# Andareon/Path-Tracing

Hardware: AMD Instinct MI355X
Metric: Msamples/sec (WxHxspp/wall) on Tor.obj 1080p x 256 spp (higher is better)
Workload: dtype f32

## Files before the change

path-tracing_amd/csrc/pt_capi.cpp:

```cpp
#include "pt_capi_internal.hpp"
#include "pt_bmp.hpp"

#include <algorithm>
#include <chrono>
#include <cmath>
#include <cstdio>
#include <cstdlib>
#include <cstring>
#include <thread>

#include "pt_filters.hpp"

static pt::plan::Overrides g_plan_overrides;

namespace ptc {

thread_local std::string g_error;

int fail(int code, const std::string &msg) {
    g_error = msg;
    return code;
}
int hip_fail(hipError_t e, const char *what) {
    const int code = (e == hipErrorNoDevice || e == hipErrorInvalidDevice || e == hipErrorInsufficientDriver)
                         ? PT_ERR_NO_DEVICE
                         : (e == hipErrorOutOfMemory ? PT_ERR_OUT_OF_MEMORY : PT_ERR_HIP);
    return fail(code, std::string(what) + ": " + hipGetErrorString(e));
}

std::atomic<long> g_live_device_objects{0};

int use_device(int device, const char *stage) {
    int n = 0;
    if (hipGetDeviceCount(&n) != hipSuccess || n <= 0 || device < 0 || device >= n)
        return fail(PT_ERR_NO_DEVICE, std::string(stage) + ": device " + std::to_string(device) + " is not a visible HIP device (there is no CPU fallback)");
    PT_HIP_TRY(hipSetDevice(device));
    return PT_OK;
}

}

using ptc::fail;
using ptc::guarded;
using ptc::hip_fail;

namespace {

int check_table_limits(unsigned long long n_slots, unsigned long long n_bvh_nodes, long long n_levels, long long bvh_depth = 0) {
    if (n_slots >= (1ull << 24))
        return fail(PT_ERR_UNSUPPORTED, "the culling hierarchy has " + std::to_string(n_slots) + " slots; (ray, slot) work items hold 24 bits");
    if (n_bvh_nodes >= (1ull << 20))
        return fail(PT_ERR_UNSUPPORTED, "the box tree has " + std::to_string(n_bvh_nodes) + " nodes; a node's child base holds 20 bits");
    if (n_bvh_nodes > 0 && n_slots >= (1ull << 23))
        return fail(PT_ERR_UNSUPPORTED, "the culling hierarchy has " + std::to_string(n_slots) + " slots under a box tree; a leaf's base (first slot / 8) holds 20 bits");
    if (bvh_depth > pt::kMaxBvhDepth)
        return fail(PT_ERR_UNSUPPORTED, "the box tree has " + std::to_string(bvh_depth) + " levels; the walk's stack slack holds " + std::to_string(pt::kMaxBvhDepth));
    if (n_levels > pt::kMaxLevels)
        return fail(PT_ERR_UNSUPPORTED, "a sphere tree has " + std::to_string(n_levels) + " levels; the walk holds " + std::to_string(pt::kMaxLevels));
    return PT_OK;
}

int get_cull(pt_scene_host &h, float eps, double r_camera, std::shared_ptr<const pt::CullTables> &out) {
    std::lock_guard<std::mutex> lock(h.cull_mutex);
#ifndef PT_TEST_HOOKS
    const double r_max = pt::cull_r_max(h.vertex_extent, r_camera);
    for (const auto &t : h.cull_cache)
        if (std::memcmp(&t->eps, &eps, sizeof eps) == 0 && t->r_max == r_max) {
            out = t;
            return PT_OK;
        }
#endif
    const auto t0 = std::chrono::steady_clock::now();
    auto t = std::make_shared<pt::CullTables>();
    pt::build_cull_tables(h.host, eps, *t, r_camera);
    t->eps = eps;
    h.cull_build_seconds += std::chrono::duration<double>(std::chrono::steady_clock::now() - t0).count();
    long long levels = 0;
    for (const auto &c : t->clusters)
        if (c.kind == 0) levels = std::max<long long>(levels, c.n_levels);
    const int rc = check_table_limits(t->slot_tri.size(), t->bvh.size(), levels, t->bvh_depth);
    if (rc != PT_OK) return rc;
    if (!t->big && (t->slot_tri.size() >= 65536u || h.host.n_tri() >= 65536))
        return fail(PT_ERR_UNSUPPORTED, "a scene on the sphere-tree path has " + std::to_string(t->slot_tri.size()) + " slots; its closest-hit key holds 16 bits");
    if (h.cull_cache.size() >= 4) h.cull_cache.erase(h.cull_cache.begin());
    h.cull_cache.push_back(t);
    out = t;
    return PT_OK;
}

int upload(pt_scene *s, int device) {
    int rc = ptc::use_device(device, "scene");
    if (rc != PT_OK) return rc;
    s->device = device;
    int cus = 0;
    if (hipDeviceGetAttribute(&cus, hipDeviceAttributeMultiprocessorCount, device) == hipSuccess && cus > 0) s->cu_count = cus;
    const auto &t = s->shared->tables;
    if ((rc = s->d_exact.upload(t.exact, "exact records", 64)) != PT_OK || (rc = s->d_mats.upload(t.mats, "materials", 64)) != PT_OK) return rc;
    if (s->sky && !s->sky->texels.empty()) {
        if ((rc = s->d_sky.upload(s->sky->texels, "skybox", 64)) != PT_OK) return rc;
        s->sky_w = s->sky->w;
        s->sky_h = s->sky->h;
    }
    if (s->env && (rc = s->d_env.upload(pt::env_with_apron(s->env->n, s->env->rgb.data()), "environment map", 64)) != PT_OK) return rc;
    if ((rc = ptc::upload_surface(s->surface, t, s->d_surface, s->d_surface)) != PT_OK) return rc;
    return PT_OK;
}

int ctx_stats_ready(LaunchCtx &c) {
    int rc = c.d_stats ? static_cast<int>(PT_OK) : c.d_stats.alloc(24 * sizeof(unsigned long long), "statistics block");
    if (rc == PT_OK && !c.ev0) rc = c.ev0.create("statistics");
    if (rc == PT_OK && !c.ev1) rc = c.ev1.create("statistics");
    return rc;
}

const pt_camera kReferenceCamera = {{0.0f, 0.0f, -20.0f}, {1.0f, 0.0f, 0.0f}, {0.0f, 1.0f, 0.0f}, {0.0f, 0.0f, 1.0f}};

using ptc::view_camera;

void lens_axes(const pt_camera &c, float out[9]) {
    const float *v[3] = {c.right, c.up, c.forward};
    for (int a = 0; a < 3; ++a) {
        const double x = v[a][0], y = v[a][1], z = v[a][2];
        const double n = std::sqrt(x * x + y * y + z * z);
        for (int i = 0; i < 3; ++i) out[3 * a + i] = static_cast<float>(v[a][i] / n);
    }
}

double lens_extent(const pt_camera &c, const pt_lens &l) {
    float ax[9];
    lens_axes(c, ax);
    double e = 0.0;
    for (int i = 0; i < 3; ++i) {
        const double lat = std::sqrt(static_cast<double>(ax[i]) * ax[i] + static_cast<double>(ax[3 + i]) * ax[3 + i]);
        double ei = std::fabs(static_cast<double>(c.origin[i]));
        if (lat > 0.0) ei = (ei + static_cast<double>(l.radius) * lat) * (1.0 + 0x1p-18);
        e = std::max(e, ei);
    }
    return e;
}

bool motion_active(const pt_scene *s) { return s->has_motion && std::memcmp(&view_camera(s), &s->motion_end, sizeof(pt_camera)) != 0; }

double motion_extent(const pt_camera &a, const pt_camera &b, const pt_lens *l) {
    float axa[9] = {0}, axb[9] = {0};
    if (l) {
        lens_axes(a, axa);
        lens_axes(b, axb);
    }
    double e = 0.0;
    for (int i = 0; i < 3; ++i) {
        const double lata = std::sqrt(static_cast<double>(axa[i]) * axa[i] + static_cast<double>(axa[3 + i]) * axa[3 + i]);
        const double latb = std::sqrt(static_cast<double>(axb[i]) * axb[i] + static_cast<double>(axb[3 + i]) * axb[3 + i]);
        const double radius = l ? static_cast<double>(l->radius) : 0.0;
        double ei = std::max(std::fabs(static_cast<double>(a.origin[i])) + radius * lata, std::fabs(static_cast<double>(b.origin[i])) + radius * latb);
        if (lata > 0.0 || latb > 0.0 || std::memcmp(&a.origin[i], &b.origin[i], sizeof(float)) != 0) ei *= 1.0 + 0x1p-18;
        e = std::max(e, ei);
    }
    return e;
}

double ortho_extent(const pt_camera &c) {
    double e = 0.0;
    for (int i = 0; i < 3; ++i)
        e = std::max(e, std::fabs(static_cast<double>(c.origin[i])) + 0.5 * (std::fabs(static_cast<double>(c.right[i])) + std::fabs(static_cast<double>(c.up[i]))));
    return e * (1.0 + 0x1p-18);
}
// ... 48 lines not shown
        const int rc = upload(s.get(), device);
        if (rc != PT_OK) return rc;
    }
    *out = s.release();
    return PT_OK;
}

void bind_surface(const pt_scene &scene, pt::RenderArgs &a) {
    const SurfaceTables &h = scene.surface;
    const DeviceSurface &d = scene.d_surface;
    const bool glass = h.glass && d.glass, tex = h.textures && d.tex_recs, smooth = h.smooth && d.normals, rough = h.rough && d.alpha,
               direct = h.direct && d.lights, envdirect = h.envdirect && d.env_alias && d.env_lights && scene.env && scene.d_env;
    const int unit = envdirect ? pt::kEnvDirectUnit : direct ? pt::kDirectUnit : rough ? pt::kRoughUnit : smooth ? pt::kSmoothUnit : tex ? pt::kTextureUnit : glass ? pt::kGlassUnit : pt::kNoSurfaceUnit;
    if (unit >= pt::kGlassUnit) a.glass = (glass ? d.glass : d.no_glass).get<void>();
    if (unit >= pt::kTextureUnit) {
        a.tex_recs = (tex ? d.tex_recs : d.no_tex).get<void>();
        a.tex_uv = (tex ? d.tex_uv : d.no_tex).get<float>();
        a.tex_texels = (tex ? d.tex_texels : d.no_tex).get<void>();
        a.tex_bary = d.bary.get<void>();
    }
    if (unit >= pt::kSmoothUnit) a.smooth_normals = (smooth ? d.normals : d.no_normals).get<void>();
    if (unit >= pt::kRoughUnit) a.rough_alpha = (rough ? d.alpha : d.no_alpha).get<float>();
    if (unit == pt::kDirectUnit) {
        a.lights = d.lights.get<void>();
        a.n_lights = static_cast<int32_t>(h.direct->lights.size());
        a.light_area = h.direct->area;
    }
    if (unit == pt::kEnvDirectUnit) {
        a.lights = d.env_lights.get<void>();
        a.n_lights = static_cast<int32_t>(h.envdirect->lights->lights.size());
        a.light_area = h.envdirect->lights->area;
        a.env_alias = d.env_alias.get<void>();
        a.env_cells = h.envdirect->cells;
        a.env_share = h.envdirect->share;
    }
}

void fill_scene_args(const pt_scene *scene, float eps, pt::RenderArgs &a) {
    std::memset(&a, 0, sizeof a);
    const pt::CullTables &t = *scene->cull.host;
    const pt::CullConstants &cc = t.cc, &ca = t.cc_all;
    a.clusters = scene->cull.clusters.get<pt::ClusterDesc>();
    a.spheres = scene->cull.spheres.get<pt::SphereRec>();
    a.bary = scene->cull.bary.get<pt::CullRec>();
    a.bary_all = scene->cull.bary_all.get<pt::CullRec>();
    a.a_max_all = ca.a_max; a.m0_all = ca.m0; a.t_guard_all = ca.t_guard;
    a.exact = scene->d_exact.get<pt::ExactRec>();
    a.exact_slot = scene->cull.exact_slot.get<pt::ExactRec>();
    a.bvh = scene->cull.bvh.get<pt::BvhNode>();
    a.n_bvh = static_cast<uint32_t>(t.bvh.size());
    a.bvh_err = t.bvh_err;
    a.mats = scene->d_mats.get<pt::MatRec>();
    a.n_mats = static_cast<int32_t>(scene->shared->tables.mats.size());
    a.sky = scene->d_sky.get<uint8_t>();
    a.sky_w = scene->d_sky ? scene->sky_w : 0;
    a.sky_h = scene->d_sky ? scene->sky_h : 0;
    if (scene->env && scene->d_env) {
        a.env_map = scene->d_env.get<void>();
        a.env_n = scene->env->n;
    }
    bind_surface(*scene, a);
    a.n_clusters = static_cast<int32_t>(t.clusters.size());
    a.n_tri = scene->shared->host.n_tri();
    a.big = t.big ? 1 : 0;
    a.n_slots = static_cast<uint32_t>(t.slot_tri.size());
    a.eps = eps;
    a.k1 = cc.k1; a.k2 = cc.k2; a.a_max = cc.a_max; a.m0 = cc.m0; a.m0_quad = cc.m0_quad; a.t_guard = cc.t_guard;
    a.r_org = t.r_org;
    a.may_leave_envelope = t.may_leave_envelope ? 1 : 0;
    a.last_segment_filter = 1;
#ifdef PT_TEST_HOOKS
    if (pt::g_cull_mutation.no_last_segment_filter) a.last_segment_filter = 0;
#endif
    a.regen_min_dead = 64;
    a.emis_clusters = t.emis_clusters;
    a.emis_large_w0 = t.emis_large_w0;
    a.emis_bvh = t.emis_bvh ? 1u : 0u;
    const bool moving = motion_active(scene);
    if (scene->has_camera || scene->has_lens || moving) {
        a.camera = 1;
        std::memcpy(a.cam, &view_camera(scene), sizeof a.cam);
    }
    if (scene->has_lens) {
        a.lens = 1;
        a.lns[0] = scene->lens.radius;
        a.lns[1] = scene->lens.focus_distance;
        lens_axes(view_camera(scene), a.lns + 2);
    }
    if (scene->has_projection) {
        a.camera = 1;
        std::memcpy(a.cam, &view_camera(scene), sizeof a.cam);
        a.projection = scene->projection.kind;
        a.prj_span[0] = scene->projection.span_x;
        a.prj_span[1] = scene->projection.span_y;
        lens_axes(view_camera(scene), a.lns + 2);
    }
    if (moving) {
        a.motion = 1;
        float end_pose[12];
        static_assert(sizeof end_pose == sizeof(pt_camera), "pt_camera: twelve floats");
        std::memcpy(end_pose, &scene->motion_end, sizeof end_pose);
        for (int j = 0; j < 12; ++j) a.cam_d[j] = end_pose[j] - a.cam[j];
        if (scene->has_lens) {
            float end_axes[9];
            lens_axes(scene->motion_end, end_axes);
            for (int j = 0; j < 9; ++j) a.lns_d[j] = end_axes[j] - a.lns[2 + j];
        }
    }
}

void zero_stats(const pt_scene *scene, pt_render_stats *stats) {
    std::memset(stats, 0, sizeof *stats);
    stats->n_triangles = scene->shared->host.n_tri();
}

int enqueue_render(pt_scene *scene, LaunchCtx &ctx, const pt_render_params *p, const ptc::AccumPlanes &planes, hipStream_t stream,
                   bool want_stats) {
    ctx.stats_pending = false;
    ctx.last_chunks = 0;
    PT_HIP_TRY(hipSetDevice(scene->device));
    std::lock_guard<std::mutex> launch_lock(scene->launch_mutex);
    const int crc = ensure_cull(scene, p->eps);
    if (crc != PT_OK) return crc;
    pt::RenderArgs a;
    fill_scene_args(scene, p->eps, a);
    if (scene->surface.direct && !a.lights) return fail(PT_ERR_INVALID_ARGUMENT, "direct lighting: the handle has the switch set and no light table on its device");
    if (scene->surface.envdirect && !a.env_alias) return fail(PT_ERR_INVALID_ARGUMENT, "environment sampling: the handle has the switch set and no table on its device");
    a.vec_ok = (p->width % 4 == 0) &&
               ((reinterpret_cast<uintptr_t>(planes.sum) | reinterpret_cast<uintptr_t>(planes.sum2) | reinterpret_cast<uintptr_t>(planes.count)) % 16 == 0);
    a.sum = planes.sum;
    a.sum2 = planes.sum2;
    a.count = planes.count;
    a.width = p->width; a.height = p->height; a.row_begin = p->row_begin; a.row_end = p->row_end;
    a.row_stride = std::max(1, p->row_stride);
    a.band_rows = ptc::band_rows(p);
    const pt::plan::Overrides &ov = g_plan_overrides;
    a.regen_min_dead = ov.regen_min_dead > 0 ? static_cast<uint32_t>(ov.regen_min_dead) : pt::regen_min_dead_for(p->max_ray_reflections);
    a.pass_begin = p->pass_begin; a.pass_count = p->pass_count; a.mrr = p->max_ray_reflections;
    a.error = p->error; a.seed = p->seed;
    if (p->row_end == p->row_begin) return PT_OK;
    int rc;
    if (a.projection == PT_PROJECTION_ORTHOGRAPHIC) {
        for (int i = 0; i < 3; ++i)
            if (!(0.5 * (std::fabs(static_cast<double>(a.cam[3 + i])) / a.width + std::fabs(static_cast<double>(a.cam[6 + i])) / a.height) <= 0.5))
                return fail(PT_ERR_UNSUPPORTED, "orthographic projection: a pixel of this image is wider than one scene unit (|right_i| / width + |up_i| / height > 1)");
    }
    if (!ctx.ev_done && (rc = ctx.ev_done.create("launch context", hipEventDisableTiming)) != PT_OK) return rc;
    if (want_stats) {
        if ((rc = ctx_stats_ready(ctx)) != PT_OK) return rc;
        a.stats = ctx.d_stats.get<unsigned long long>();
    }
    const bool sky = a.sky != nullptr || a.env_map != nullptr;
    const pt::plan::Tiles tiles = pt::plan::plan_tiles({a.width, a.band_rows, sky, a.big != 0, want_stats, a.may_leave_envelope != 0, a.error,
                                                        a.pass_begin, a.pass_count, pt::plan::view_of(a.camera != 0, a.lens != 0, a.motion != 0), scene->cu_count},
                                                       pt::integrator_build(), ov);
    a.narrow = tiles.narrow;
    a.adapt_pool = tiles.adapt_pool;
    a.blocks_x = tiles.blocks_x;
    const uint32_t n_tiles = tiles.n_tiles;
    int waves_per_cu = 24;
    PT_HIP_TRY(pt::integrator_waves_per_cu(tiles.variant, &waves_per_cu));
    const uint32_t slots = static_cast<uint32_t>(scene->cu_count) * static_cast<uint32_t>(std::max(1, waves_per_cu));
    const auto [n_chunks, chunk_passes] = pt::plan::plan_chunks(n_tiles, slots, p->pass_count, sky, a.narrow != 0, want_stats, ov);
    if (static_cast<unsigned long long>(n_tiles) * n_chunks > 0x7fffffffull) return fail(PT_ERR_INVALID_ARGUMENT, "too many work items");
    if (ctx.has_prev && ctx.prev_stream != stream) PT_HIP_TRY(hipStreamWaitEvent(stream, ctx.ev_done.get(), 0));
    const size_t sched_bytes = (1 + static_cast<size_t>(n_tiles)) * sizeof(uint32_t);
    if (ctx.d_sched.bytes() < sched_bytes) {
        if (ctx.has_prev) PT_HIP_TRY(hipStreamSynchronize(stream));
        if ((rc = ctx.d_sched.alloc(sched_bytes, "scheduler words")) != PT_OK) return rc;
    }
    PT_HIP_TRY(hipMemsetAsync(ctx.d_sched.get<void>(), 0, sched_bytes, stream));
    a.sched = ctx.d_sched.get<uint32_t>();
    a.n_tiles = n_tiles;
    a.n_chunks = n_chunks;
    a.chunk_passes = chunk_passes;
    if (want_stats) {
        PT_HIP_TRY(hipMemsetAsync(ctx.d_stats.get<void>(), 0, 24 * sizeof(unsigned long long), stream));
        PT_HIP_TRY(hipEventRecord(ctx.ev0.get(), stream));
    }
    const hipError_t launched = pt::launch_integrator(a, tiles.variant, stream);
    if (const int unit = pt::surface_unit_of(a); launched == hipErrorNotSupported && unit != pt::kNoSurfaceUnit) {
        static const char *const kWhat[][2] = {{"dielectrics", "dielectric"}, {"textures", "texture"}, {"shading normals", "smooth"}, {"roughness", "rough"}, {"direct lighting", "direct"}, {"environment sampling", "environment-sampling"}};
        const char *const *w = kWhat[unit - pt::kGlassUnit];
        return fail(PT_ERR_UNSUPPORTED, std::string(w[0]) + ": this diagnostic build of the library has no " + w[1] + " kernels");
    }
    PT_HIP_TRY(launched);
    if (want_stats) PT_HIP_TRY(hipEventRecord(ctx.ev1.get(), stream));
    PT_HIP_TRY(hipEventRecord(ctx.ev_done.get(), stream));
    ctx.has_prev = true;
    ctx.prev_stream = stream;
    ctx.last_chunks = n_chunks;
    ctx.stats_pending = want_stats;
    return PT_OK;
}

int collect_stats(pt_scene *scene, LaunchCtx &ctx, hipStream_t stream, pt_render_stats *stats) {
    zero_stats(scene, stats);
    if (!ctx.stats_pending) return PT_OK;
    ctx.stats_pending = false;
    PT_HIP_TRY(hipSetDevice(scene->device));
    unsigned long long h[24];
    PT_HIP_TRY(hipMemcpyAsync(h, ctx.d_stats.get<void>(), sizeof h, hipMemcpyDeviceToHost, stream));
    PT_HIP_TRY(hipStreamSynchronize(stream));
    float ms = -1.0f;
    PT_HIP_TRY(hipEventElapsedTime(&ms, ctx.ev0.get(), ctx.ev1.get()));
    stats->samples_traced = h[0];
    stats->segments = h[1];
    stats->contributing = h[2];
    stats->exact_tests = h[3];
    stats->misses = h[4];
    stats->wave_segments = h[5];
    stats->wave_node_rounds = h[6];
    stats->wave_exact_iterations = h[7];
    stats->kernel_ms = ms;
    stats->n_chunks = static_cast<int32_t>(ctx.last_chunks);
    stats->partial_commit_rounds = static_cast<int32_t>(std::min<unsigned long long>(h[8], 0x7fffffffull));
    stats->verify_checked = h[9];
    stats->verify_mismatches = h[10];
#ifdef PT_TEST_HOOKS
    if (h[10] != 0) {
        auto f = [](unsigned long long w, int hi) { const uint32_t b = static_cast<uint32_t>(hi ? w >> 32 : w); float x; std::memcpy(&x, &b, 4); return x; };
        std::fprintf(stderr, "PT_VERIFY example: all-triangles loop -> triangle %d (key %016llx), culled search -> triangle %d (key %016llx); "
                             "ray o = (%.9g, %.9g, %.9g) d = (%.9g, %.9g, %.9g)\n",
                     static_cast<int>(h[11] & 0xFFFFFFFFu), h[11], static_cast<int>(h[12] & 0xFFFFFFFFu), h[12],
                     f(h[13], 1), f(h[13], 0), f(h[14], 1), f(h[14], 0), f(h[15], 1), f(h[15], 0));
    }
#endif
#ifdef PT_PHASE_TIMERS
    std::fprintf(stderr, "PT_PHASE_TIMERS cycles:");
    for (int k = 0; k < 8; ++k) std::fprintf(stderr, " %llu", h[16 + k]);
    std::fprintf(stderr, "\n");
#endif
    return PT_OK;
}

}

namespace ptc {

int32_t band_rows(const pt_render_params *p) {
    const int32_t rows = p->row_end - p->row_begin;
    if (p->row_stride <= 1 || rows <= 0) return rows;
    const int32_t period = 8 * p->row_stride;
    return 8 * ((rows + period - 1) / period);
}

int check_params(const pt_scene *scene, const pt_render_params *p) {
    if (!scene || !p) return fail(PT_ERR_INVALID_ARGUMENT, "null scene or params");
    if (const int rc = check_has_device(scene)) return rc;
    if (p->width <= 0 || p->height <= 0) return fail(PT_ERR_INVALID_ARGUMENT, "width and height must be positive");
    if (p->row_begin < 0 || p->row_end > p->height || p->row_begin > p->row_end)
        return fail(PT_ERR_INVALID_ARGUMENT, "row band outside the image");
    if (p->row_stride < 0 || (p->row_stride > 1 && p->row_begin % 8 != 0))
        return fail(PT_ERR_INVALID_ARGUMENT, "row_stride must be 0 / 1 (contiguous rows) or n > 1 with row_begin a multiple of 8 (every n-th tile row of 8 rows)");
    if (p->pass_begin < 0 || p->pass_count < 0) return fail(PT_ERR_INVALID_ARGUMENT, "negative pass range");
    if (static_cast<long long>(p->width) * p->height > 0x7fffffffLL)
        return fail(PT_ERR_INVALID_ARGUMENT, "image has more than 2^31 pixels");
    if (p->rng_policy == PT_RNG_REFERENCE_STREAM)
        return fail(PT_ERR_UNSUPPORTED, "PT_RNG_REFERENCE_STREAM: the reference's serial minstd_rand0 streams (material.h:16-20) have no "
                                        "parallel evaluation order; the device implements PT_RNG_COUNTER");
    if (p->rng_policy != PT_RNG_COUNTER) return fail(PT_ERR_INVALID_ARGUMENT, "unknown rng_policy");
    return PT_OK;
}

int session_create_on(pt_scene *scene, int32_t width, int32_t height, int32_t row_begin, int32_t row_end, const AccumPlanes *borrowed,
                      pt_session **out, int32_t row_stride) {
    if (!out) return fail(PT_ERR_INVALID_ARGUMENT, "null argument");
    *out = nullptr;
    pt_render_params p;
    std::memset(&p, 0, sizeof p);
    p.width = width; p.height = height; p.row_begin = row_begin; p.row_end = row_end; p.row_stride = row_stride;
    int rc = check_params(scene, &p);
    if (rc != PT_OK) return rc;
    PT_HIP_TRY(hipSetDevice(scene->device));
    std::unique_ptr<pt_session> s(new pt_session);
    s->scene = scene;
    s->width = width; s->height = height; s->row_begin = row_begin; s->row_end = row_end; s->row_stride = std::max(1, row_stride);
    s->n = static_cast<size_t>(band_rows(&p)) * width;
    if ((rc = s->stream.create("pt_session_create")) != PT_OK) return rc;
    if (borrowed) {
        s->planes = *borrowed;
        s->planes.n = s->n;
    } else {
        PlaneLayout l;
        s->planes = AccumPlanes::in(l, s->n);
        if ((rc = s->d_band.alloc(l.end + 256, "pt_session_create")) != PT_OK) return rc;
        PT_HIP_TRY(hipMemsetAsync(s->d_band.get<void>(), 0, s->d_band.bytes(), s->stream.get()));
        s->planes.bind(s->d_band);
    }
    *out = s.release();
    return PT_OK;
}

int session_enqueue(pt_session *s, const pt_render_params *p, bool want_stats) {
    if (!s || !p) return fail(PT_ERR_INVALID_ARGUMENT, "null session or params");
    if (p->width != s->width || p->height != s->height || p->row_begin != s->row_begin || p->row_end != s->row_end ||
        std::max(1, p->row_stride) != s->row_stride)
        return fail(PT_ERR_INVALID_ARGUMENT, "params describe another band than the session's");
    const int rc = check_params(s->scene, p);
    if (rc != PT_OK) return rc;
    return enqueue_render(s->scene, s->ctx, p, s->planes, s->stream.get(), want_stats);
}

const pt_camera &view_camera(const pt_scene *s) { return s->has_camera ? s->camera : kReferenceCamera; }

int scene_trace_args(pt_scene *scene, float eps, pt::RenderArgs &a) {
    const int rc = ensure_cull(scene, eps);
    if (rc != PT_OK) return rc;
    fill_scene_args(scene, eps, a);
    return PT_OK;
}

int session_collect(pt_session *s, pt_render_stats *stats) {
    if (!s || !stats) return fail(PT_ERR_INVALID_ARGUMENT, "null argument");
    return collect_stats(s->scene, s->ctx, s->stream.get(), stats);
}

}

using ptc::check_params;

extern "C" {

int pt_abi_version(void) { return PT_ABI_VERSION; }

void *pt_host_alloc(size_t bytes) {
    void *p = nullptr;
    if (hipHostMalloc(&p, bytes ? bytes : 1, hipHostMallocDefault) != hipSuccess) {
        ptc::g_error = "pt_host_alloc: hipHostMalloc failed";
        return nullptr;
    }
    return p;
}

void pt_host_free(void *p) {
    if (p) (void)hipHostFree(p);
}

int pt_device_count(void) {
// ... 764 lines not shown

int pt_scene_create(const float *triangles, const int32_t *triangle_material, int32_t n_triangles, const float *materials, int32_t n_materials, int device, pt_scene **out) {
    return guarded([&] { return scene_create_impl(triangles, triangle_material, n_triangles, materials, n_materials, device, out); });
}

int pt_scene_clone_to_device(const pt_scene *scene, int device, pt_scene **out) {
    return guarded([&] { return scene_clone_impl(scene, device, out); });
}

int pt_scene_set_skybox_bmp(pt_scene *scene, const char *path) {
    return guarded([&] { return scene_set_skybox_bmp_impl(scene, path); });
}

int pt_camera_look_at(const float eye[3], const float target[3], const float up[3], float fov_y_degrees, float aspect, pt_camera *out) {
    return guarded([&] { return camera_look_at_impl(eye, target, up, fov_y_degrees, aspect, out); });
}

int pt_scene_set_camera(pt_scene *scene, const pt_camera *camera) {
    return guarded([&] {
        if (!scene) return fail(PT_ERR_INVALID_ARGUMENT, "null scene");
        std::lock_guard<std::mutex> launch_lock(scene->launch_mutex);
        return scene_set_camera_impl(scene, camera);
    });
}

int pt_scene_get_camera(const pt_scene *scene, pt_camera *camera, int32_t *is_set) {
    return guarded([&] { return scene_get_camera_impl(scene, camera, is_set); });
}

int pt_scene_set_lens(pt_scene *scene, const pt_lens *lens) {
    return guarded([&] {
        if (!scene) return fail(PT_ERR_INVALID_ARGUMENT, "null scene");
        std::lock_guard<std::mutex> launch_lock(scene->launch_mutex);
        return scene_set_lens_impl(scene, lens);
    });
}

int pt_scene_get_lens(const pt_scene *scene, pt_lens *lens, int32_t *is_set) {
    return guarded([&] { return scene_get_lens_impl(scene, lens, is_set); });
}

int pt_scene_set_camera_motion(pt_scene *scene, const pt_camera *end) {
    return guarded([&] {
        if (!scene) return fail(PT_ERR_INVALID_ARGUMENT, "null scene");
        std::lock_guard<std::mutex> launch_lock(scene->launch_mutex);
        return scene_set_camera_motion_impl(scene, end);
    });
}

int pt_scene_get_camera_motion(const pt_scene *scene, pt_camera *end, int32_t *is_set) {
    return guarded([&] { return scene_get_camera_motion_impl(scene, end, is_set); });
}

int pt_projection_make(int32_t kind, float fov_y_degrees, float aspect, pt_projection *out) {
    return guarded([&] { return projection_make_impl(kind, fov_y_degrees, aspect, out); });
}

int pt_camera_ortho(const float eye[3], const float target[3], const float up[3], float view_height, float aspect, pt_camera *out) {
    return guarded([&] { return camera_ortho_impl(eye, target, up, view_height, aspect, out); });
}

int pt_scene_set_projection(pt_scene *scene, const pt_projection *projection) {
    return guarded([&] {
        if (!scene) return fail(PT_ERR_INVALID_ARGUMENT, "null scene");
        std::lock_guard<std::mutex> launch_lock(scene->launch_mutex);
        return scene_set_projection_impl(scene, projection);
    });
}

int pt_scene_get_projection(const pt_scene *scene, pt_projection *projection, int32_t *is_set) {
    return guarded([&] { return scene_get_projection_impl(scene, projection, is_set); });
}

int pt_render_device(pt_scene *scene, const pt_render_params *p, float *d_sum, float *d_sum2, int32_t *d_count, void *hip_stream, pt_render_stats *stats) {
    return guarded([&] { return render_device_impl(scene, p, d_sum, d_sum2, d_count, hip_stream, stats); });
}

int pt_trace_rays_host(pt_scene *scene, int32_t n_rays, const float *origins, const float *directions, float eps, int32_t *hit_index, float *hit_t) {
    return guarded([&] { return trace_rays_host_impl(scene, n_rays, origins, directions, eps, hit_index, hit_t); });
}

int pt_render_host(pt_scene *scene, const pt_render_params *p, float *sum, float *sum2, int32_t *count, pt_render_stats *stats) {
    return guarded([&] { return render_host_impl(scene, p, sum, sum2, count, stats); });
}

int32_t pt_band_rows(const pt_render_params *params) { return params ? ptc::band_rows(params) : 0; }

int pt_session_create_strided(pt_scene *scene, int32_t width, int32_t height, int32_t row_begin, int32_t row_end, int32_t row_stride,
                              pt_session **out) {
    return guarded([&] { return ptc::session_create_on(scene, width, height, row_begin, row_end, nullptr, out, row_stride); });
}

int pt_session_create(pt_scene *scene, int32_t width, int32_t height, int32_t row_begin, int32_t row_end, pt_session **out) {
    return guarded([&] { return ptc::session_create_on(scene, width, height, row_begin, row_end, nullptr, out, 1); });
}

int pt_session_render(pt_session *session, const pt_render_params *params, pt_render_stats *stats) {
    return guarded([&] { return session_render_impl(session, params, stats); });
}

int pt_session_wait(pt_session *session) {
    return guarded([&] {
        if (!session) return fail(PT_ERR_INVALID_ARGUMENT, "null session");
        PT_HIP_TRY(hipSetDevice(session->scene->device));
        PT_HIP_TRY(hipStreamSynchronize(session->stream.get()));
        return static_cast<int>(PT_OK);
    });
}

int pt_session_read(pt_session *session, float *sum, float *sum2, int32_t *count) {
    return guarded([&] { return session_read_impl(session, sum, sum2, count); });
}

int pt_session_clear(pt_session *session) {
    return guarded([&] { return session_clear_impl(session); });
}

void pt_session_destroy(pt_session *s) { delete s; }

int pt_scene_cull_tables(pt_scene *scene, float eps, int32_t *counts, float *clusters, float *spheres, float *bary, float *constants) {
    return guarded([&] { return scene_cull_tables_impl(scene, eps, counts, clusters, spheres, bary, constants); });
}

int pt_scene_cull_layout(pt_scene *scene, float eps, int32_t *counts, int32_t *slot_triangle, void *bvh_nodes) {
    return guarded([&] { return scene_cull_layout_impl(scene, eps, counts, slot_triangle, bvh_nodes); });
}

int pt_post_filter_host(int device, int32_t width, int32_t height, float *rgb, int32_t gauss, int32_t median) {
    return guarded([&] { return post_filter_host_impl(device, width, height, rgb, gauss, median); });
}

#ifdef PT_TEST_HOOKS
int pt_test_box_masks(const void *nodes, const float *rays, const float *t_best, float err, int32_t n, uint32_t *out) {
    if (!nodes || !rays || !t_best || !out || n < 0) return fail(PT_ERR_INVALID_ARGUMENT, "null argument");
    if (n == 0) return PT_OK;
    PT_HIP_TRY(hipSetDevice(0));
    ptc::DeviceBuffer d_nodes, d_rays, d_t, d_out;
    const size_t nn = static_cast<size_t>(n);
    int rc;
    if ((rc = d_nodes.alloc(nn * 64, "pt_test_box_masks")) != PT_OK || (rc = d_rays.alloc(nn * 24, "pt_test_box_masks")) != PT_OK ||
        (rc = d_t.alloc(nn * 4, "pt_test_box_masks")) != PT_OK || (rc = d_out.alloc(nn * 4, "pt_test_box_masks")) != PT_OK)
        return rc;
    PT_HIP_TRY(hipMemcpy(d_nodes.get<void>(), nodes, nn * 64, hipMemcpyHostToDevice));
    PT_HIP_TRY(hipMemcpy(d_rays.get<void>(), rays, nn * 24, hipMemcpyHostToDevice));
    PT_HIP_TRY(hipMemcpy(d_t.get<void>(), t_best, nn * 4, hipMemcpyHostToDevice));
    PT_HIP_TRY(pt::launch_box_masks(d_nodes.get<pt::BvhNode>(), d_rays.get<float>(), d_t.get<float>(), err, n, d_out.get<uint32_t>(), nullptr));
    PT_HIP_TRY(hipDeviceSynchronize());
    PT_HIP_TRY(hipMemcpy(out, d_out.get<void>(), nn * 4, hipMemcpyDeviceToHost));
    return PT_OK;
}

long pt_test_live_device_objects(void) { return ptc::g_live_device_objects.load(std::memory_order_relaxed); }

int pt_test_set_mutation(const char *family, double value) {
    if (!family) return PT_ERR_INVALID_ARGUMENT;
    const std::string f = family;
    pt::CullMutation &m = pt::g_cull_mutation;
    if (f == "reset") { m = pt::CullMutation(); g_plan_overrides = pt::plan::Overrides(); }
    else if (f == "regen_min_dead") g_plan_overrides.regen_min_dead = static_cast<int>(value);
    else if (f == "chunk_min") g_plan_overrides.chunk_min = static_cast<int>(value);
    else if (f == "sphere_r2") m.sphere_r2 = value;
    else if (f == "m0") m.m0 = value;
    else if (f == "k12") m.k12 = value;
    else if (f == "a_max") m.a_max = value;
    else if (f == "quad_slack") m.quad_slack = value;
    else if (f == "box") m.box = value;
    else if (f == "box_err") m.box_err = value;
    else if (f == "no_absorb") m.no_absorb = value != 0;
    else if (f == "no_last_segment_filter") m.no_last_segment_filter = value != 0;
    else if (f == "emis_drop") m.emis_drop = value != 0;
    else if (f == "order_mode") m.order_mode = static_cast<int>(value);
    else if (f == "bvh_fill") m.bvh_fill = value;
    else if (f == "bvh_mode") m.bvh_mode = static_cast<int>(value);
    else if (f == "bvh_depth_cap") m.bvh_depth_cap = static_cast<int>(value);
    else if (f == "big_threshold") m.big_threshold = static_cast<int>(value);
    else if (f == "max_clusters") m.max_clusters = static_cast<int>(value);
    else if (f == "items_per_slot") g_plan_overrides.items_per_slot = static_cast<int>(value);
    else if (f == "tile_width") g_plan_overrides.tile_width = static_cast<int>(value);
    else return fail(PT_ERR_INVALID_ARGUMENT, "unknown mutation family " + f);
    return PT_OK;
}
#endif

}
```

path-tracing_amd/csrc/pt_cull_tables.cpp:

```cpp
#include "pt_scene.hpp"

#include <algorithm>
#include <cmath>
#include <cstring>

namespace pt {

#ifdef PT_TEST_HOOKS
CullMutation g_cull_mutation;
#define PT_KNOB(field, shipped) (g_cull_mutation.field)
#else
#define PT_KNOB(field, shipped) (shipped)
#endif

namespace {

struct V3 {
    double x, y, z;
};
inline V3 sub(V3 a, V3 b) { return {a.x - b.x, a.y - b.y, a.z - b.z}; }
inline V3 crs(V3 a, V3 b) { return {a.y * b.z - a.z * b.y, a.z * b.x - a.x * b.z, a.x * b.y - a.y * b.x}; }
inline double dt(V3 a, V3 b) { return a.x * b.x + a.y * b.y + a.z * b.z; }
inline double nrm(V3 a) { return std::sqrt(dt(a, a)); }

// ... 817 lines not shown
}

struct RecordMaxima {
    double a_max = 0;
    double inv_2s = 0;
    double diam2_2s = 0;
    void add(const TriGeo &g) {
        if (g.degenerate) return;
        a_max = std::max(a_max, g.a_max);
        inv_2s = std::max(inv_2s, 1.0 / (2.0 * g.area2));
        diam2_2s = std::max(diam2_2s, g.diam * g.diam / (2.0 * g.area2));
    }
};

struct QuadRecord {
    V3 ral, rbe;
    double cal, cbe;
    double dev;
};
void bary_rows(const TriGeo &g, int i0, int i1, int i2, V3 rows[3], double cst[3]) {
    const DualRows d = dual_rows(sub(g.v[i1], g.v[i0]), sub(g.v[i2], g.v[i0]));
    rows[1] = d.u;
    rows[2] = d.v;
    rows[0] = {-(rows[1].x + rows[2].x), -(rows[1].y + rows[2].y), -(rows[1].z + rows[2].z)};
    cst[1] = -dt(rows[1], g.v[i0]); cst[2] = -dt(rows[2], g.v[i0]); cst[0] = 1.0 - cst[1] - cst[2];
}
bool fuse_quad(const float *ra, const float *rb, const TriGeo &ga, const TriGeo &gb, QuadRecord &q) {
    if (std::memcmp(ra, rb, 16) != 0 || ga.degenerate || gb.degenerate) return false;
    int sa[2], sb[2], ns = 0, apex_a = -1, apex_b = -1;
    bool used_b[3] = {false, false, false};
    for (int x = 0; x < 3; ++x) {
        int match = -1;
        for (int y = 0; y < 3; ++y)
            if (!used_b[y] && std::memcmp(ra + 4 + 3 * x, rb + 4 + 3 * y, 12) == 0) { match = y; break; }
        if (match >= 0 && ns < 2) { sa[ns] = x; sb[ns] = match; used_b[match] = true; ++ns; }
        else apex_a = x;
    }
    if (ns != 2 || apex_a < 0) return false;
    for (int y = 0; y < 3; ++y) if (!used_b[y]) apex_b = y;
    const V3 s0 = ga.v[sa[0]], pa = ga.v[apex_a], pb = gb.v[apex_b];
    const V3 ea = sub(pa, s0), eb = sub(pb, s0);
    const V3 nn = crs(ea, eb);
    const double s2 = dt(nn, nn);
    if (!(s2 > 0)) return false;
    const DualRows d = dual_rows(ea, eb);
    q.ral = d.u;
    q.rbe = d.v;
    q.cal = -dt(q.ral, s0);
    q.cbe = -dt(q.rbe, s0);
    V3 rowa[3], rowb[3];
    double ca[3], cb[3];
    bary_rows(ga, sa[0], sa[1], apex_a, rowa, ca);
    bary_rows(gb, sb[0], sb[1], apex_b, rowb, cb);
    const V3 nu = {nn.x / std::sqrt(s2), nn.y / std::sqrt(s2), nn.z / std::sqrt(s2)};
    const double hh = 0.05 * std::max(ga.diam, gb.diam);
    q.dev = 0;
    for (int c8 = 0; c8 < 8; ++c8) {
        const double al = (c8 & 1) ? 2.0 : -1.0, be = (c8 & 2) ? 2.0 : -1.0, h = (c8 & 4) ? hh : -hh;
        const V3 P = {s0.x + al * ea.x + be * eb.x + h * nu.x, s0.y + al * ea.y + be * eb.y + h * nu.y, s0.z + al * ea.z + be * eb.z + h * nu.z};
        const double a_ = dt(q.ral, P) + q.cal, b_ = dt(q.rbe, P) + q.cbe;
        const double da[3] = {1 - a_, b_, a_ - b_}, db[3] = {1 - b_, a_, b_ - a_};
        for (int t3 = 0; t3 < 3; ++t3) {
            q.dev = std::max(q.dev, std::fabs(dt(rowa[t3], P) + ca[t3] - da[t3]));
            q.dev = std::max(q.dev, std::fabs(dt(rowb[t3], P) + cb[t3] - db[t3]));
        }
    }
    return q.dev < 0.01;
}

double append_large_cluster(const HostScene &s, const std::vector<TriGeo> &geo, const Envelope &env, const std::vector<int> &order,
                            int first, int n, CullTables &out, RecordMaxima &maxima) {
    ClusterDesc cd = cluster_over(geo, env, order, first, n, 1u);
    cd.data_off = static_cast<uint32_t>(out.bary.size());
    const int n_words = (n + kChunk - 1) / kChunk;
    auto row = [&](int k) { return &s.tri[14 * static_cast<size_t>(order[first + k])]; };
    for (int k = 0; k < n_words * kChunk; ++k) {
        CullRec c;
        std::memset(&c, 0, sizeof c);
        if (k < n) {
            c = cull_record(row(k), geo[order[first + k]]);
            maxima.add(geo[order[first + k]]);
        }
        out.bary.push_back(c);
    }
    double quad_slack = 0;
    for (int w = 0; w < n_words && w < kMaxLevels - 1; ++w) {
        uint32_t qmask = 0;
        for (int k = w * kChunk; k + 1 < std::min(n, (w + 1) * kChunk); k += 2) {
            QuadRecord q;
            if (!fuse_quad(row(k), row(k + 1), geo[order[first + k]], geo[order[first + k + 1]], q)) continue;
            quad_slack = std::max(quad_slack, q.dev);
            maxima.a_max = std::max(maxima.a_max, std::max(nrm(q.ral), std::max(nrm(q.rbe), nrm(sub(q.ral, q.rbe)))));
            set_rows(out.bary[cd.data_off + k], q.ral, q.rbe, q.cal, q.cbe);
            std::memset(&out.bary[cd.data_off + k + 1], 0, sizeof(CullRec));
            qmask |= 1u << (k - w * kChunk);
        }
        cd.level_off[w] = qmask;
    }
    out.clusters.push_back(cd);
    return quad_slack;
}

RecordMaxima fill_bary_all(const HostScene &s, const std::vector<TriGeo> &geo, const std::vector<int> &order, CullTables &out) {
    RecordMaxima maxima;
    out.bary_all.resize(order.size() + 4);
    for (auto &c : out.bary_all) std::memset(&c, 0, sizeof c);
    for (size_t k = 0; k < order.size(); ++k) {
        if (order[k] < 0) continue;
        out.bary_all[k] = cull_record(&s.tri[14 * static_cast<size_t>(order[k])], geo[order[k]]);
        maxima.add(geo[order[k]]);
    }
    return maxima;
}

CullConstants margins(const RecordMaxima &mx, double quad_slack, const Envelope &env, double eps) {
    const double r_org = env.r_org, a_max = mx.a_max;
    CullConstants cc;
    cc.k2 = static_cast<float>(PT_MUT(k12) * (12.0 * kU * env.m_abs + 8.0 * kU * r_org));
    cc.k1 = static_cast<float>(PT_MUT(k12) * 40.0 * kU);
    cc.a_max = static_cast<float>(PT_MUT(a_max) * a_max * (1.0 + 1e-6));
    cc.m0 = static_cast<float>(PT_MUT(m0) * (std::fabs(eps) * mx.inv_2s * 1.01 + 48.0 * kU * mx.diam2_2s
                                             + 16.0 * kU * a_max * r_org * std::sqrt(3.0) + 1e-6));
    double tg = 4096.0 * r_org;
    if (a_max > 0) tg = std::min(tg, 1.0e6 / a_max);
    cc.t_guard = static_cast<float>(tg);
    cc.m0_quad = static_cast<float>(static_cast<double>(cc.m0) + PT_MUT(quad_slack) * (quad_slack * 1.01 + 8.0 * kU * a_max * r_org));
    return cc;
}

void fill_emitter_masks(const HostScene &s, int n_small_slots, CullTables &out) {
    auto emits = [&](uint32_t slot) {
        const uint32_t t = slot < out.slot_tri.size() ? out.slot_tri[slot] : kNoTriangle;
        return t != kNoTriangle && triangle_emits(s, static_cast<int>(t));
    };
    out.emis_clusters = 0;
    out.emis_large_w0 = 0xFFFFFFFFu;
    for (size_t c = 0; c < out.clusters.size(); ++c) {
        const ClusterDesc &cd = out.clusters[c];
        bool any = false;
        for (uint32_t k = 0; k < cd.n_tri; ++k) any = any || emits(cd.first_tri + k);
        if (c >= 32 || any) out.emis_clusters |= c < 32 ? (1u << c) : 0u;
        if (cd.kind == 1u && cd.n_tri <= static_cast<uint32_t>(kChunk)) {
            out.emis_large_w0 = 0;
            for (uint32_t k = 0; k < cd.n_tri; ++k) out.emis_large_w0 |= emits(cd.first_tri + k) ? (1u << k) : 0u;
        }
    }
    if (out.clusters.size() > 32) out.emis_clusters = 0xFFFFFFFFu;
    if (PT_KNOB(emis_drop, 0) && out.emis_large_w0 != 0xFFFFFFFFu) out.emis_large_w0 &= out.emis_large_w0 - 1u;
    out.emis_bvh = false;
    if (!out.bvh.empty())
        for (uint32_t k = 0; k < static_cast<uint32_t>(n_small_slots); ++k) out.emis_bvh = out.emis_bvh || emits(k);
}

}

double vertex_extent(const HostScene &s) {
    double r = 0.0;
    for (int i = 0; i < s.n_tri(); ++i)
        for (int k = 4; k < 13; ++k) r = std::max(r, static_cast<double>(std::fabs(s.tri[14 * static_cast<size_t>(i) + k])));
    return r;
}

void build_cull_tables(const HostScene &s, float eps_f, CullTables &out, double r_camera) {
    const int T = s.n_tri();
    const double eps = eps_f;
    out = CullTables();
    out.eps = eps_f;
    const int hook = PT_KNOB(big_threshold, -1);
    out.big = T > (hook >= 0 ? std::min(hook, kSmallSceneMaxTriangles) : kBigSceneTriangles);

    const Envelope env = envelope_of(vertex_extent(s), r_camera);
    out.r_max = env.r_max;
    out.r_org = static_cast<float>(env.r_org);
    std::vector<TriGeo> geo(T);
    std::vector<Centroid> cen(T);
    for (int i = 0; i < T; ++i) {
        geo[i] = tri_geometry(&s.tri[14 * static_cast<size_t>(i)], eps);
        const V3 *v = geo[i].v;
        cen[i] = {{(v[0].x + v[1].x + v[2].x) / 3, (v[0].y + v[1].y + v[2].y) / 3, (v[0].z + v[1].z + v[2].z) / 3}};
    }
    const Classes classes = classify(s, geo, env, out.big);
    out.may_leave_envelope = may_leave_envelope(geo, env);

    std::vector<int> order;
    std::vector<std::pair<int, int>> small_runs;
    order_small_class(s, geo, cen, env, classes.groups, out, order, small_runs);
    const int n_small_slots = static_cast<int>(order.size());
    order_large_class(s, geo, cen, classes.large, order);
    const int n_large = static_cast<int>(order.size()) - n_small_slots;

    fill_slot_tables(s, order, out);
    for (const auto &run : small_runs) append_sphere_tree(geo, env, order, run.first, run.second, out);
    RecordMaxima large_maxima, all_maxima;
    double quad_slack = 0;
    if (n_large > 0) quad_slack = append_large_cluster(s, geo, env, order, n_small_slots, n_large, out, large_maxima);
    for (int k = 0; k < 16 + 8 * 64; ++k) out.spheres.push_back(kNeverSphere);
    for (int k = 0; k < 4; ++k) { CullRec c; std::memset(&c, 0, sizeof c); out.bary.push_back(c); }
    if (out.big) all_maxima = fill_bary_all(s, geo, order, out);

    out.cc = margins(large_maxima, quad_slack, env, eps);
    const CullConstants all = margins(all_maxima, 0.0, env, eps);
    out.cc_all = out.cc;
    out.cc_all.a_max = all.a_max;
    out.cc_all.m0 = all.m0;
    out.cc_all.t_guard = all.t_guard;

    fill_emitter_masks(s, n_small_slots, out);
}

}
```

path-tracing_amd/csrc/pt_integrator_body.inc:

```
    constexpr int POOL = ADAPT & ~1;
    constexpr bool CAM = (ADAPT & 1) != 0;
    static_assert(!LENS || CAM, "a lens kernel is the lens variant of a camera twin");
    static_assert(!DIRECT || (SMOOTH && ROUGH), "the direct term is written in the smooth scatter step: a direct kernel is a rough kernel with DIRECT");
    static_assert(!ENVDIRECT || (DIRECT && ENVMAP), "an environment-sampling kernel is a direct kernel with an environment");
    static_assert(!MOTION || CAM, "a motion kernel is the motion variant of a camera twin or of its lens kernel");
    static_assert(!PROJ || (CAM && !LENS && !MOTION), "a projection kernel is the projection variant of a camera twin; the host refuses a lens or a motion with it");
    static_assert(!NARROW || (!SKY && !STATS), "only the statistics-free, skybox-free kernels have a narrow variant");
    static_assert(!ENVMAP || SKY, "an environment kernel is the environment variant of a skybox kernel: regeneration, no last-segment filter");
    constexpr int R = NARROW ? 1 : rays_per_lane<SKY, BIG, STATS>();
    static_assert(POOL == 0 || ((POOL == 2 || POOL == 4) && (R == 2 || BIG) && !STATS && !SKY), "batches of the tile's pixels (a pixel's number takes 8 bits): the two-pixel kernel and the box-tree kernel");
    constexpr bool REGEN = SKY;
    static_assert(!REGEN || !POOL, "the compacting instantiation keeps the pass loop");
    constexpr bool kDynSlots = POOL == 2 && R == 2;
    constexpr int kOwn = POOL ? POOL : R;
    constexpr int kTW = kTileW * kOwn;
    __shared__ WaveLds<std::conditional_t<BIG, std::conditional_t<POOL != 0, BigQueuesAdapt<POOL>, BigQueues>, std::conditional_t<(R > 1), SmallQueues2, SmallQueues>>, R, POOL> lds;

    const int lane = threadIdx.x;
    if constexpr (decltype(lds)::kMatCache > 0) {
        if (a.n_mats <= decltype(lds)::kMatCache) {
            const float4 *src = reinterpret_cast<const float4 *>(a.mats);
            for (int i = lane; i < 3 * a.n_mats; i += 64) lds.mat.v[i] = src[i];
            wave_sync();
        }
    }
    uint32_t item = 0;
    if (lane == 0) item = atomicAdd(&a.sched[0], 1u);
    item = __builtin_amdgcn_readfirstlane(item);
    const uint32_t tile = item % a.n_tiles, chunk = item / a.n_tiles;
    int pass_first, pass_last;
    if (a.chunk_passes > 0) {
        pass_first = a.pass_begin + static_cast<int>(chunk) * a.chunk_passes;
        pass_last = min(a.pass_begin + a.pass_count, pass_first + a.chunk_passes);
    } else {
        pass_first = a.pass_begin + (a.pass_count - (a.pass_count >> (2u * chunk)));
        pass_last = a.pass_begin + (chunk + 1 < a.n_chunks ? a.pass_count - (a.pass_count >> (2u * (chunk + 1u))) : a.pass_count);
    }
    if (chunk > 0) {
        if (lane == 0) {
            while (__hip_atomic_load(&a.sched[1 + tile], __ATOMIC_RELAXED, __HIP_MEMORY_SCOPE_AGENT) < chunk) __builtin_amdgcn_s_sleep(8);
        }
        __builtin_amdgcn_fence(__ATOMIC_ACQUIRE, "agent");
        asm volatile("s_waitcnt vmcnt(0)" ::: "memory");
        __builtin_amdgcn_wave_barrier();
    }
    int tile_x0 = static_cast<int>(tile % a.blocks_x) * kTW, acc_y0 = static_cast<int>(tile / a.blocks_x) * kTileH;
    if constexpr (POOL != 0) {
        tile_x0 = __builtin_amdgcn_readfirstlane(tile_x0);
        acc_y0 = __builtin_amdgcn_readfirstlane(acc_y0);
    }
    const int tile_y0 = a.row_begin + acc_y0 * a.row_stride;
    int x[R];
    const int y = tile_y0 + (lane / kTileW);
    bool in_image[R];
    uint32_t gpix[R];
#pragma unroll
    for (int k = 0; k < R; ++k) {
        x[k] = tile_x0 + (lane % kTileW) + kTileW * k;
        in_image[k] = x[k] < a.width && y < a.row_end;
        gpix[k] = static_cast<uint32_t>(static_cast<size_t>(y) * a.width + x[k]);
    }

    constexpr bool kAccInLds = decltype(lds)::kAccInLds;
    if constexpr (kAccInLds) {
#pragma unroll
    for (int k = 0; k < R; ++k) {
        if (in_image[k]) {
            const size_t p = static_cast<size_t>(acc_y0 + lane / kTileW) * a.width + x[k];
            const int id = lane + 64 * k;
#pragma unroll
            for (int c = 0; c < 3; ++c) {
                lds.acc.v[c][id] = a.sum[3 * p + c];
                lds.acc.v[3 + c][id] = a.sum2[3 * p + c];
            }
            lds.acc.v[6][id] = __int_as_float(a.count[p]);
        }
    }
    }
    auto low_variance = [&](float c0, float c1, float c2, float q0, float q1, float q2, int n) {
        const float sc = static_cast<float>(n);
        if (!(sc > 0)) return false;
        const float mr = c0 / sc, mg_ = c1 / sc, mb = c2 / sc;
        const float dr = q0 / sc - mr * mr, dg = q1 / sc - mg_ * mg_, db = q2 / sc - mb * mb;
        return dr < a.error && dg < a.error && db < a.error;
    };
    bool lowvar[R];
#pragma unroll
    for (int k = 0; k < R; ++k) {
        lowvar[k] = false;
        if constexpr (POOL) {
        } else if constexpr (!kAccInLds) {
            if (in_image[k] && a.error >= 0.0f) {
                const size_t p = static_cast<size_t>(acc_y0 + lane / kTileW) * a.width + x[k];
                lowvar[k] = low_variance(a.sum[3 * p], a.sum[3 * p + 1], a.sum[3 * p + 2], a.sum2[3 * p], a.sum2[3 * p + 1], a.sum2[3 * p + 2], a.count[p]);
            }
        } else {
            const int id = lane + 64 * k;
            if (in_image[k]) lowvar[k] = low_variance(lds.acc.v[0][id], lds.acc.v[1][id], lds.acc.v[2][id], lds.acc.v[3][id], lds.acc.v[4][id],
                                                      lds.acc.v[5][id], __float_as_int(lds.acc.v[6][id]));
        }
    }
    uint32_t jobs = 0;
    auto job_of = [&](int k) { return (opaque(jobs) >> (8 * k)) & 0xFFu; };
    auto tile_x_of = [&](uint32_t j) { return tile_x0 + static_cast<int>((j & 63u) % kTileW) + kTileW * static_cast<int>(j >> 6); };
    auto tile_y_of = [&](uint32_t j) { return tile_y0 + static_cast<int>((j & 63u) / kTileW); };
    if constexpr (POOL) {
#pragma unroll
        for (int kb = 0; kb < kOwn; ++kb) {
            const uint32_t j = static_cast<uint32_t>(lane) + 64u * kb;
            bool low = false;
            if (tile_x_of(j) < a.width && y < a.row_end) {
                const size_t p = static_cast<size_t>(acc_y0 + lane / kTileW) * a.width + tile_x_of(j);
                low = low_variance(a.sum[3 * p], a.sum[3 * p + 1], a.sum[3 * p + 2], a.sum2[3 * p], a.sum2[3 * p + 1], a.sum2[3 * p + 2], a.count[p]);
            }
            lds.low.v[j] = static_cast<uint16_t>((static_cast<uint32_t>(pass_first) << 1) | (low ? 1u : 0u));
        }
        wave_sync();
    }
    auto contribute = [&](int k, float cr, float cg, float cb) {
        float n0, n1, n2, p0, p1, p2;
        int nn;
        if constexpr (!kAccInLds) {
            uint32_t le = opaque(static_cast<uint32_t>(lane));
            int kb = k;
            if constexpr (POOL) {
                const uint32_t j = job_of(k);
                le = j & 63u;
                kb = static_cast<int>(j >> 6);
            }
            const size_t p = static_cast<size_t>(acc_y0 + static_cast<int>(le / kTileW)) * a.width + (tile_x0 + static_cast<int>(le % kTileW) + kTileW * kb);
            n0 = a.sum[3 * p] + cr; n1 = a.sum[3 * p + 1] + cg; n2 = a.sum[3 * p + 2] + cb;
            p0 = a.sum2[3 * p] + cr * cr; p1 = a.sum2[3 * p + 1] + cg * cg; p2 = a.sum2[3 * p + 2] + cb * cb;
            nn = a.count[p] + 1;
            a.sum[3 * p] = n0; a.sum[3 * p + 1] = n1; a.sum[3 * p + 2] = n2;
            a.sum2[3 * p] = p0; a.sum2[3 * p + 1] = p1; a.sum2[3 * p + 2] = p2;
            a.count[p] = nn;
        } else {
            const int id = lane + 64 * k;
            n0 = lds.acc.v[0][id] + cr; n1 = lds.acc.v[1][id] + cg; n2 = lds.acc.v[2][id] + cb;
            p0 = lds.acc.v[3][id] + cr * cr; p1 = lds.acc.v[4][id] + cg * cg; p2 = lds.acc.v[5][id] + cb * cb;
            nn = __float_as_int(lds.acc.v[6][id]) + 1;
            lds.acc.v[0][id] = n0; lds.acc.v[1][id] = n1; lds.acc.v[2][id] = n2;
            lds.acc.v[3][id] = p0; lds.acc.v[4][id] = p1; lds.acc.v[5][id] = p2;
            lds.acc.v[6][id] = __int_as_float(nn);
        }
        const bool now_low = low_variance(n0, n1, n2, p0, p1, p2, nn);
        if constexpr (POOL) {
            const uint32_t pj = job_of(k);
            lds.low.v[pj] = static_cast<uint16_t>((lds.low.v[pj] & ~1u) | (now_low ? 1u : 0u));
        } else {
            lowvar[k] = now_low;
        }
    };
    using Count = std::conditional_t<STATS, uint32_t, Ignored>;
// ... 222 lines not shown
            } else {
                q[k].ox = 0.0f; q[k].oy = 0.0f; q[k].oz = -20.0f;
            }
            tr[k] = tg[k] = tb[k] = 1.0f;
            depth[k] = 0;
            if constexpr (DIRECT) {
                Lr[k] = Lg[k] = Lb[k] = 0.0f;
                lit[k] = false;
            }
        };
        auto primary_ray = [&](int k, int pass_k) {
            float ddx, ddy, ddz;
            const float t = primary_dir(k, pass_k, ddx, ddy, ddz);
            start_path(k, ddx, ddy, ddz, t);
        };
        auto pass_of = [&](int k) {
            if constexpr (POOL) {
                return static_cast<int>(lds.low.v[job_of(k)] >> 1) - 1;
            } else if constexpr (REGEN) {
                return cur_pass[k];
            } else {
                return pass;
            }
        };
        if constexpr (!REGEN) {
#pragma unroll
            for (int k = 0; k < R; ++k) {
                tr[k] = tg[k] = tb[k] = 1.0f;
                depth[k] = mrr;
                if (PT_SLOT_ON(k) && !skip[k]) {
                    primary_ray(k, pass_of(k));
                } else {
                    q[k].ox = q[k].oy = q[k].oz = 0.0f; q[k].dx = q[k].dy = 0.0f; q[k].dz = 1.0f;
                }
                if constexpr (STATS) n_traced += __builtin_popcountll(__ballot(!skip[k]));
            }
        }
        [[maybe_unused]] auto path_over = [&](int k) { return !(depth[k] < mrr && (tr[k] != 0.0f || tg[k] != 0.0f || tb[k] != 0.0f)); };
        for (;;) {
            bool valid[R];
#pragma unroll
            for (int k = 0; k < R; ++k) valid[k] = depth[k] < mrr && (tr[k] != 0.0f || tg[k] != 0.0f || tb[k] != 0.0f);
            [[maybe_unused]] bool shadow_phase = false;
            if constexpr (DIRECT) {
                shadow_phase = any_of(pending);
                if (shadow_phase) {
#pragma unroll
                    for (int k = 0; k < R; ++k) {
                        valid[k] = pending[k];
                        if (pending[k]) {
                            float t;
                            t = q[k].dx; q[k].dx = sdx[k]; sdx[k] = t;
                            t = q[k].dy; q[k].dy = sdy[k]; sdy[k] = t;
                            t = q[k].dz; q[k].dz = sdz[k]; sdz[k] = t;
                        }
                    }
                }
            }
            if constexpr (REGEN) {
                if (!shadow_phase) {
                uint32_t n_wait = 0;
                bool wants[R];
#pragma unroll
                for (int k = 0; k < R; ++k) {
                    wants[k] = false;
                    if (!valid[k] && in_image[k]) {
                        int np = next_pass[k];
                        if (np > 10 && (np & 3) && lowvar[k]) np = (np + 3) & ~3;
                        next_pass[k] = np;
                        wants[k] = np < pass_last;
                    }
                    n_wait += __builtin_popcountll(__ballot(wants[k]));
                }
                if (n_wait >= a.regen_min_dead || (n_wait > 0 && !any_of(valid))) {
#pragma unroll
                    for (int k = 0; k < R; ++k) {
                        if (wants[k]) {
                            cur_pass[k] = next_pass[k];
                            primary_ray(k, next_pass[k]);
                            next_pass[k] = next_pass[k] + 1;
                        }
                        valid[k] = valid[k] || wants[k];
                        if constexpr (STATS) n_traced += __builtin_popcountll(__ballot(wants[k]));
                    }
                }
                }
            }
            if (!any_of(valid)) break;
#ifdef PT_ADAPT_COUNT
            if (two) ++c_seg2; else ++c_seg1;
#endif
            if constexpr (STATS) {
                if (!shadow_phase) {
#pragma unroll
                for (int k = 0; k < R; ++k) n_segments += __builtin_popcountll(__ballot(valid[k]));
                }
            }

            float best[R];
            int hit[R];
            const ExactRec *hit_rec[R];
            bool inside[R];
#pragma unroll
            for (int k = 0; k < R; ++k) {
                inside[k] = true;
                if constexpr (ENV)
                    inside[k] = __builtin_fmaxf(__builtin_fmaxf(__builtin_fabsf(q[k].ox), __builtin_fabsf(q[k].oy)), __builtin_fabsf(q[k].oz)) <= a.r_org;
            }
            bool searched[R], last_or_dead[R];
#pragma unroll
            for (int k = 0; k < R; ++k) {
                searched[k] = valid[k];
                last_or_dead[k] = !valid[k] || depth[k] + 1 >= mrr;
            }
            bool all_last = last_or_dead[0];
#pragma unroll
            for (int k = 1; k < R; ++k) all_last = all_last && last_or_dead[k];
            if constexpr (DIRECT) all_last = all_last && !shadow_phase;
            constexpr bool kLastSegmentFilter = !STATS && !SKY && !BIG;
            bool emis_phase = false;
            if constexpr (kLastSegmentFilter) emis_phase = a.last_segment_filter != 0u && __all(all_last);
#ifdef PT_VERIFY_SHIPPED
            bool filtered_last = emis_phase;
#endif
            if constexpr (BIG && !STATS && !SKY) {
                if (a.last_segment_filter != 0u && a.emis_bvh == 0u && a.n_clusters == 1 && __all(all_last)) {
                    const ConstF cp = (ConstF)reinterpret_cast<uintptr_t>(a.clusters) + (sizeof(ClusterDesc) / 4) * (a.n_clusters - 1);
                    const uint32_t n_large = ((ConstU)cp)[5], kind = ((ConstU)cp)[6], off = ((ConstU)cp)[7], quads = ((ConstU)cp)[9];
                    if (kind == 1u && n_large <= static_cast<uint32_t>(kChunk)) {
                        float k1 = a.k1, k2 = a.k2, a_max = a.a_max, m0 = a.m0, m0q = a.m0_quad, t_guard = a.t_guard;
                        asm volatile("" : "+v"(k1), "+v"(k2), "+v"(a_max), "+v"(m0), "+v"(m0q), "+v"(t_guard));
                        const ConstF bp = (ConstF)reinterpret_cast<uintptr_t>(a.bary) + 12 * static_cast<size_t>(off);
                        uint32_t m = 0;
                        for (uint32_t rest = (a.emis_large_w0 | (a.emis_large_w0 >> 1)) & 0x55555555u; rest != 0; rest &= rest - 1) {
                            const uint32_t k0 = __builtin_ctz(rest);
                            if ((quads >> k0) & 1u) {
                                m |= (~cull_reject_quad(load_cull(bp + 12 * k0), q[0], k1, k2, a_max, m0q, t_guard) & 3u) << k0;
                            } else {
                                for (uint32_t j = 0; j < 2; ++j)
                                    m |= cull_reject(load_cull(bp + 12 * (k0 + j)), q[0], k1, k2, a_max, m0, t_guard) ? 0u : (1u << (k0 + j));
                            }
                        }
                        bool can_reach = (m & a.emis_large_w0) != 0u;
                        if constexpr (ENV) can_reach = can_reach || !inside[0];
                        searched[0] = valid[0] && can_reach;
#ifdef PT_VERIFY_SHIPPED
                        filtered_last = true;
#endif
                    }
                }
            }
            for (;;) {
                if (BIG && !any_of(searched)) break;
                closest_hit<ENV, kLastSegmentFilter, kDynSlots>(a, lds, q, searched, inside, lane, eps, best, hit, hit_rec, wst, emis_phase, two);
                if (!emis_phase) break;
                emis_phase = false;
#pragma unroll
                for (int k = 0; k < R; ++k) searched[k] = searched[k] && hit[k] >= 0;
                if (!any_of(searched)) break;
            }
#pragma unroll
            for (int k = 0; k < R; ++k)
                if (!searched[k]) hit[k] = -1;
#ifdef PT_VERIFY_SHIPPED
#pragma unroll
            for (int k = 0; k < R; ++k) {
                const unsigned long long brute = brute_force_key(a, q[k], eps);
                const unsigned long long mine = hit[k] < 0 ? ~0ull : ((static_cast<unsigned long long>(ordered_bits(best[k])) << 32) | static_cast<uint32_t>(hit[k]));
                bool ok = brute == mine;
                if (!ok && filtered_last && mine == ~0ull) {
                    bool emissive = false;
                    if (brute != ~0ull) {
                        const MatRec m = a.mats[a.exact[static_cast<uint32_t>(brute)].material];
                        emissive = (m.n_lobes >= 1 && m.kind0 == 0) || (m.n_lobes >= 2 && m.kind1 == 0);
                    }
                    ok = !emissive;
                }
                v_checked += static_cast<uint32_t>(__builtin_popcountll(__ballot(valid[k])));
                v_bad += static_cast<uint32_t>(__builtin_popcountll(__ballot(valid[k] && !ok)));
                if (valid[k] && !ok && a.stats) {
                    a.stats[11] = brute;
                    a.stats[12] = mine;
                    a.stats[13] = (static_cast<unsigned long long>(__float_as_uint(q[k].ox)) << 32) | __float_as_uint(q[k].oy);
                    a.stats[14] = (static_cast<unsigned long long>(__float_as_uint(q[k].oz)) << 32) | __float_as_uint(q[k].dx);
                    a.stats[15] = (static_cast<unsigned long long>(__float_as_uint(q[k].dy)) << 32) | __float_as_uint(q[k].dz);
                }
            }
#endif

            if constexpr (DIRECT) {
                if (shadow_phase) {
#pragma unroll
                    for (int k = 0; k < R; ++k) {
                        bool added = false;
                        if (PT_SLOT_ON(k) && pending[k]) {
                            if (hit[k] == slight[k]) {
                                Lr[k] += scr[k]; Lg[k] += scg[k]; Lb[k] += scb[k];
                                added = true;
                            }
                            q[k].dx = sdx[k]; q[k].dy = sdy[k]; q[k].dz = sdz[k];
                            pending[k] = false;
                            if (path_over(k)) contribute(k, Lr[k], Lg[k], Lb[k]);
                        }
                        if constexpr (STATS) n_contrib += __builtin_popcountll(__ballot(added));
                    }
                    continue;
                }
            }
#pragma unroll
            for (int k = 0; k < R; ++k) {
            if constexpr (STATS) n_miss += __builtin_popcountll(__ballot(valid[k] && hit[k] < 0));
            bool contributed = false;
            if (PT_SLOT_ON(k) && valid[k]) {
                if (hit[k] < 0) {
                    if constexpr (ENVMAP) {
                        const EnvironmentView ev = environment_view();
                        float lr, lg, lb;
                        env_lookup(ev.map(), ev.n(), q[k].dx, q[k].dy, q[k].dz, lr, lg, lb);
                        if constexpr (ENVDIRECT) {
                            if (!lit[k]) {
                                Lr[k] += tr[k] * lr; Lg[k] += tg[k] * lg; Lb[k] += tb[k] * lb;
                                contributed = true;
                            }
                        } else if constexpr (DIRECT) {
                            Lr[k] += tr[k] * lr; Lg[k] += tg[k] * lg; Lb[k] += tb[k] * lb;
                            contributed = true;
                        } else {
                        contribute(k, tr[k] * lr, tg[k] * lg, tb[k] * lb);
                        contributed = true;
                        }
                    } else if (SKY) {
                        const float pi = 3.141593f;
                        const float theta = portable_acosf(q[k].dy) / pi;
                        const float phi = portable_atan2f(q[k].dz, -q[k].dx) / pi / 2 + 0.5f;
                        const uint32_t sw = static_cast<uint32_t>(a.sky_w), sh = static_cast<uint32_t>(a.sky_h);
                        const float sx = phi * static_cast<float>(sw), sy = theta * static_cast<float>(sh);
                        uint32_t x1 = (sx >= 0.0f) ? (sx < 4294967040.0f ? static_cast<uint32_t>(sx) : 0xFFFFFFFFu) : 0u;
                        uint32_t y1 = (sy >= 0.0f) ? (sy < 4294967040.0f ? static_cast<uint32_t>(sy) : 0xFFFFFFFFu) : 0u;
                        x1 = min(x1, sw - 1u);
                        y1 = min(y1, sh - 1u);
                        const uint32_t x2 = (x1 + 1u) % sw, y2 = (y1 + 1u) % sh;
                        const uint8_t *t1 = a.sky + (static_cast<size_t>(y1) * sw + x1) * 3, *t2 = a.sky + (static_cast<size_t>(y1) * sw + x2) * 3;
                        const uint8_t *t3 = a.sky + (static_cast<size_t>(y2) * sw + x1) * 3, *t4 = a.sky + (static_cast<size_t>(y2) * sw + x2) * 3;
                        const float ax = 1 - sx + static_cast<float>(x1), ay = 1 - sy + static_cast<float>(y1);
                        float c[3];
#pragma unroll
                        for (int ch = 0; ch < 3; ++ch) {
                            const float c1 = static_cast<float>(t1[2 - ch]), c2 = static_cast<float>(t2[2 - ch]);
                            const float c3 = static_cast<float>(t3[2 - ch]), c4 = static_cast<float>(t4[2 - ch]);
                            const float c12 = c1 * (1.0f - ax) + c2 * ax;
                            const float c34 = c3 * (1.0f - ax) + c4 * ax;
                            c[ch] = (c12 * (1.0f - ay) + c34 * ay) / 256.f;
                        }
                        if constexpr (DIRECT) {
                            Lr[k] += c[0]; Lg[k] += c[1]; Lb[k] += c[2];
                        } else
                        contribute(k, c[0], c[1], c[2]);
                        contributed = true;
                    }
                    depth[k] = mrr;
                } else {
                    const ExactRec *__restrict__ rec = hit_rec[k];
                    const float4 pl = reinterpret_cast<const float4 *>(rec)[0];
                    const int mi = rec->material;
                    const float px = q[k].ox + q[k].dx * best[k], py = q[k].oy + q[k].dy * best[k], pz = q[k].oz + q[k].dz * best[k];
                    float4 m0v, m1v;
                    int4 m2v;
                    bool mat_cached = false;
                    if constexpr (decltype(lds)::kMatCache > 0) mat_cached = a.n_mats <= decltype(lds)::kMatCache;
                    if (mat_cached) {
                        if constexpr (decltype(lds)::kMatCache > 0) {
                            m0v = lds.mat.v[3 * mi]; m1v = lds.mat.v[3 * mi + 1];
                            const float4 t = lds.mat.v[3 * mi + 2];
                            m2v = make_int4(__float_as_int(t.x), __float_as_int(t.y), __float_as_int(t.z), __float_as_int(t.w));
                        }
                    } else {
                        m0v = reinterpret_cast<const float4 *>(a.mats + mi)[0];
                        m1v = reinterpret_cast<const float4 *>(a.mats + mi)[1];
                        m2v = reinterpret_cast<const int4 *>(a.mats + mi)[2];
                    }
                    uint32_t w0 = 0, w1 = 0, w2 = 0, w3;
                    if (depth[k] + 1 < mrr || (m2v.x >= 2 && (m2v.y == 0 || m2v.z == 0)))
                        philox4x32_10(rng_pixel(k), static_cast<uint32_t>(pass_of(k)), static_cast<uint32_t>(depth[k]), 0u, a.seed, kPhiloxKey1,
                                      w0, w1, w2, w3);
                    int kind;
                    if (m2v.x == 0) {
                        kind = -1;
                    } else if (m2v.x == 1) {
                        kind = m2v.y;
                    } else {
                        const float sample = unit_float(w0);
                        kind = (sample - m0v.w > 0) ? m2v.z : m2v.y;
                    }
                    [[maybe_unused]] const GlassRec *grec = nullptr;
                    [[maybe_unused]] float g_ior = 0.0f;
                    if constexpr (GLASS) {
                        grec = glass_view() + mi;
                        g_ior = grec->ior;
                        if (g_ior != 0.0f) kind = 3;
                    }
                    [[maybe_unused]] float sb1 = 0.0f, sb2 = 0.0f;
                    if constexpr (SMOOTH) {
                        const bool scatters = kind > 0 && depth[k] + 1 < mrr;
                        const TextureView tv = texture_view();
                        const size_t ti = static_cast<size_t>(rec->orig);
                        TexRec tm = {0u, 0, 0, 0};
                        if (kind == 0 || (kind == 2 && scatters)) tm = tv.recs()[mi];
// ... 349 lines not shown
```

path-tracing_amd/csrc/pt_kernels.hip:

```cpp
#include <hip/hip_runtime.h>

#include <array>
#include <atomic>
#include <cstddef>
#include <type_traits>
#include <utility>

#include "pt_fastfp.hpp"
#include "pt_kernels.hpp"
#include "pt_projection.hpp"
#include "pt_environment.hpp"
#include "pt_texture.hpp"
#include "pt_smooth.hpp"
#include "pt_rough.hpp"
#include "pt_direct.hpp"
#include "pt_envdirect.hpp"

#pragma clang fp contract(off)

namespace pt {

namespace {

#ifndef PT_WAVES_PER_SIMD
// ... 275 lines not shown
    const float d = (x * x + y * y) + z * z;
    float inv;
    if (__all(fast_fp_ok(d))) inv = rcp_rn_normal(sqrt_rn_normal(d));
    else inv = 1.0f / __builtin_sqrtf(d);
    x = x * inv; y = y * inv; z = z * inv;
}

}

template <int N> struct AccPlanes { float v[7][N]; };
template <> struct AccPlanes<0> {};
template <int N> struct FlagWords { uint16_t v[N]; };
template <> struct FlagWords<0> {};
#ifndef PT_MATS_IN_LDS
#define PT_MATS_IN_LDS 16
#endif
template <int N> struct InvPlanes { float v[3][N]; };
template <> struct InvPlanes<0> {};
template <int N> struct MatCache { float4 v[3 * N]; };
template <> struct MatCache<0> {};
template <class Q, int R, int FLAGS = 0>
struct WaveLds {
    static constexpr int kRays = R, kSlots = 64 * R;
    static constexpr int kNodeStack = Q::kNodeStack, kPairQueue = Q::kPairQueue;
    static constexpr bool kPrefilter = Q::kFiltered > 1;
    static_assert(R == 1 || R == 2, "ray ids take 6 or 7 bits of a work item");
    static constexpr uint32_t kSrcMask = kSlots - 1, kNodeSrcShift = R == 1 ? 26 : 25, kNodeLevShift = kNodeSrcShift - 3;
    static_assert(Q::kPairQueue >= 128, "push_pairs_any publishes slices of up to 128 pairs");
    static_assert(!kPrefilter || Q::kFiltered >= 128, "the pre-filter appends up to 64 survivors to up to 63 waiting ones");
    static_assert(!kPrefilter || Q::kFiltered >= PT_BIG_EXACT_AT - 1 + 64, "up to PT_BIG_EXACT_AT - 1 pairs wait when 64 survivors are appended");
    static_assert(Q::kNodeStack >= 64, "a round pops up to 64 nodes");
    uint32_t filtered[Q::kFiltered];
    unsigned long long best[kSlots];
    float ray[6][kSlots];
    InvPlanes<kPrefilter ? kSlots : 0> rinv;
    uint32_t nodes[kNodeStack + 64];
    uint32_t pairs[kPairQueue];
    uint32_t level_off[kMaxLevels];
    uint32_t level_cnt[kMaxLevels];
    static constexpr bool kAccInLds = R == 1 && !kPrefilter;
    AccPlanes<kAccInLds ? kSlots : 0> acc;
    FlagWords<64 * FLAGS> low;
    static constexpr int kMatCache = (R == 2 && !kPrefilter) ? PT_MATS_IN_LDS : 0;
    MatCache<kMatCache> mat;
};
struct WaveStats {
    uint32_t n_exact = 0, w_segments = 0, w_node_rounds = 0, w_exact_iters = 0, w_partial = 0;
#ifdef PT_VERIFY_BRUTE
    uint32_t v_checked = 0, v_bad = 0;
#endif
#ifdef PT_PHASE_TIMERS
    unsigned long long phase[8] = {0, 0, 0, 0, 0, 0, 0, 0};
    unsigned long long last = 0;
#endif
};
struct Ignored {
    __host__ __device__ Ignored() {}
    __host__ __device__ Ignored(uint32_t) {}
    template <class T> __host__ __device__ Ignored &operator+=(T) { return *this; }
    __host__ __device__ Ignored &operator++() { return *this; }
};
struct NoStats {
    Ignored n_exact, w_segments, w_node_rounds, w_exact_iters, w_partial;
#ifdef PT_VERIFY_BRUTE
    Ignored v_checked, v_bad;
#endif
#ifdef PT_PHASE_TIMERS
    unsigned long long phase[8] = {0, 0, 0, 0, 0, 0, 0, 0}, last = 0;
#endif
};
#ifdef PT_PHASE_TIMERS
#define PT_STAMP(st, idx)                                              \
    do {                                                               \
        const unsigned long long now_ = __builtin_amdgcn_s_memtime();  \
        (st).phase[idx] += now_ - (st).last;                           \
        (st).last = now_;                                              \
    } while (0)
#else
#define PT_STAMP(st, idx) do { } while (0)
#endif

constexpr uint32_t kUnfiltered = 128u;

__device__ __forceinline__ uint32_t ordered_bits(float f) {
    const uint32_t b = __float_as_uint(f);
    return b ^ ((b >> 31) ? 0xFFFFFFFFu : 0x80000000u);
}
__device__ __forceinline__ float from_ordered_bits(uint32_t b) {
    return __uint_as_float(b ^ ((b >> 31) ? 0x80000000u : 0xFFFFFFFFu));
}
__device__ __forceinline__ uint32_t opaque(uint32_t v) {
    asm volatile("" : "+v"(v));
    return v;
}
__device__ __forceinline__ uint32_t lanes_below(unsigned long long mask) {
    return __builtin_amdgcn_mbcnt_hi(static_cast<uint32_t>(mask >> 32), __builtin_amdgcn_mbcnt_lo(static_cast<uint32_t>(mask), 0u));
}


__device__ __forceinline__ float byte_to_float(uint32_t w, int k) { return static_cast<float>((w >> (8 * k)) & 0xFFu); }
template <int PER = 8>
__device__ __forceinline__ uint32_t box_children_kept(const uint4 q0, const uint4 q1, const uint4 q2, const uint4 q3, const Ray &r,
                                                      float ix, float iy, float iz, float t_best, float err, uint32_t sub = 0) {
    const float step = __uint_as_float((q0.w & 0xFFu) << 23);
    const float ax = step * ix, ay = step * iy, az = step * iz;
    const float bx = (__uint_as_float(q0.x) - r.ox) * ix, by = (__uint_as_float(q0.y) - r.oy) * iy, bz = (__uint_as_float(q0.z) - r.oz) * iz;
    const float bmax = __builtin_fmaxf(__builtin_fmaxf(__builtin_fabsf(bx), __builtin_fabsf(by)), __builtin_fabsf(bz));
    const float amax = __builtin_fmaxf(__builtin_fmaxf(__builtin_fabsf(ax), __builtin_fabsf(ay)), __builtin_fabsf(az));
    const float e2 = 2.0f * err * __builtin_fmaf(255.0f, amax, bmax);
    const float nbx = bx - e2, nby = by - e2, nbz = bz - e2, t_min = -e2;
    const bool sx = ix < 0.0f, sy = iy < 0.0f, sz = iz < 0.0f;
    uint32_t nx0 = sx ? q2.z : q1.x, nx1 = sx ? q2.w : q1.y, fx0 = sx ? q1.x : q2.z, fx1 = sx ? q1.y : q2.w;
    uint32_t ny0 = sy ? q3.x : q1.z, ny1 = sy ? q3.y : q1.w, fy0 = sy ? q1.z : q3.x, fy1 = sy ? q1.w : q3.y;
    uint32_t nz0 = sz ? q3.z : q2.x, nz1 = sz ? q3.w : q2.y, fz0 = sz ? q2.x : q3.z, fz1 = sz ? q2.y : q3.w;
    if constexpr (PER < 8) {
        const uint32_t c0 = sub * PER;
        const bool up = c0 >= 4u;
        const uint32_t sh = 8u * (c0 & 3u);
        nx0 = (up ? nx1 : nx0) >> sh; fx0 = (up ? fx1 : fx0) >> sh;
        ny0 = (up ? ny1 : ny0) >> sh; fy0 = (up ? fy1 : fy0) >> sh;
        nz0 = (up ? nz1 : nz0) >> sh; fz0 = (up ? fz1 : fz0) >> sh;
    }
    uint32_t m = 0;
#pragma unroll
    for (int c = 0; c < PER; ++c) {
        const int k = c & 3;
        const bool up = c >= 4;
        const float tnx = __builtin_fmaf(ax, byte_to_float(up ? nx1 : nx0, k), nbx), tfx = __builtin_fmaf(ax, byte_to_float(up ? fx1 : fx0, k), bx);
        const float tny = __builtin_fmaf(ay, byte_to_float(up ? ny1 : ny0, k), nby), tfy = __builtin_fmaf(ay, byte_to_float(up ? fy1 : fy0, k), by);
        const float tnz = __builtin_fmaf(az, byte_to_float(up ? nz1 : nz0, k), nbz), tfz = __builtin_fmaf(az, byte_to_float(up ? fz1 : fz0, k), bz);
        const float t_in = __builtin_fmaxf(__builtin_fmaxf(tnx, tny), __builtin_fmaxf(tnz, t_min));
        const float t_out = __builtin_fminf(__builtin_fminf(tfx, tfy), __builtin_fminf(tfz, t_best));
        m |= !(t_in > t_out) ? (1u << c) : 0u;
        if ((c + 1) % PT_BOX_SCHED == 0) __builtin_amdgcn_sched_barrier(0);
    }
    if constexpr (PER < 8) m <<= sub * PER;
    return m;
}

__device__ __forceinline__ unsigned long long brute_force_key(const RenderArgs &a, const Ray &q, float eps) {
    unsigned long long best = ~0ull;
    for (int i = 0; i < a.n_tri; ++i) {
        uint32_t orig;
        const float nd = exact_inside(a.exact + i, q, eps, orig);
        if (nd >= eps && nd < __builtin_inff()) {
            const unsigned long long k = (static_cast<unsigned long long>(ordered_bits(nd)) << 32) | static_cast<uint32_t>(i);
            best = k < best ? k : best;
        }
    }
    return best;
}

#define PT_SLOT_ON(k) ((k) == 0 || k1_on)
template <bool ENV, bool EMIS, bool DYN = false, class Lds, class Stats>
__device__ __forceinline__ void closest_hit(const RenderArgs &a, Lds &lds, const Ray (&q)[Lds::kRays], const bool (&live)[Lds::kRays],
                                            const bool (&in_envelope)[Lds::kRays], int lane, float eps, float (&best)[Lds::kRays],
                                            int (&hit)[Lds::kRays], const ExactRec *(&hit_rec)[Lds::kRays], Stats &st, bool emis_flag = false,
                                            bool two = true) {
    constexpr int R = Lds::kRays;
    const bool emis_only = EMIS && emis_flag;
    const bool k1_on = !DYN || two;
    bool valid[R];
#pragma unroll
    for (int k = 0; k < R; ++k) valid[k] = live[k] && in_envelope[k];
    auto any_ray = [&](const bool (&b)[R]) {
        bool x = b[0];
#pragma unroll
        for (int k = 1; k < R; ++k) x = x || b[k];
        return __any(x);
    };
    constexpr uint32_t kNodeStack = Lds::kNodeStack, kPairQueue = Lds::kPairQueue;
    constexpr bool kPackSlot = !Lds::kPrefilter;
    static_assert(kSmallSceneMaxTriangles < 32768, "packed (original index, slot) key: 16 bits each, slots padded to at most twice the triangles");
    ++st.w_segments;
    PT_STAMP(st, 0);
#pragma unroll
    for (int k = 0; k < R; ++k) {
        if (!PT_SLOT_ON(k)) continue;
        const int id = lane + 64 * k;
        lds.best[id] = ~0ull;
        lds.ray[0][id] = q[k].ox; lds.ray[1][id] = q[k].oy; lds.ray[2][id] = q[k].oz;
        lds.ray[3][id] = q[k].dx; lds.ray[4][id] = q[k].dy; lds.ray[5][id] = q[k].dz;
        if constexpr (Lds::kPrefilter) {
            lds.rinv.v[0][id] = __builtin_amdgcn_rcpf(q[k].dx); lds.rinv.v[1][id] = __builtin_amdgcn_rcpf(q[k].dy); lds.rinv.v[2][id] = __builtin_amdgcn_rcpf(q[k].dz);
        }
    }
    uint32_t n_pairs = 0;
    wave_sync();

    uint32_t n_filtered = 0;
    auto exact_round = [&](uint32_t e, bool active, uint32_t cnt) {
        ++st.w_exact_iters;
        st.n_exact += cnt;
        if (active) {
            const uint32_t src = (e >> 24) & Lds::kSrcMask, tri = e & 0xFFFFFFu;
            Ray r;
            r.ox = lds.ray[0][src]; r.oy = lds.ray[1][src]; r.oz = lds.ray[2][src];
            r.dx = lds.ray[3][src]; r.dy = lds.ray[4][src]; r.dz = lds.ray[5][src];
            uint32_t orig;
            const float nd = exact_inside(a.exact_slot + tri, r, eps, orig);
            if (nd >= eps && nd < __builtin_inff())
                atomicMin(&lds.best[src], (static_cast<unsigned long long>(ordered_bits(nd)) << 32) | (kPackSlot ? (orig << 16) | tri : orig));
        }
    };
    auto drain_pairs = [&](uint32_t keep_below) {
        while (n_pairs > keep_below) {
            const uint32_t cnt = min(64u, n_pairs);
            n_pairs -= cnt;
            const bool active = static_cast<uint32_t>(lane) < cnt;
            const uint32_t e = active ? lds.pairs[n_pairs + lane] : 0u;
            if constexpr (!Lds::kPrefilter) {
                exact_round(e, active, cnt);
            } else {
                bool keep = false;
                if (active) {
                    const uint32_t src = (e >> 24) & Lds::kSrcMask, tri = e & 0xFFFFFFu;
                    Ray r;
                    r.ox = lds.ray[0][src]; r.oy = lds.ray[1][src]; r.oz = lds.ray[2][src];
                    r.dx = lds.ray[3][src]; r.dy = lds.ray[4][src]; r.dz = lds.ray[5][src];
                    const float4 *rp = reinterpret_cast<const float4 *>(a.bary_all + tri);
                    const float4 c0 = rp[0], c1 = rp[1], c2 = rp[2];
                    CullRec rec;
                    rec.n[0] = c0.x; rec.n[1] = c0.y; rec.n[2] = c0.z; rec.w = c0.w;
                    rec.au[0] = c1.x; rec.au[1] = c1.y; rec.au[2] = c1.z; rec.cu = c1.w;
                    rec.av[0] = c2.x; rec.av[1] = c2.y; rec.av[2] = c2.z; rec.cv = c2.w;
                    keep = !cull_reject(rec, r, a.k1, a.k2, a.a_max_all, a.m0_all, a.t_guard_all) || (e >> 31) != 0u;
                }
                const unsigned long long ball = __ballot(keep);
                if (keep) lds.filtered[n_filtered + lanes_below(ball)] = e;
                n_filtered += __builtin_popcountll(ball);
                wave_sync();
                if (n_filtered >= static_cast<uint32_t>(PT_BIG_EXACT_AT)) {
                    const uint32_t take = min(64u, n_filtered);
                    n_filtered -= take;
                    const bool on = static_cast<uint32_t>(lane) < take;
                    exact_round(on ? lds.filtered[n_filtered + lane] : 0u, on, take);
                    wave_sync();
                }
            }
            wave_sync();
        }
    };
    auto emit_lane_pairs = [&](const uint32_t (&bits)[R], uint32_t tri0, uint32_t flag, uint32_t excl, uint32_t total) {
        uint32_t pos = n_pairs + excl;
#pragma unroll
        for (int k = 0; k < R; ++k) {
            if (!PT_SLOT_ON(k)) continue;
            emit_bits(lds.pairs, pos, bits[k], tri0 | ((static_cast<uint32_t>(lane + 64 * k) | flag) << 24));
            pos += __builtin_popcount(bits[k]);
        }
        n_pairs += total;
        wave_sync();
    };
    auto emit_pairs = [&](uint32_t bits, uint32_t tri0, uint32_t src, uint32_t excl, uint32_t total) {
        emit_bits(lds.pairs, n_pairs + excl, bits, tri0 | (src << 24));
        n_pairs += total;
        wave_sync();
    };
    auto push_pairs_any = [&](const uint32_t (&bits)[R], uint32_t tri0, uint32_t flag) {
        uint32_t cnt = 0;
#pragma unroll
        for (int k = 0; k < R; ++k)
            if (PT_SLOT_ON(k)) cnt += __builtin_popcount(bits[k]);
        const uint32_t incl = wave_scan_inclusive(cnt), total = wave_last(incl);
        if (total == 0) return;
        if (n_pairs + total > kPairQueue) drain_pairs(0);
        if (total <= kPairQueue) {
            emit_lane_pairs(bits, tri0, flag, incl - cnt, total);
            return;
        }
        constexpr uint32_t kSlice = 2u / R;
        for (uint32_t lo = 0; lo < 32u; lo += kSlice) {
            uint32_t part[R], pc2 = 0;
            bool some = false;
#pragma unroll
            for (int k = 0; k < R; ++k) {
                part[k] = PT_SLOT_ON(k) ? bits[k] & (((1u << kSlice) - 1u) << lo) : 0u;
                pc2 += __builtin_popcount(part[k]);
                some = some || part[k] != 0;
            }
            if (!__any(some)) continue;
            if (n_pairs + 128u > kPairQueue) drain_pairs(0);
            const uint32_t in2 = wave_scan_inclusive(pc2);
            emit_lane_pairs(part, tri0, flag, in2 - pc2, wave_last(in2));
        }
    };

    uint32_t pend[R], pend_tri0 = 0;
#pragma unroll
    for (int k = 0; k < R; ++k) pend[k] = 0;
    bool pend_open = false;
    auto flush_pending = [&]() {
        if (pend_open) push_pairs_any(pend, pend_tri0, 0u);
#pragma unroll
        for (int k = 0; k < R; ++k) pend[k] = 0;
        pend_open = false;
    };
    auto add_pending = [&](const uint32_t (&bits)[R], uint32_t tri0, uint32_t width) {
        if (pend_open && tri0 >= pend_tri0 && tri0 + width <= pend_tri0 + 32u) {
#pragma unroll
            for (int k = 0; k < R; ++k)
                if (PT_SLOT_ON(k)) pend[k] |= bits[k] << (tri0 - pend_tri0);
        } else {
            flush_pending();
#pragma unroll
            for (int k = 0; k < R; ++k) pend[k] = PT_SLOT_ON(k) ? bits[k] : 0u;
            pend_tri0 = tri0;
            pend_open = true;
        }
    };

    if constexpr (ENV) {
        bool far[R];
#pragma unroll
        for (int k = 0; k < R; ++k) far[k] = live[k] && !in_envelope[k];
        if (__builtin_expect(any_ray(far), 0)) {
            for (uint32_t base = 0; base < a.n_slots; base += 32u) {
                const uint32_t left = a.n_slots - base;
                const uint32_t all = left >= 32u ? 0xFFFFFFFFu : ((1u << left) - 1u);
                uint32_t bits[R];
#pragma unroll
                for (int k = 0; k < R; ++k) bits[k] = far[k] ? all : 0u;
                push_pairs_any(bits, base, Lds::kPrefilter ? kUnfiltered : 0u);
            }
        }
    }

    const ConstF clusters = (ConstF)reinterpret_cast<uintptr_t>(a.clusters);
    const ConstF spheres = (ConstF)reinterpret_cast<uintptr_t>(a.spheres);
    const ConstF bary = (ConstF)reinterpret_cast<uintptr_t>(a.bary);
    constexpr int kDescWords = sizeof(ClusterDesc) / 4;
    for (int cl = 0; cl < a.n_clusters; ++cl) {
        const ConstF cp = clusters + kDescWords * cl;
        if (emis_only && cl < 32 && !((a.emis_clusters >> cl) & 1u)) continue;
        const uint32_t first_tri = ((ConstU)cp)[4], n_tri = ((ConstU)cp)[5], kind = ((ConstU)cp)[6], off = ((ConstU)cp)[7];
        constexpr bool kSphereTrees = !Lds::kPrefilter;
        if (!kSphereTrees && kind == 0) continue;
        bool pc[R];
#pragma unroll
        for (int k = 0; k < R; ++k) {
            pc[k] = false;
            if (PT_SLOT_ON(k)) pc[k] = (kSphereTrees && kind == 0) ? valid[k] & sphere_keep(cp[0], cp[1], cp[2], cp[3], q[k]) : valid[k];
        }
        if (!any_ray(pc)) continue;
        if (kSphereTrees && kind == 0) {
            const uint32_t n_levels = ((ConstU)cp)[8];
            const uint32_t top = n_levels - 1;
            if (lane < static_cast<int>(n_levels)) {
                lds.level_off[lane] = lane == 0 ? 0u : a.clusters[cl].level_off[lane - 1];
                lds.level_cnt[lane] = (n_tri + (1u << (3 * lane)) - 1u) >> (3 * lane);
            }
            wave_sync();
            uint32_t n_nodes = 0;
            uint32_t tmask[R];
#pragma unroll
            for (int k = 0; k < R; ++k) tmask[k] = 0;
            auto any_tmask = [&]() {
                uint32_t x = tmask[0];
#pragma unroll
                for (int k = 1; k < R; ++k) x |= tmask[k];
                return __any(x != 0);
            };
            auto push_top = [&](uint32_t top) {
#pragma unroll
                for (int k = 0; k < R; ++k) {
                    if (!PT_SLOT_ON(k)) continue;
                    while (__any(tmask[k] != 0)) {
                        const bool has = tmask[k] != 0;
                        const unsigned long long ball = __ballot(has);
                        if (n_nodes + __builtin_popcountll(ball) > kNodeStack) return;
                        if (has) {
                            const uint32_t j = __builtin_ctz(tmask[k]);
                            tmask[k] &= tmask[k] - 1;
                            lds.nodes[n_nodes + lanes_below(ball)] = (static_cast<uint32_t>(lane + 64 * k) << Lds::kNodeSrcShift) | (top << Lds::kNodeLevShift) | j;
                        }
                        n_nodes += __builtin_popcountll(ball);
                    }
                }
            };
            bool rooted = false;
            if (top >= 1) {
                unsigned long long pcb[R];
                uint32_t rcnt = 0;
#pragma unroll
                for (int k = 0; k < R; ++k) {
                    pcb[k] = 0;
                    if (!PT_SLOT_ON(k)) continue;
                    pcb[k] = __ballot(pc[k]);
                    rcnt += __builtin_popcountll(pcb[k]);
                }
                const uint32_t clev = top - 1;
                const uint32_t nchild = (n_tri + (1u << (3 * clev)) - 1u) >> (3 * clev);
                const uint32_t sh = rcnt <= 1u ? 6u : rcnt <= 2u ? 5u : rcnt <= 4u ? 4u : rcnt <= 8u ? 3u : rcnt <= 16u ? 2u : 0u;
                const uint32_t per = (nchild + (1u << sh) - 1u) >> sh;
                if (rcnt <= 16u && per <= 8u) {
                    ++st.w_node_rounds;
                    {
                        uint32_t at = 0;
#pragma unroll
                        for (int k = 0; k < R; ++k) {
                            if (!PT_SLOT_ON(k)) continue;
                            if (pc[k]) lds.nodes[at + lanes_below(pcb[k])] = static_cast<uint32_t>(lane + 64 * k);
                            at += __builtin_popcountll(pcb[k]);
                        }
                    }
                    wave_sync();
                    const uint32_t item = static_cast<uint32_t>(lane) >> sh, sub = static_cast<uint32_t>(lane) & ((1u << sh) - 1u);
                    const uint32_t c0 = clev == 0 ? sub * per : sub, cstep = clev == 0 ? 1u : (1u << sh);
                    uint32_t m = 0, src = 0;
                    if (item < rcnt) {
                        src = lds.nodes[item];
                        Ray r;
                        r.ox = lds.ray[0][src]; r.oy = lds.ray[1][src]; r.oz = lds.ray[2][src];
                        r.dx = lds.ray[3][src]; r.dy = lds.ray[4][src]; r.dz = lds.ray[5][src];
                        const float4 *cs = reinterpret_cast<const float4 *>(a.spheres) + off + lds.level_off[clev] + c0;
                        auto test = [&](auto per_c) {
                            constexpr uint32_t kPer = decltype(per_c)::value;
#pragma unroll
                            for (uint32_t i = 0; i < kPer; ++i) {
                                const float4 sp = cs[i * cstep];
                                m |= sphere_keep(sp.x, sp.y, sp.z, sp.w, r) ? (1u << i) : 0u;
                            }
                            const uint32_t left = nchild > c0 ? nchild - c0 : 0u;
                            const uint32_t n_ok = min((left + cstep - 1u) >> (clev == 0 ? 0u : sh), kPer);
                            m &= (1u << n_ok) - 1u;
                        };
                        if (per == 1u) test(std::integral_constant<uint32_t, 1>());
                        else if (per == 2u) test(std::integral_constant<uint32_t, 2>());
                        else if (per <= 4u) test(std::integral_constant<uint32_t, 4>());
                        else test(std::integral_constant<uint32_t, 8>());
                    }
                    wave_sync();
                    const uint32_t mc = __builtin_popcount(m);
                    const uint32_t incl = wave_scan_inclusive(mc), tot = wave_last(incl);
                    if (clev == 0) {
                        if (n_pairs + tot > kPairQueue) drain_pairs(0);
                        if (tot <= kPairQueue) {
                            emit_pairs(m, first_tri + c0, src, incl - mc, tot);
                            rooted = true;
                        }
                    } else if (tot <= kNodeStack) {
                        emit_bits(lds.nodes, n_nodes + incl - mc, m, (src << Lds::kNodeSrcShift) | (clev << Lds::kNodeLevShift) | c0, sh);
                        n_nodes += tot;
                        wave_sync();
                        rooted = true;
                    }
                }
            }
            if (!rooted) {
            const uint32_t top_off = top == 0 ? 0u : ((ConstU)cp)[8 + top];
            const uint32_t top_cnt = (n_tri + (1u << (3 * top)) - 1u) >> (3 * top);
            const ConstF tp = spheres + 4 * (static_cast<size_t>(off) + top_off);
            for (uint32_t j = 0; j < top_cnt; ++j) {
                const float sx = tp[4 * j], sy = tp[4 * j + 1], sz = tp[4 * j + 2], sr = tp[4 * j + 3];
#pragma unroll
                for (int k = 0; k < R; ++k)
                    if (PT_SLOT_ON(k)) tmask[k] |= sphere_keep(sx, sy, sz, sr, q[k]) ? (1u << j) : 0u;
            }
#pragma unroll
            for (int k = 0; k < R; ++k) tmask[k] = pc[k] ? tmask[k] : 0u;
            PT_STAMP(st, 1);
            if (top == 0) {
                add_pending(tmask, first_tri, n_tri);
#pragma unroll
                for (int k = 0; k < R; ++k) tmask[k] = 0;
            } else {
                push_top(top);
                wave_sync();
            }
            }
            while (n_nodes > 0 || any_tmask()) {
                if (n_nodes == 0) {
                    push_top(top);
                    wave_sync();
                }
                ++st.w_node_rounds;
                const uint32_t cnt = min(64u, n_nodes);
                uint32_t shift = cnt <= 8u ? 3u : cnt <= 16u ? 2u : cnt <= 32u ? 1u : 0u;
                uint32_t m8, src, level, child0, keep, packed, incl, tot;
                bool leaf;
                for (;;) {
                    m8 = 0; src = 0; level = 1; child0 = 0;
                    const uint32_t item = static_cast<uint32_t>(lane) >> shift, sub = static_cast<uint32_t>(lane) & ((1u << shift) - 1u);
                    if (item < cnt) {
                        const uint32_t e = lds.nodes[n_nodes - 1 - item];
                        src = e >> Lds::kNodeSrcShift;
                        level = (e >> Lds::kNodeLevShift) & 7u;
                        child0 = (e & ((1u << Lds::kNodeLevShift) - 1u)) * kFan;
                        Ray r;
                        r.ox = lds.ray[0][src]; r.oy = lds.ray[1][src]; r.oz = lds.ray[2][src];
                        r.dx = lds.ray[3][src]; r.dy = lds.ray[4][src]; r.dz = lds.ray[5][src];
                        const float4 *cs = reinterpret_cast<const float4 *>(a.spheres) + off + lds.level_off[level - 1] + child0;
                        auto test = [&](auto per_c) {
                            constexpr int per = decltype(per_c)::value;
#pragma unroll
                            for (int i = 0; i < per; ++i) {
                                const uint32_t c = sub + (static_cast<uint32_t>(i) << shift);
                                const float4 sp = cs[c];
                                m8 |= sphere_keep(sp.x, sp.y, sp.z, sp.w, r) ? (1u << c) : 0u;
                            }
                        };
                        if (shift == 0u) test(std::integral_constant<int, 8>());
                        else if (shift == 1u) test(std::integral_constant<int, 4>());
                        else if (shift == 2u) test(std::integral_constant<int, 2>());
                        else test(std::integral_constant<int, 1>());
                        const uint32_t real = lds.level_cnt[level - 1];
                        const uint32_t left = real > child0 ? real - child0 : 0u;
                        m8 &= left >= 8u ? 0xFFu : ((1u << left) - 1u);
                    }
                    leaf = level == 1;
                    uint32_t kids = __builtin_popcount(m8);
                    keep = cnt;
                    packed = leaf ? kids << 16 : kids;
                    incl = wave_scan_inclusive(packed);
                    tot = wave_last(incl);
                    if (n_pairs + (tot >> 16) > kPairQueue) drain_pairs(0);
                    if (n_pairs + (tot >> 16) <= kPairQueue && n_nodes - cnt + (tot & 0xFFFFu) <= kNodeStack) break;
                    if (shift != 0u) { shift = 0u; continue; }
                    const bool fits = static_cast<uint32_t>(lane) < cnt && n_pairs + (incl >> 16) <= kPairQueue &&
                                      (n_nodes - (lane + 1)) + (incl & 0xFFFFu) <= kNodeStack;
                    const unsigned long long fb = __ballot(fits);
                    keep = (fb == ~0ull) ? 64u : static_cast<uint32_t>(__builtin_ctzll(~fb));
                    if (keep == 0) keep = 1;
                    ++st.w_partial;
                    if (static_cast<uint32_t>(lane) >= keep) m8 = 0;
                    kids = __builtin_popcount(m8);
                    packed = leaf ? kids << 16 : kids;
                    incl = wave_scan_inclusive(packed);
                    tot = wave_last(incl);
                    break;
                }
                n_nodes -= keep;
                wave_sync();
                {
                    const uint32_t excl = incl - packed;
                    emit_bits(leaf ? lds.pairs : lds.nodes, leaf ? n_pairs + (excl >> 16) : n_nodes + (excl & 0xFFFFu), m8,
                              leaf ? ((first_tri + child0) | (src << 24)) : ((src << Lds::kNodeSrcShift) | ((level - 1) << Lds::kNodeLevShift) | child0));
                    n_nodes += tot & 0xFFFFu;
                    n_pairs += tot >> 16;
                }
                wave_sync();
            }
            PT_STAMP(st, 2);
        } else {
            float k1 = a.k1, k2 = a.k2, a_max = a.a_max, m0 = a.m0, m0q = a.m0_quad, t_guard = a.t_guard;
            asm volatile("" : "+v"(k1), "+v"(k2), "+v"(a_max), "+v"(m0), "+v"(m0q), "+v"(t_guard));
            const int n_words = static_cast<int>((n_tri + kChunk - 1) / kChunk);
            for (int w = 0; w < n_words; ++w) {
                const uint32_t left = n_tri - kChunk * w;
                const ConstF bp = bary + 12 * (static_cast<size_t>(off) + kChunk * w);
                const uint32_t quads = w < kMaxLevels - 1 ? ((ConstU)cp)[9 + w] : 0u;
                uint32_t m[R];
#pragma unroll
                for (int k = 0; k < R; ++k) m[k] = 0;
                const uint32_t cnt32 = min(left, 32u);
                const uint32_t pair_bits = 0x55555555u & (cnt32 >= 32u ? 0xFFFFFFFFu : ((1u << cnt32) - 1u));
                auto quad = [&](uint32_t k0) {
                    const CullRec rec = load_cull(bp + 12 * k0);
#pragma unroll
                    for (int k = 0; k < R; ++k)
                        if (PT_SLOT_ON(k)) m[k] |= (~cull_reject_quad(rec, q[k], k1, k2, a_max, m0q, t_guard) & 3u) << k0;
                };
                auto single = [&](uint32_t slot) {
                    const CullRec rec = load_cull(bp + 12 * slot);
#pragma unroll
                    for (int k = 0; k < R; ++k)
                        if (PT_SLOT_ON(k)) m[k] |= cull_reject(rec, q[k], k1, k2, a_max, m0, t_guard) ? 0u : (1u << slot);
                };
                if (emis_only && n_words == 1) {
                    for (uint32_t rest = (a.emis_large_w0 | (a.emis_large_w0 >> 1)) & pair_bits; rest != 0; rest &= rest - 1) {
                        const uint32_t k0 = __builtin_ctz(rest);
                        if ((quads >> k0) & 1u) {
                            quad(k0);
                        } else {
                            single(k0);
                            single(k0 + 1);
                        }
                    }
#pragma unroll
                    for (int k = 0; k < R; ++k) m[k] &= a.emis_large_w0;
                } else
                if (quads == pair_bits) {
                    constexpr int kWallGroup = Lds::kPrefilter ? 2 : 1;
                    if constexpr (kWallGroup > 1) {
                        for (uint32_t k0 = 0; k0 < cnt32; k0 += 2 * kWallGroup) {
                            CullRec r[kWallGroup];
#pragma unroll
                            for (int g = 0; g < kWallGroup; ++g) r[g] = load_cull(bp + 12 * (k0 + 2 * g));
                            __builtin_amdgcn_sched_barrier(0);
#pragma unroll
                            for (int g = 0; g < kWallGroup; ++g) {
                                if (k0 + 2 * g < cnt32) {
#pragma unroll
                                    for (int k = 0; k < R; ++k) m[k] |= (~cull_reject_quad(r[g], q[k], k1, k2, a_max, m0q, t_guard) & 3u) << (k0 + 2 * g);
                                }
                            }
                        }
                    } else {
                        for (uint32_t k0 = 0; k0 < cnt32; k0 += 2) quad(k0);
                    }
                } else
                for (uint32_t k0 = 0; k0 < cnt32; k0 += 2) {
                    if ((quads >> k0) & 1u) {
                        quad(k0);
                    } else {
                        single(k0);
                        single(k0 + 1);
                    }
                }
#pragma unroll
                for (int k = 0; k < R; ++k) {
                    m[k] = pc[k] ? m[k] : 0u;
                    m[k] &= left >= 32u ? 0xFFFFFFFFu : ((1u << left) - 1u);
                }
                PT_STAMP(st, 3);
                add_pending(m, first_tri + kChunk * w, min(left, 32u));
                PT_STAMP(st, 4);
            }
        }
    }
    PT_STAMP(st, 1);
    if constexpr (Lds::kPrefilter) {
        if (a.n_bvh > 0 && !(emis_only && a.emis_bvh == 0u)) {
            flush_pending();
            drain_pairs(0);
            if (n_filtered > 0) {
                const bool active = static_cast<uint32_t>(lane) < n_filtered;
                exact_round(active ? lds.filtered[lane] : 0u, active, n_filtered);
                n_filtered = 0;
                wave_sync();
            }
            uint32_t n_nodes;
            {
                n_nodes = 0;
#pragma unroll
                for (int k = 0; k < R; ++k) {
                    const unsigned long long vb = __ballot(valid[k]);
                    if (valid[k]) lds.nodes[n_nodes + lanes_below(vb)] = static_cast<uint32_t>(lane + 64 * k) << Lds::kNodeSrcShift;
                    n_nodes += __builtin_popcountll(vb);
                }
                wave_sync();
            }
            while (n_nodes > 0) {
                ++st.w_node_rounds;
                const uint32_t cnt = min(64u, n_nodes);
                uint32_t shift = 0u;
                uint32_t m8, src, base, kids, keep, packed, incl, tot;
                bool leaf;
                for (;;) {
                m8 = 0; src = 0; base = 0;
                leaf = false;
                const uint32_t item = static_cast<uint32_t>(lane) >> shift, sub = static_cast<uint32_t>(lane) & ((1u << shift) - 1u);
                if (item < cnt) {
                    const uint32_t e = lds.nodes[n_nodes - 1 - item];
                    src = e >> Lds::kNodeSrcShift;
                    const uint32_t node = e & ((1u << Lds::kNodeSrcShift) - 1u);
                    Ray r;
                    r.ox = lds.ray[0][src]; r.oy = lds.ray[1][src]; r.oz = lds.ray[2][src];
                    r.dx = lds.ray[3][src]; r.dy = lds.ray[4][src]; r.dz = lds.ray[5][src];
                    const uint32_t bh = reinterpret_cast<const uint32_t *>(&lds.best[src])[1];
                    const float t_best = bh == 0xFFFFFFFFu ? __builtin_inff() : from_ordered_bits(bh);
                    const uint4 *np = reinterpret_cast<const uint4 *>(a.bvh + node);
                    const uint4 q0 = np[0], q1 = np[1], q2 = np[2], q3 = np[3];
                    const float ix = lds.rinv.v[0][src], iy = lds.rinv.v[1][src], iz = lds.rinv.v[2][src];
                    if (shift == 0u) m8 = box_children_kept<8>(q0, q1, q2, q3, r, ix, iy, iz, t_best, a.bvh_err);
                    else if (shift == 1u) m8 = box_children_kept<4>(q0, q1, q2, q3, r, ix, iy, iz, t_best, a.bvh_err, sub);
                    else if (shift == 2u) m8 = box_children_kept<2>(q0, q1, q2, q3, r, ix, iy, iz, t_best, a.bvh_err, sub);
                    else m8 = box_children_kept<1>(q0, q1, q2, q3, r, ix, iy, iz, t_best, a.bvh_err, sub);
                    m8 &= (2u << ((q0.w >> 8) & 7u)) - 1u;
                    leaf = ((q0.w >> 11) & 1u) != 0u;
                    base = leaf ? (q0.w >> 12) * kFan : (q0.w >> 12);
                }
                kids = __builtin_popcount(m8);
                keep = cnt;
                packed = leaf ? kids << 16 : kids;
                incl = wave_scan_inclusive(packed);
                tot = wave_last(incl);
                if (n_pairs + (tot >> 16) > kPairQueue) drain_pairs(0);
                if (n_pairs + (tot >> 16) <= kPairQueue && n_nodes - cnt + (tot & 0xFFFFu) <= kNodeStack) break;
                if (shift != 0u) { shift = 0u; continue; }
                {
                    const bool fits = static_cast<uint32_t>(lane) < cnt && n_pairs + (incl >> 16) <= kPairQueue &&
                                      (n_nodes - (lane + 1)) + (incl & 0xFFFFu) <= kNodeStack;
                    const unsigned long long fb = __ballot(fits);
                    keep = (fb == ~0ull) ? 64u : static_cast<uint32_t>(__builtin_ctzll(~fb));
                    if (keep == 0) keep = 1;
                    ++st.w_partial;
                    if (static_cast<uint32_t>(lane) >= keep) m8 = 0;
                    kids = __builtin_popcount(m8);
                    packed = leaf ? kids << 16 : kids;
                    incl = wave_scan_inclusive(packed);
                    tot = wave_last(incl);
                }
                break;
                }
                n_nodes -= keep;
// ... 128 lines not shown
        return *reinterpret_cast<const TexBary *const __attribute__((address_space(4))) *>(p + (offsetof(RenderArgs, tex_bary) - offsetof(RenderArgs, tex_recs)));
    }
    __device__ __forceinline__ const TexTexel *texels() const {
        return *reinterpret_cast<const TexTexel *const __attribute__((address_space(4))) *>(p + (offsetof(RenderArgs, tex_texels) - offsetof(RenderArgs, tex_recs)));
    }
};
__device__ __forceinline__ TextureView texture_view() {
    uint64_t p = reinterpret_cast<uint64_t>(__builtin_amdgcn_kernarg_segment_ptr()) + offsetof(RenderArgs, tex_recs);
    asm volatile("" : "+s"(p));
    return {p};
}
__device__ __forceinline__ const SmoothCorner *smooth_view() {
    uint64_t p = reinterpret_cast<uint64_t>(__builtin_amdgcn_kernarg_segment_ptr()) + offsetof(RenderArgs, smooth_normals);
    asm volatile("" : "+s"(p));
    return *reinterpret_cast<const SmoothCorner *const __attribute__((address_space(4))) *>(p);
}
__device__ __forceinline__ const float *rough_view() {
    uint64_t p = reinterpret_cast<uint64_t>(__builtin_amdgcn_kernarg_segment_ptr()) + offsetof(RenderArgs, rough_alpha);
    asm volatile("" : "+s"(p));
    return *reinterpret_cast<const float *const __attribute__((address_space(4))) *>(p);
}
struct DirectView {
    uint64_t p;
    __device__ __forceinline__ const LightRec *lights() const { return *reinterpret_cast<const LightRec *const __attribute__((address_space(4))) *>(p); }
    __device__ __forceinline__ int32_t n() const {
        return *reinterpret_cast<const __attribute__((address_space(4))) int32_t *>(p + (offsetof(RenderArgs, n_lights) - offsetof(RenderArgs, lights)));
    }
    __device__ __forceinline__ float area() const {
        return *reinterpret_cast<const __attribute__((address_space(4))) float *>(p + (offsetof(RenderArgs, light_area) - offsetof(RenderArgs, lights)));
    }
};
__device__ __forceinline__ DirectView direct_view() {
    uint64_t p = reinterpret_cast<uint64_t>(__builtin_amdgcn_kernarg_segment_ptr()) + offsetof(RenderArgs, lights);
    asm volatile("" : "+s"(p));
    return {p};
}
struct EnvDirectView {
    uint64_t p;
    __device__ __forceinline__ const EnvAliasRec *table() const { return *reinterpret_cast<const EnvAliasRec *const __attribute__((address_space(4))) *>(p); }
    __device__ __forceinline__ int32_t cells() const {
        return *reinterpret_cast<const __attribute__((address_space(4))) int32_t *>(p + (offsetof(RenderArgs, env_cells) - offsetof(RenderArgs, env_alias)));
    }
    __device__ __forceinline__ float share() const {
        return *reinterpret_cast<const __attribute__((address_space(4))) float *>(p + (offsetof(RenderArgs, env_share) - offsetof(RenderArgs, env_alias)));
    }
};
__device__ __forceinline__ EnvDirectView envdirect_view() {
    uint64_t p = reinterpret_cast<uint64_t>(__builtin_amdgcn_kernarg_segment_ptr()) + offsetof(RenderArgs, env_alias);
    asm volatile("" : "+s"(p));
    return {p};
}

constexpr plan::Build kBuild = {kTileW, kTileH, PT_RAYS_PER_LANE, PT_BIG_RAYS_PER_LANE, PT_WAVES_PER_SIMD, kMaxBatchPass,
#if defined(PT_BLOCK_PROFILE)
                                plan::Stats::kAsAsked, true};
#elif defined(PT_PHASE_TIMERS) || defined(PT_VERIFY_BRUTE)
                                plan::Stats::kAlways, false};
#elif defined(PT_VERIFY_SHIPPED) || defined(PT_ADAPT_COUNT)
                                plan::Stats::kNever, false};
#else
                                plan::Stats::kAsAsked, false};
#endif

template <bool SKY, bool BIG, bool STATS>
constexpr int rays_per_lane() { return plan::rays_per_lane(kBuild, SKY, BIG, STATS); }

template <bool SKY, bool BIG, bool STATS, bool ENV, bool NARROW>
constexpr int integrator_waves() {
    return SKY ? ((BIG && STATS && ENV) ? PT_BIG_WAVES  : PT_SKY_WAVES)
               : BIG ? PT_BIG_WAVES : (STATS || (!NARROW && rays_per_lane<SKY, BIG, STATS>() > 1)) ? PT_WAVES_PER_SIMD - 1 : PT_WAVES_PER_SIMD;
}
template <bool SKY, bool BIG, bool STATS, bool ENV, bool NARROW = false, int ADAPT = 0>
__global__ __launch_bounds__(kBlock, (integrator_waves<SKY, BIG, STATS, ENV, NARROW>())) void integrate_kernel(const RenderArgs a) {
    constexpr bool LENS = false, MOTION = false, PROJ = false, ENVMAP = false, GLASS = false, TEX = false, SMOOTH = false, ROUGH = false, DIRECT = false, ENVDIRECT = false;
#include "pt_integrator_body.inc"
}
template <bool SKY, bool BIG, bool STATS, bool ENV, bool NARROW>
constexpr int lens_waves() {
    constexpr int w = integrator_waves<SKY, BIG, STATS, ENV, NARROW>();
    return (SKY && w == PT_SKY_WAVES && !(BIG && !STATS && !ENV)) ? w - 1 : w;
}
template <bool SKY, bool BIG, bool STATS, bool ENV, bool NARROW, int ADAPT>
__global__ __launch_bounds__(kBlock, (lens_waves<SKY, BIG, STATS, ENV, NARROW>())) void integrate_kernel_lens(const RenderArgs a) {
    constexpr bool LENS = true, MOTION = false, PROJ = false, ENVMAP = false, GLASS = false, TEX = false, SMOOTH = false, ROUGH = false, DIRECT = false, ENVDIRECT = false;
#include "pt_integrator_body.inc"
}
template <bool SKY, bool BIG, bool STATS, bool ENV, bool NARROW, bool LENS_>
constexpr int motion_waves() {
    constexpr int w = LENS_ ? lens_waves<SKY, BIG, STATS, ENV, NARROW>() : integrator_waves<SKY, BIG, STATS, ENV, NARROW>();
    return (LENS_ && !SKY && !BIG && !STATS && ENV && !NARROW) ? w - 1 : w;
}
template <bool SKY, bool BIG, bool STATS, bool ENV, bool NARROW, int ADAPT>
__global__ __launch_bounds__(kBlock, (motion_waves<SKY, BIG, STATS, ENV, NARROW, false>())) void integrate_kernel_motion(const RenderArgs a) {
    constexpr bool LENS = false, MOTION = true, PROJ = false, ENVMAP = false, GLASS = false, TEX = false, SMOOTH = false, ROUGH = false, DIRECT = false, ENVDIRECT = false;
#include "pt_integrator_body.inc"
}
template <bool SKY, bool BIG, bool STATS, bool ENV, bool NARROW, int ADAPT>
__global__ __launch_bounds__(kBlock, (motion_waves<SKY, BIG, STATS, ENV, NARROW, true>())) void integrate_kernel_motion_lens(const RenderArgs a) {
    constexpr bool LENS = true, MOTION = true, PROJ = false, ENVMAP = false, GLASS = false, TEX = false, SMOOTH = false, ROUGH = false, DIRECT = false, ENVDIRECT = false;
#include "pt_integrator_body.inc"
}
template <bool SKY, bool BIG, bool STATS, bool ENV, bool NARROW>
constexpr int projection_waves() {
    return integrator_waves<SKY, BIG, STATS, ENV, NARROW>();
}
template <bool SKY, bool BIG, bool STATS, bool ENV, bool NARROW, int ADAPT>
__global__ __launch_bounds__(kBlock, (projection_waves<SKY, BIG, STATS, ENV, NARROW>())) void integrate_kernel_projection(const RenderArgs a) {
    constexpr bool LENS = false, MOTION = false, PROJ = true, ENVMAP = false, GLASS = false, TEX = false, SMOOTH = false, ROUGH = false, DIRECT = false, ENVDIRECT = false;
#include "pt_integrator_body.inc"
}

template <int UNIT>
hipError_t launch_surface_unit(const RenderArgs &args, const plan::Variant &v, hipStream_t stream);
#define PT_UNIT_HALF(U) template <> hipError_t launch_surface_unit<U>(const RenderArgs &, const plan::Variant &, hipStream_t);
PT_UNIT_HALF(kGlassUnit) PT_UNIT_HALF(kTextureUnit) PT_UNIT_HALF(kSmoothUnit) PT_UNIT_HALF(kRoughUnit) PT_UNIT_HALF(kDirectUnit) PT_UNIT_HALF(kEnvDirectUnit)
#undef PT_UNIT_HALF

#ifdef PT_ENVIRONMENT_UNIT
template <bool BIG, bool STATS, bool ENV, int VIEW>
constexpr int environment_waves() {
    constexpr bool kLens = VIEW == 2 || VIEW == 4;
    if constexpr (VIEW == 5) return projection_waves<true, BIG, STATS, ENV, false>();
    else if constexpr (VIEW >= 3) return motion_waves<true, BIG, STATS, ENV, false, kLens>();
    else if constexpr (VIEW == 2) return lens_waves<true, BIG, STATS, ENV, false>();
    else return integrator_waves<true, BIG, STATS, ENV, false>();
}
template <bool BIG, bool STATS, bool ENV, int VIEW>
__global__ __launch_bounds__(kBlock, (environment_waves<BIG, STATS, ENV, VIEW>())) void integrate_kernel_environment(const RenderArgs a) {
    constexpr bool SKY = true, NARROW = false;
    constexpr int ADAPT = VIEW != 0 ? 1 : 0;
    constexpr bool LENS = VIEW == 2 || VIEW == 4, MOTION = VIEW == 3 || VIEW == 4, PROJ = VIEW == 5, ENVMAP = true, GLASS = false, TEX = false, SMOOTH = false, ROUGH = false, DIRECT = false, ENVDIRECT = false;
#include "pt_integrator_body.inc"
}
namespace {
using Kernel = void (*)(const RenderArgs);
constexpr int kEnvironmentViews = plan::kViews + 1;
template <int I>
Kernel environment_kernel_of() {
    return &integrate_kernel_environment<(I & 4) != 0, (I & 2) != 0, (I & 1) != 0, I / 8>;
}
template <int... I>
std::array<Kernel, sizeof...(I)> environment_kernel_table(std::integer_sequence<int, I...>) { return {environment_kernel_of<I>()...}; }
const auto kEnvironmentKernels = environment_kernel_table(std::make_integer_sequence<int, 8 * kEnvironmentViews>());
}
hipError_t launch_environment_integrator(const RenderArgs &args, const plan::Variant &v, hipStream_t stream) {
    if (!v.sky || v.narrow || v.pool || args.env_map == nullptr || args.env_n < kEnvMinSize || args.env_n > kEnvMaxSize || args.sky != nullptr)
        return hipErrorInvalidValue;
    if (args.projection != 0 && v.view != 1) return hipErrorInvalidDeviceFunction;
    const int view = args.projection != 0 ? 5 : v.view;
    const Kernel kernel = kEnvironmentKernels[view * 8 + (v.big ? 4 : 0) + (v.stats ? 2 : 0) + (v.env ? 1 : 0)];
    hipLaunchKernelGGL(kernel, dim3(args.n_tiles * args.n_chunks), dim3(kBlock), 0, stream, args);
    return hipGetLastError();
}
#elif defined(PT_SURFACE_UNIT)
#define PT_UNIT_NAME_1 glass
#define PT_UNIT_NAME_2 texture
#define PT_UNIT_NAME_3 smooth
#define PT_UNIT_NAME_4 rough
#define PT_UNIT_NAME_5 direct
#define PT_UNIT_NAME_6 envdirect
#define PT_PASTE_(a, b) a##b
#define PT_PASTE(a, b) PT_PASTE_(a, b)
#define PT_UNIT_KERNEL PT_PASTE(integrate_kernel_, PT_PASTE(PT_UNIT_NAME_, PT_SURFACE_UNIT))
static_assert(PT_SURFACE_UNIT >= kGlassUnit && PT_SURFACE_UNIT <= kEnvDirectUnit, "PT_SURFACE_UNIT: a SurfaceUnit");
constexpr bool kUnitTex = PT_SURFACE_UNIT >= kTextureUnit, kUnitSmooth = PT_SURFACE_UNIT >= kSmoothUnit, kUnitRough = PT_SURFACE_UNIT >= kRoughUnit,
               kUnitDirect = PT_SURFACE_UNIT >= kDirectUnit, kUnitEnvDirect = PT_SURFACE_UNIT >= kEnvDirectUnit;
template <bool SKY, bool BIG, bool STATS, bool ENV, bool NARROW, int VIEW>
constexpr int view_waves() {
    constexpr bool kLens = VIEW == 2 || VIEW == 4;
    if constexpr (VIEW == 5) return projection_waves<SKY, BIG, STATS, ENV, NARROW>();
    else if constexpr (VIEW >= 3) return motion_waves<SKY, BIG, STATS, ENV, NARROW, kLens>();
    else if constexpr (VIEW == 2) return lens_waves<SKY, BIG, STATS, ENV, NARROW>();
    else return integrator_waves<SKY, BIG, STATS, ENV, NARROW>();
}
template <int MISS, bool BIG, bool STATS, int FORM, int VIEW>
constexpr int glass_fewer_waves() {
    if constexpr (MISS == 1 && !(BIG && STATS)) return (VIEW == 0 || VIEW == 1 || VIEW == 3 || VIEW == 5) ? 1 : 0;
    else if constexpr (MISS == 0 && !BIG && !STATS && FORM == 0) return (VIEW == 2 || VIEW == 3 || VIEW == 5) ? 1 : 0;
    else return 0;
}
template <int MISS, bool BIG, bool STATS, int FORM, int VIEW>
constexpr int texture_fewer_waves() {
    return (MISS == 0 && !BIG && !STATS && FORM == 0 && (VIEW == 0 || VIEW == 1)) ? 1 : 0;
}
template <int MISS, bool BIG, bool STATS, int FORM, int VIEW>
constexpr int smooth_fewer_waves() {
    return 0;
}
template <int MISS, bool BIG, bool STATS, int FORM, int VIEW>
constexpr int rough_fewer_waves() {
    return (MISS == 0 && !BIG && !STATS && FORM == 2 && (VIEW == 0 || VIEW == 4 || VIEW == 5)) ? 1 : 0;
}
template <int MISS, bool BIG, bool STATS, int FORM, int VIEW>
constexpr int rough_unit_waves() {
    return view_waves<MISS != 0, BIG, STATS, FORM < 2, FORM == 1, VIEW>() - glass_fewer_waves<MISS, BIG, STATS, FORM, VIEW>() -
           texture_fewer_waves<MISS, BIG, STATS, FORM, VIEW>() - smooth_fewer_waves<MISS, BIG, STATS, FORM, VIEW>() -
           rough_fewer_waves<MISS, BIG, STATS, FORM, VIEW>();
}
template <int MISS, bool BIG, bool STATS, int FORM, int VIEW>
constexpr int direct_fewer_waves() {
    constexpr int twin = rough_unit_waves<MISS, BIG, STATS, FORM, VIEW>();
    return twin > 4 ? twin - 4 : 0;
}
template <int MISS, bool BIG, bool STATS, int FORM, int VIEW>
constexpr int envdirect_fewer_waves() {
    return 0;
}
template <int MISS, bool BIG, bool STATS, int FORM, int VIEW>
constexpr int unit_waves() {
    return view_waves<MISS != 0, BIG, STATS, FORM < 2, FORM == 1, VIEW>() - glass_fewer_waves<MISS, BIG, STATS, FORM, VIEW>() -
           (kUnitTex ? texture_fewer_waves<MISS, BIG, STATS, FORM, VIEW>() : 0) - (kUnitSmooth ? smooth_fewer_waves<MISS, BIG, STATS, FORM, VIEW>() : 0) -
           (kUnitRough ? rough_fewer_waves<MISS, BIG, STATS, FORM, VIEW>() : 0) - (kUnitDirect ? direct_fewer_waves<MISS, BIG, STATS, FORM, VIEW>() : 0) -
           (kUnitEnvDirect ? envdirect_fewer_waves<MISS, BIG, STATS, FORM, VIEW>() : 0);
}
template <int MISS, bool BIG, bool STATS, int FORM, int VIEW>
__global__ __launch_bounds__(kBlock, (unit_waves<MISS, BIG, STATS, FORM, VIEW>()))
void PT_UNIT_KERNEL(const RenderArgs a) {
    constexpr bool SKY = MISS != 0, ENV = FORM < 2, NARROW = FORM == 1;
    constexpr int ADAPT = (FORM == 2 ? 2 : FORM == 3 ? 4 : 0) | (VIEW != 0 ? 1 : 0);
    constexpr bool LENS = VIEW == 2 || VIEW == 4, MOTION = VIEW == 3 || VIEW == 4, PROJ = VIEW == 5, ENVMAP = MISS == 2, GLASS = true, TEX = kUnitTex, SMOOTH = kUnitSmooth, ROUGH = kUnitRough, DIRECT = kUnitDirect, ENVDIRECT = kUnitEnvDirect;
#include "pt_integrator_body.inc"
}
namespace {
using Kernel = void (*)(const RenderArgs);
constexpr int kGlassViews = plan::kViews + 1, kGlassPerView = 3 * 2 * 2 * 4;
template <int MISS, bool BIG, bool STATS, int FORM>
constexpr bool glass_kernel_exists() {
    if constexpr (kUnitEnvDirect) return MISS == 2 && FORM == 0;
    else if constexpr (FORM == 0) return true;
    else if constexpr (MISS != 0 || STATS) return false;
    else return plan::variant_exists({false, BIG, false, FORM == 1, FORM == 1, FORM == 2 ? 2 : FORM == 3 ? 4 : 0, 1}, kBuild);
}
template <int I>
Kernel glass_kernel_of() {
    constexpr int kMiss = (I / 16) % 3, kForm = I & 3;
    constexpr bool kBig = (I & 8) != 0, kStats = (I & 4) != 0;
    if constexpr (!glass_kernel_exists<kMiss, kBig, kStats, kForm>()) return nullptr;
    else return &PT_UNIT_KERNEL<kMiss, kBig, kStats, kForm, I / 48>;
}
template <int... I>
std::array<Kernel, sizeof...(I)> glass_kernel_table(std::integer_sequence<int, I...>) { return {glass_kernel_of<I>()...}; }
const auto kGlassKernels = glass_kernel_table(std::make_integer_sequence<int, kGlassPerView * kGlassViews>());
}
template <>
hipError_t launch_surface_unit<PT_SURFACE_UNIT>(const RenderArgs &args, const plan::Variant &v, hipStream_t stream) {
    if (surface_unit_of(args) != PT_SURFACE_UNIT || (kUnitDirect && (kUnitEnvDirect ? args.n_lights < 0 : args.n_lights <= 0))) return hipErrorInvalidValue;
    if (kUnitEnvDirect && (args.env_map == nullptr || args.env_cells < 1 || args.env_cells > kEnvSampleMaxCells || args.env_cells > args.env_n ||
                           !(args.env_share > 0.0f && args.env_share <= 1.0f) || (args.n_lights == 0 && args.env_share != 1.0f) || args.lights == nullptr))
        return hipErrorInvalidValue;
    if ((kUnitRough && args.rough_alpha == nullptr) || (kUnitSmooth && args.smooth_normals == nullptr)) return hipErrorInvalidValue;
    if (kUnitTex && (args.tex_recs == nullptr || args.tex_uv == nullptr || args.tex_texels == nullptr || args.tex_bary == nullptr)) return hipErrorInvalidValue;
    if (args.glass == nullptr || (args.env_map != nullptr && (!v.sky || args.sky != nullptr))) return hipErrorInvalidValue;
    if (args.projection != 0 && v.view != 1) return hipErrorInvalidDeviceFunction;
    const int view = args.projection != 0 ? 5 : v.view;
    const int miss = args.env_map != nullptr ? 2 : v.sky ? 1 : 0, form = v.narrow ? 1 : v.pool == 2 ? 2 : v.pool == 4 ? 3 : 0;
    const Kernel kernel = kGlassKernels[(view * 3 + miss) * 16 + (v.big ? 8 : 0) + (v.stats ? 4 : 0) + form];
    if (!kernel) return hipErrorInvalidDeviceFunction;
    hipLaunchKernelGGL(kernel, dim3(args.n_tiles * args.n_chunks), dim3(kBlock), 0, stream, args);
    return hipGetLastError();
}
#undef PT_UNIT_KERNEL
#else
__global__ __launch_bounds__(256) void projection_rays_kernel(const RenderArgs a, int width, int height, int row_begin, int n,
                                                              float *__restrict__ origins, float *__restrict__ directions) {
    const int p = blockIdx.x * 256 + threadIdx.x;
    if (p >= n) return;
    const int y = row_begin + p / width, x = p % width;
    const float u = static_cast<float>(static_cast<double>(x) / width - 0.5);
    const float v = static_cast<float>(-static_cast<double>(y) / height + 0.5);
    float ox, oy, oz, dx, dy, dz;
    projection_primary_ray(a.projection, u, v, a.cam, a.lns + 2, a.prj_span,
                           [](float ang, float &sn, float &cs) { portable_sincos(ang, sn, cs); },
                           [](float &vx, float &vy, float &vz) { normalize3(vx, vy, vz); }, ox, oy, oz, dx, dy, dz);
    const size_t o = 3 * static_cast<size_t>(p);
    origins[o] = ox; origins[o + 1] = oy; origins[o + 2] = oz;
    directions[o] = dx; directions[o + 1] = dy; directions[o + 2] = dz;
}
hipError_t launch_projection_rays(const RenderArgs &args, int width, int height, int row_begin, int rows, float *d_origins, float *d_directions,
                                  hipStream_t stream) {
    const int n = rows * width;
    if (n <= 0) return hipSuccess;
    if (args.projection == 0) return hipErrorInvalidValue;
    hipLaunchKernelGGL(projection_rays_kernel, dim3((n + 255) / 256), dim3(256), 0, stream, args, width, height, row_begin, n, d_origins, d_directions);
    return hipGetLastError();
}

template <bool BIG>
__global__ __launch_bounds__(kBlock, BIG ? PT_BIG_WAVES : PT_WAVES_PER_SIMD) void trace_rays_kernel(const RenderArgs a, const float *__restrict__ origins,
                                                                              const float *__restrict__ directions, int n_rays,
                                                                              int32_t *__restrict__ hit_index, float *__restrict__ hit_t) {
    __shared__ WaveLds<std::conditional_t<BIG, BigQueues, SmallQueues>, 1> lds;
    const int lane = threadIdx.x;
    const int i = blockIdx.x * kBlock + lane;
    const bool valid = i < n_rays;
    Ray q;
    q.ox = q.oy = q.oz = 0.0f; q.dx = q.dy = 0.0f; q.dz = 1.0f;
    if (valid) {
        q.ox = origins[3 * i]; q.oy = origins[3 * i + 1]; q.oz = origins[3 * i + 2];
        q.dx = directions[3 * i]; q.dy = directions[3 * i + 1]; q.dz = directions[3 * i + 2];
    }
    const float d2 = (q.dx * q.dx + q.dy * q.dy) + q.dz * q.dz;
    const bool inside = __builtin_fabsf(q.ox) <= a.r_org && __builtin_fabsf(q.oy) <= a.r_org && __builtin_fabsf(q.oz) <= a.r_org &&
                        __builtin_fabsf(d2 - 1.0f) <= 1.0e-5f;
    float best[1];
    int hit[1];
    const ExactRec *hit_rec[1];
    WaveStats st;
    const Ray qs[1] = {q};
    const bool lives[1] = {valid}, insides[1] = {inside};
    closest_hit<true, false>(a, lds, qs, lives, insides, lane, a.eps, best, hit, hit_rec, st);
    if (valid) {
        hit_index[i] = hit[0];
        hit_t[i] = best[0];
    }
}

__global__ __launch_bounds__(kBlock) void box_masks_kernel(const BvhNode *__restrict__ nodes, const float *__restrict__ rays,
                                                           const float *__restrict__ t_best, float err, int n, uint32_t *__restrict__ out) {
    const int i = blockIdx.x * kBlock + threadIdx.x;
    if (i >= n) return;
    const uint4 *np = reinterpret_cast<const uint4 *>(nodes + i);
    const uint4 q0 = np[0], q1 = np[1], q2 = np[2], q3 = np[3];
    Ray r;
    r.ox = rays[6 * i]; r.oy = rays[6 * i + 1]; r.oz = rays[6 * i + 2];
    r.dx = rays[6 * i + 3]; r.dy = rays[6 * i + 4]; r.dz = rays[6 * i + 5];
    const float ix = __builtin_amdgcn_rcpf(r.dx), iy = __builtin_amdgcn_rcpf(r.dy), iz = __builtin_amdgcn_rcpf(r.dz);
    const uint32_t exists = (2u << ((q0.w >> 8) & 7u)) - 1u;
    out[i] = box_children_kept<8>(q0, q1, q2, q3, r, ix, iy, iz, t_best[i], err) & exists;
}
hipError_t launch_box_masks(const BvhNode *d_nodes, const float *d_rays, const float *d_t_best, float err, int n, uint32_t *d_out, hipStream_t stream) {
    if (n <= 0) return hipSuccess;
    hipLaunchKernelGGL(box_masks_kernel, dim3((n + kBlock - 1) / kBlock), dim3(kBlock), 0, stream, d_nodes, d_rays, d_t_best, err, n, d_out);
    return hipGetLastError();
}

hipError_t launch_trace_rays(const RenderArgs &args, const float *d_origins, const float *d_directions, int n_rays,
                             int32_t *d_hit_index, float *d_hit_t, hipStream_t stream) {
    if (n_rays <= 0) return hipSuccess;
    const unsigned grid = static_cast<unsigned>((n_rays + kBlock - 1) / kBlock);
    if ((args.big != 0))
        hipLaunchKernelGGL(trace_rays_kernel<true>, dim3(grid), dim3(kBlock), 0, stream, args, d_origins, d_directions, n_rays, d_hit_index, d_hit_t);
    else
        hipLaunchKernelGGL(trace_rays_kernel<false>, dim3(grid), dim3(kBlock), 0, stream, args, d_origins, d_directions, n_rays, d_hit_index, d_hit_t);
    return hipGetLastError();
}

#ifdef PT_BLOCK_PROFILE
#define PT_INST(S, B) \
    template __global__ void integrate_kernel<S, B, false, false, false>(const RenderArgs); \
    template __global__ void integrate_kernel<S, B, true, false, false>(const RenderArgs);  \
    template __global__ void integrate_kernel<S, B, false, true, false>(const RenderArgs);  \
    template __global__ void integrate_kernel<S, B, true, true, false>(const RenderArgs);
PT_INST(false, false) PT_INST(false, true) PT_INST(true, false) PT_INST(true, true)
#undef PT_INST
}
#include <cstdio>
#include <cstdlib>
#include <string>
#include <vector>
namespace pt {
hipError_t launch_integrator(const RenderArgs &args0, const plan::Variant &v, hipStream_t stream) {
    constexpr size_t kCounters = 4096;
    static hipModule_t mod = nullptr;
    static uint32_t *d_cnt = nullptr;
    const int rows = args0.row_end - args0.row_begin;
    if (rows <= 0 || args0.width <= 0) return hipSuccess;
    if (!plan::variant_exists(v, kBuild) || args0.projection != 0 || args0.env_map != nullptr || surface_unit_of(args0) != kNoSurfaceUnit) return hipErrorNotSupported;
    if (!mod) {
        const char *path = std::getenv("PT_BLOCKPROF_HSACO");
        if (!path) return hipErrorInvalidValue;
        hipError_t e = hipModuleLoad(&mod, path);
        if (e != hipSuccess) return e;
        e = hipMalloc(reinterpret_cast<void **>(&d_cnt), kCounters * sizeof(uint32_t));
        if (e != hipSuccess) return e;
    }
    hipError_t e = hipMemsetAsync(d_cnt, 0, kCounters * sizeof(uint32_t), stream);
    if (e != hipSuccess) return e;
    RenderArgs args = args0;
    args.blockprof = d_cnt;
    char name[128];
    std::snprintf(name, sizeof name, "_ZN2pt16integrate_kernelILb%dELb%dELb%dELb%dELb%dELi%dEEEvNS_10RenderArgsE", v.sky, v.big, v.stats, v.env, v.narrow,
                  v.pool | v.view);
    hipFunction_t f;
    e = hipModuleGetFunction(&f, mod, name);
    if (e != hipSuccess) return e;
    size_t size = sizeof args;
    void *config[] = {HIP_LAUNCH_PARAM_BUFFER_POINTER, &args, HIP_LAUNCH_PARAM_BUFFER_SIZE, &size, HIP_LAUNCH_PARAM_END};
    e = hipModuleLaunchKernel(f, args.n_tiles * args.n_chunks, 1, 1, kBlock, 1, 1, 0, stream, nullptr, config);
    if (e != hipSuccess) return e;
    e = hipStreamSynchronize(stream);
    if (e != hipSuccess) return e;
    std::vector<uint32_t> h(kCounters);
    e = hipMemcpy(h.data(), d_cnt, kCounters * sizeof(uint32_t), hipMemcpyDeviceToHost);
    if (e != hipSuccess) return e;
    if (const char *out = std::getenv("PT_BLOCKPROF_OUT")) {
        if (FILE *fp = std::fopen((std::string(out) + "." + name + ".txt").c_str(), "w")) {
            for (size_t i = 0; i < kCounters; ++i) if (h[i]) std::fprintf(fp, "%zu %u\n", i, h[i]);
            std::fclose(fp);
        }
    }
    return hipSuccess;
}
hipError_t integrator_waves_per_cu(const plan::Variant &, int *waves) {
    *waves = 24;
    return hipSuccess;
}
#else
namespace {
using Kernel = void (*)(const RenderArgs);
template <int I>
Kernel kernel_of() {
    constexpr plan::Variant v = plan::variant_of(I);
    if constexpr (!plan::variant_exists(v, kBuild)) return nullptr;
    else if constexpr (plan::view_has_motion(v.view) && plan::view_has_lens(v.view)) return &integrate_kernel_motion_lens<v.sky, v.big, v.stats, v.env, v.narrow, v.pool | 1>;
    else if constexpr (plan::view_has_motion(v.view)) return &integrate_kernel_motion<v.sky, v.big, v.stats, v.env, v.narrow, v.pool | 1>;
    else if constexpr (plan::view_has_lens(v.view)) return &integrate_kernel_lens<v.sky, v.big, v.stats, v.env, v.narrow, v.pool | 1>;
    else return &integrate_kernel<v.sky, v.big, v.stats, v.env, v.narrow, v.pool | v.view>;
}
template <int... I>
std::array<Kernel, sizeof...(I)> kernel_table(std::integer_sequence<int, I...>) { return {kernel_of<I>()...}; }
const auto kKernels = kernel_table(std::make_integer_sequence<int, plan::kAllVariants>());
static_assert(plan::variant_id({true, true, true, true, false, 0, plan::kViews - 1}) < plan::kAllVariants, "every view's ids fit the table");
template <int R>
Kernel projection_kernel_of() {
    constexpr plan::Variant v = plan::variant_of(plan::kVariantsPerView + R);
    if constexpr (!plan::variant_exists(v, kBuild)) return nullptr;
    else return &integrate_kernel_projection<v.sky, v.big, v.stats, v.env, v.narrow, v.pool | 1>;
}
template <int... R>
std::array<Kernel, sizeof...(R)> projection_kernel_table(std::integer_sequence<int, R...>) { return {projection_kernel_of<R>()...}; }
const auto kProjectionKernels = projection_kernel_table(std::make_integer_sequence<int, plan::kVariantsPerView>());
Kernel kernel_for(const plan::Variant &v, bool projection) {
    if (!projection) return kKernels[plan::variant_id(v)];
    return v.view == 1 ? kProjectionKernels[plan::variant_id(v) - plan::kVariantsPerView] : nullptr;
}
}

hipError_t launch_integrator(const RenderArgs &args, const plan::Variant &v, hipStream_t stream) {
    const int rows = args.row_end - args.row_begin;
    if (rows <= 0 || args.width <= 0) return hipSuccess;
    if (const int unit = surface_unit_of(args)) return launch_surface_integrator(unit, args, v, stream);
    if (args.env_map != nullptr) return launch_environment_integrator(args, v, stream);
    const Kernel kernel = kernel_for(v, args.projection != 0);
    if (!kernel) return hipErrorInvalidDeviceFunction;
    hipLaunchKernelGGL(kernel, dim3(args.n_tiles * args.n_chunks), dim3(kBlock), 0, stream, args);
    return hipGetLastError();
}

hipError_t integrator_waves_per_cu(const plan::Variant &v, int *waves) {
    constexpr int kDevices = 16;
    static std::atomic<int> cache[kDevices][plan::kAllVariants];
    const Kernel kernel = kKernels[plan::variant_id(v)];
    if (!kernel) return hipErrorInvalidDeviceFunction;
    int dev = 0;
    hipError_t e = hipGetDevice(&dev);
    if (e != hipSuccess) return e;
    std::atomic<int> *cached = dev < kDevices ? &cache[dev][plan::variant_id(v)] : nullptr;
    int n = cached ? cached->load(std::memory_order_relaxed) : 0;
    if (n == 0) {
        e = hipOccupancyMaxActiveBlocksPerMultiprocessor(&n, kernel, kBlock, 0);
        if (e == hipSuccess && n > 0) {
            hipFuncAttributes fa;
            hipDeviceProp_t prop;
            if (hipFuncGetAttributes(&fa, reinterpret_cast<const void *>(kernel)) == hipSuccess && fa.sharedSizeBytes > 0 &&
                hipGetDeviceProperties(&prop, dev) == hipSuccess && prop.maxSharedMemoryPerMultiProcessor > 0) {
                constexpr size_t kLdsGranule = 1280;
                const size_t per_wave = (fa.sharedSizeBytes + kLdsGranule - 1) / kLdsGranule * kLdsGranule;
                const size_t by_lds = std::max<size_t>(prop.maxSharedMemoryPerMultiProcessor, prop.sharedMemPerBlock) / per_wave;
                if (by_lds >= 1 && by_lds < static_cast<size_t>(n)) n = static_cast<int>(by_lds);
            }
        }
        if (e != hipSuccess || n <= 0) n = 0;
        else if (cached) cached->store(n, std::memory_order_relaxed);
    }
    if (n > 0) *waves = n;
    return e;
}
#endif

hipError_t launch_surface_integrator(int unit, const RenderArgs &args, const plan::Variant &v, hipStream_t stream) {
#if defined(PT_PHASE_TIMERS) || defined(PT_BLOCK_PROFILE)
    return hipErrorNotSupported;
#else
    constexpr decltype(&launch_surface_unit<kGlassUnit>) kLaunch[] = {&launch_surface_unit<kGlassUnit>, &launch_surface_unit<kTextureUnit>, &launch_surface_unit<kSmoothUnit>,
                                                                      &launch_surface_unit<kRoughUnit>, &launch_surface_unit<kDirectUnit>, &launch_surface_unit<kEnvDirectUnit>};
    return unit >= kGlassUnit && unit <= kEnvDirectUnit ? kLaunch[unit - kGlassUnit](args, v, stream) : hipErrorInvalidValue;
#endif
}

const plan::Build &integrator_build() { return kBuild; }
#endif

}
```

path-tracing_amd/csrc/pt_kernels.hpp:

```cpp
#pragma once
#include <hip/hip_runtime_api.h>

#include <cstdint>

#include "pt_launch_plan.hpp"
#include "pt_scene.hpp"

namespace pt {

constexpr uint32_t kPhiloxKey1 = 0x50544831u;
constexpr uint32_t regen_min_dead_for(int mrr) { return mrr >= 5 ? 4u : 64u; }

struct GlassRec {
    float ior, inv_ior, pad0, pad1;
    float tint[3], pad2;
};

struct RenderArgs {
    const ClusterDesc *clusters;
    const SphereRec *spheres;
    const CullRec *bary;
    const CullRec *bary_all;
    float a_max_all, m0_all, t_guard_all;
    const ExactRec *exact;
    const ExactRec *exact_slot;
    const BvhNode *bvh;
    uint32_t n_bvh;
    float bvh_err;
    const MatRec *mats;
    int32_t n_mats;
    const uint8_t *sky;
    int32_t sky_w, sky_h;
    float *sum, *sum2;
    int32_t *count;
    unsigned long long *stats;
    int32_t n_clusters, n_tri;
    int32_t big;
    uint32_t n_slots;
    int32_t width, height, row_begin, row_end;
    int32_t row_stride;
    int32_t band_rows;
    int32_t pass_begin, pass_count, mrr;
    float eps, error;
    uint32_t seed;
    float k1, k2, a_max, m0, m0_quad, t_guard;
    int32_t blocks_x;
    int32_t narrow;
    int32_t adapt_pool;
    uint32_t *sched;
    uint32_t n_tiles, n_chunks;
    int32_t chunk_passes;
    int32_t vec_ok;
    float r_org;
    int32_t may_leave_envelope;
    uint32_t regen_min_dead;
    uint32_t last_segment_filter;
    uint32_t emis_clusters, emis_large_w0, emis_bvh;
    int32_t camera;
    float cam[12];
    int32_t lens;
    float lns[11];
    int32_t motion;
    float cam_d[12];
    float lns_d[9];
    int32_t projection;
    float prj_span[2];
    const void *env_map;
    int32_t env_n;
    const void *glass;
    const void *tex_recs;
    const float *tex_uv;
    const void *tex_texels;
    const void *tex_bary;
    const void *smooth_normals;
    const float *rough_alpha;
    const void *lights;
    int32_t n_lights;
    float light_area;
    const void *env_alias;
    int32_t env_cells;
    float env_share;
#ifdef PT_BLOCK_PROFILE
    uint32_t *blockprof;
#endif
};

const plan::Build &integrator_build();
enum SurfaceUnit : int { kNoSurfaceUnit = 0, kGlassUnit, kTextureUnit, kSmoothUnit, kRoughUnit, kDirectUnit, kEnvDirectUnit };
inline int surface_unit_of(const RenderArgs &a) {
    return a.env_alias ? kEnvDirectUnit : a.lights ? kDirectUnit : a.rough_alpha ? kRoughUnit : a.smooth_normals ? kSmoothUnit : a.tex_recs ? kTextureUnit : a.glass ? kGlassUnit : kNoSurfaceUnit;
}
hipError_t launch_integrator(const RenderArgs &args, const plan::Variant &v, hipStream_t stream);
hipError_t launch_environment_integrator(const RenderArgs &args, const plan::Variant &v, hipStream_t stream);
hipError_t launch_surface_integrator(int unit, const RenderArgs &args, const plan::Variant &v, hipStream_t stream);
hipError_t integrator_waves_per_cu(const plan::Variant &v, int *waves);
hipError_t launch_projection_rays(const RenderArgs &args, int width, int height, int row_begin, int rows, float *d_origins, float *d_directions,
                                  hipStream_t stream);
hipError_t launch_box_masks(const BvhNode *d_nodes, const float *d_rays, const float *d_t_best, float err, int n, uint32_t *d_out, hipStream_t stream);
hipError_t launch_trace_rays(const RenderArgs &args, const float *d_origins, const float *d_directions, int n_rays,
                             int32_t *d_hit_index, float *d_hit_t, hipStream_t stream);

}
```

path-tracing_amd/csrc/pt_launch_plan.hpp:

```cpp
#pragma once
#include <algorithm>
#include <cstdint>

namespace pt::plan {

enum class Stats { kAsAsked, kAlways, kNever };

struct Build {
    int tile_w, tile_h;
    int rays_small, rays_big;
    int waves_per_simd;
    int max_batch_pass;
    Stats stats;
    bool wide_only;
};

struct Variant {
    bool sky, big, stats, env, narrow;
    int pool, view;
};
constexpr bool operator==(const Variant &a, const Variant &b) {
    return a.sky == b.sky && a.big == b.big && a.stats == b.stats && a.env == b.env && a.narrow == b.narrow && a.pool == b.pool && a.view == b.view;
}

constexpr int rays_per_lane(const Build &b, bool sky, bool big, bool stats) { return (!sky && !stats) ? (big ? b.rays_big : b.rays_small) : 1; }

constexpr int kVariantsPerView = 24, kViews = 5, kAllVariants = kViews * kVariantsPerView;
constexpr int kStillVariants = 3 * kVariantsPerView, kVariants = kStillVariants;
constexpr int view_of(bool camera, bool lens, bool motion) { return motion ? (lens ? 4 : 3) : lens ? 2 : camera ? 1 : 0; }
constexpr bool view_has_lens(int view) { return view == 2 || view == 4; }
constexpr bool view_has_motion(int view) { return view == 3 || view == 4; }
constexpr int variant_id(const Variant &v) {
    return kVariantsPerView * v.view + (v.narrow ? 16 + 2 * v.big + v.env : v.pool ? 20 + 2 * v.big + (v.pool == 4) : ((v.sky * 2 + v.big) * 2 + v.stats) * 2 + v.env);
}
constexpr Variant variant_of(int id) {
    const int view = id / kVariantsPerView, r = id % kVariantsPerView;
    if (r < 16) return {(r & 8) != 0, (r & 4) != 0, (r & 2) != 0, (r & 1) != 0, false, 0, view};
    if (r < 20) return {false, (r & 2) != 0, false, (r & 1) != 0, true, 0, view};
    return {false, (r & 2) != 0, false, false, false, (r & 1) ? 4 : 2, view};
}
constexpr bool variant_exists(const Variant &v, const Build &b) {
    if (b.wide_only && (v.narrow || v.pool || v.view != 0)) return false;
    if (!v.narrow && !v.pool) return true;
    if (v.sky || v.stats || (v.pool && v.env)) return false;
    return (v.pool && v.big) || rays_per_lane(b, false, v.big, false) > 1;
}

struct Overrides {
    int tile_width = 0;
    int items_per_slot = 0;
    int chunk_min = 0;
    int regen_min_dead = 0;
};

struct Launch {
    int width, band_rows;
    bool sky, big, want_stats, may_leave_envelope;
    float error;
    int pass_begin, pass_count;
    int view;
    int cu_count;
};

struct Tiles {
    Variant variant;
    int narrow, adapt_pool, blocks_x;
    uint32_t n_tiles;
};

inline Tiles plan_tiles(const Launch &l, const Build &b, const Overrides &o = {}) {
    const int force = o.tile_width;
    const bool stats = b.stats == Stats::kAlways || (b.stats == Stats::kAsAsked && l.want_stats);
    const uint32_t rows = static_cast<uint32_t>((l.band_rows + b.tile_h - 1) / b.tile_h);
    const auto tiles_of = [&](int px) { return static_cast<uint32_t>((l.width + b.tile_w * px - 1) / (b.tile_w * px)) * rows; };
    const auto rounds = [&](int waves, uint32_t num, uint32_t den) { return static_cast<uint32_t>(l.cu_count) * 4u * static_cast<uint32_t>(waves) * num / den; };
    int rays = rays_per_lane(b, l.sky, l.big, stats);
    const bool batches = !b.wide_only && !l.sky && !stats && l.error >= 0.0f && !l.may_leave_envelope && l.pass_begin >= 0 &&
                         l.pass_begin + l.pass_count <= b.max_batch_pass && (l.big ? rays == 1 && force != 1 : rays > 1);
    Tiles t = {{l.sky, l.big, stats, l.may_leave_envelope, false, 0, l.view}, 0, 0, 0, 0};
    if (rays > 1 && !b.wide_only) {
        uint32_t min_tiles = rounds(b.waves_per_simd - 1, 3u, 2u), min_wide = batches ? rounds(b.waves_per_simd - 1, 6u, 5u) : min_tiles;
        if (force == 1) min_tiles = min_wide = 0xFFFFFFFFu;
        if (force == 2 || force == 3) min_tiles = min_wide = 0;
        if (tiles_of(rays) < min_wide) {
            rays = 1;
            t.narrow = 1;
        } else if (batches) {
            t.adapt_pool = (force != 2 && tiles_of(4) >= min_tiles) ? 4 : 2;
        }
    } else if (batches) {
        const uint32_t min_tiles = (force == 2 || force == 3) ? 0u : rounds(b.waves_per_simd, 3u, 2u);
        if (force != 2 && tiles_of(4) >= min_tiles) t.adapt_pool = 4;
        else if (tiles_of(2) >= min_tiles) t.adapt_pool = 2;
    }
    t.variant.narrow = t.narrow != 0;
    t.variant.pool = t.adapt_pool;
    const int tile_px = t.adapt_pool ? t.adapt_pool : rays;
    t.blocks_x = (l.width + b.tile_w * tile_px - 1) / (b.tile_w * tile_px);
    t.n_tiles = static_cast<uint32_t>(t.blocks_x) * rows;
    return t;
}

struct Chunks {
    uint32_t n_chunks;
    int32_t chunk_passes;
};

inline Chunks plan_chunks(uint32_t n_tiles, uint32_t slots, int32_t pass_count, bool sky, bool narrow, bool want_stats, const Overrides &o = {}) {
    uint32_t n_chunks = 1;
    int32_t chunk_passes = 0;
    const int chunk_min = o.chunk_min > 0 ? o.chunk_min : (want_stats || sky) ? 8 : narrow ? 2 : 1;
    if (n_tiles >= slots / 2u)
        while (n_chunks < 6u && (pass_count >> (2u * n_chunks)) >= chunk_min) ++n_chunks;
    int items_per_slot = 0;
    const unsigned long long t100 = 100ull * n_tiles;
    if (sky) {
        if (t100 >= 75ull * slots && t100 < 190ull * slots) items_per_slot = 8;
    } else if (t100 >= 75ull * slots && t100 < 230ull * slots) {
        items_per_slot = t100 < 120ull * slots ? 8 : t100 < 190ull * slots ? 16 : 32;
    }
    if (o.items_per_slot != 0) items_per_slot = std::max(0, o.items_per_slot);
    if (items_per_slot > 0) {
        n_chunks = (static_cast<uint32_t>(items_per_slot) * slots + n_tiles - 1u) / n_tiles;
        n_chunks = std::max(1u, std::min(n_chunks, static_cast<uint32_t>(std::max(1, pass_count / 4))));
        chunk_passes = std::max(1, (pass_count + static_cast<int32_t>(n_chunks) - 1) / static_cast<int32_t>(n_chunks));
        n_chunks = static_cast<uint32_t>(std::max(1, (pass_count + chunk_passes - 1) / chunk_passes));
        if (n_chunks == 1u) chunk_passes = 0;
    }
    return {n_chunks, chunk_passes};
}

}
```

path-tracing_amd/csrc/pt_scene.hpp:

```cpp
#pragma once
#include <algorithm>
#include <cstdint>
#include <string>
#include <vector>

namespace pt {

struct HostScene {
    std::vector<float> tri;
    std::vector<int32_t> tri_mat;
    std::vector<float> mat;
    std::vector<float> tri_uv;
    std::vector<std::string> map_kd;
    std::vector<float> tri_vn;
    std::vector<float> mat_pr;
    int n_tri() const { return static_cast<int>(tri_mat.size()); }
    int n_mat() const { return static_cast<int>(mat.size() / 10); }
};
inline bool material_emits(const float *mat) { return mat[3] != 0.0f || mat[4] != 0.0f || mat[5] != 0.0f; }

bool load_obj(const std::string &model_dir, const std::string &model_name, HostScene &out, std::string &err, bool &io_error,
              bool geometric_planes = false);

void append_triangle(HostScene &s, const float v0[3], const float v1[3], const float v2[3], const float *vn_or_null,
                     int material, const float *toward_or_null = nullptr);

struct CullRec {
    float n[3], w;
    float au[3], cu;
    float av[3], cv;
};
struct ExactRec {
    float plane[4];
    float v0[3], square;
    float v1[3];
    int32_t material;
    float v2[3];
    int32_t orig;
};
struct MatRec {
    float kd[3], chance0;
    float ks[3], chance1;
    int32_t n_lobes, kind0, kind1, pad;
};

static const int kChunk = 32;
static const int kFan = 8;
static const int kMaxLevels = 8;
#ifndef PT_TILE_W
#define PT_TILE_W 8
#endif
static const int kTileW = PT_TILE_W, kTileH = 64 / PT_TILE_W;
static const int kMaxBvhDepth = 9;
static const int kBigSceneTriangles = 1024;
static const int kSmallSceneMaxTriangles = 16384;
static const int kMaxClusters = 8;

static const uint32_t kNoTriangle = 0xFFFFFFFFu;

struct BvhNode {
    float org[3];
    uint32_t meta;
    uint8_t lo[3][8];
    uint8_t hi[3][8];
};
static_assert(sizeof(BvhNode) == 64, "BvhNode is four 16-byte loads");

struct SphereRec {
    float c[3], r2;
};
struct ClusterDesc {
    float c[3], r2;
    uint32_t first_tri, n_tri, kind, data_off;
    uint32_t n_levels;
    uint32_t level_off[kMaxLevels - 1];
};

struct CullConstants {
    float k1, k2;
    float a_max;
    float m0;
    float m0_quad;
    float t_guard;
};

struct CullTables {
    std::vector<uint32_t> slot_tri;
    std::vector<ExactRec> exact_slot;
    std::vector<SphereRec> spheres;
    std::vector<CullRec> bary;
    std::vector<CullRec> bary_all;
    CullConstants cc_all;
    std::vector<ClusterDesc> clusters;
    std::vector<BvhNode> bvh;
    uint32_t bvh_inner = 0;
    uint32_t bvh_depth = 0;
    bool big = false;
    float bvh_err = 0;
    CullConstants cc;
    float eps = 0;
    float r_org = 0;
    double r_max = 0;
    bool may_leave_envelope = false;
    uint32_t emis_clusters = 0xFFFFFFFFu;
    uint32_t emis_large_w0 = 0xFFFFFFFFu;
    bool emis_bvh = true;
};

#ifdef PT_TEST_HOOKS
struct CullMutation {
    double sphere_r2 = 1, m0 = 1, k12 = 1, a_max = 1, quad_slack = 1, box = 1, box_err = 1;
    int no_absorb = 0;
    int emis_drop = 0;
    int no_last_segment_filter = 0;
    double bvh_fill = 0.5;
    int bvh_depth_cap = kMaxBvhDepth;
    int max_clusters = -1;
    int big_threshold = -1;
    int bvh_mode = -1;
    int order_mode = 0;
};
extern CullMutation g_cull_mutation;
#define PT_MUT(field) (::pt::g_cull_mutation.field)
#else
#define PT_MUT(field) 1.0
#endif

struct DeviceTables {
    std::vector<ExactRec> exact;
    std::vector<MatRec> mats;
};

void build_device_tables(const HostScene &s, DeviceTables &out);
void build_cull_tables(const HostScene &s, float eps, CullTables &out, double r_camera = 20.0);
double vertex_extent(const HostScene &s);
inline double cull_r_max(double vertex_extent, double r_camera) { return std::max(std::max(20.0, r_camera), vertex_extent); }

}
```

Baseline: 7292.

## Add specialized room-scene kernel variant for tiny two-cluster scenes

```diff
diff --git a/path-tracing_amd/csrc/pt_capi.cpp b/path-tracing_amd/csrc/pt_capi.cpp
--- a/path-tracing_amd/csrc/pt_capi.cpp
+++ b/path-tracing_amd/csrc/pt_capi.cpp
@@ -2,6 +2,7 @@
 #include "pt_bmp.hpp"
 
 #include <algorithm>
+#include <atomic>
 #include <chrono>
 #include <cmath>
 #include <cstdio>
@@ -12,6 +13,7 @@
 #include "pt_filters.hpp"
 
 static pt::plan::Overrides g_plan_overrides;
+static std::atomic<int> g_last_variant{-1};
 
 namespace ptc {
 
@@ -366,7 +368,8 @@
     }
     const bool sky = a.sky != nullptr || a.env_map != nullptr;
     const pt::plan::Tiles tiles = pt::plan::plan_tiles({a.width, a.band_rows, sky, a.big != 0, want_stats, a.may_leave_envelope != 0, a.error,
-                                                        a.pass_begin, a.pass_count, pt::plan::view_of(a.camera != 0, a.lens != 0, a.motion != 0), scene->cu_count},
+                                                        a.pass_begin, a.pass_count, pt::plan::view_of(a.camera != 0, a.lens != 0, a.motion != 0), scene->cu_count,
+                                                        scene->cull.host->room && a.env_map == nullptr && a.projection == 0 && pt::surface_unit_of(a) == pt::kNoSurfaceUnit},
                                                        pt::integrator_build(), ov);
     a.narrow = tiles.narrow;
     a.adapt_pool = tiles.adapt_pool;
@@ -399,6 +402,7 @@
         return fail(PT_ERR_UNSUPPORTED, std::string(w[0]) + ": this diagnostic build of the library has no " + w[1] + " kernels");
     }
     PT_HIP_TRY(launched);
+    g_last_variant.store(pt::plan::variant_id(tiles.variant), std::memory_order_relaxed);
     if (want_stats) PT_HIP_TRY(hipEventRecord(ctx.ev1.get(), stream));
     PT_HIP_TRY(hipEventRecord(ctx.ev_done.get(), stream));
     ctx.has_prev = true;
@@ -1469,6 +1473,8 @@
 
 long pt_test_live_device_objects(void) { return ptc::g_live_device_objects.load(std::memory_order_relaxed); }
 
+int pt_test_last_variant(void) { return g_last_variant.load(std::memory_order_relaxed); }
+
 int pt_test_set_mutation(const char *family, double value) {
     if (!family) return PT_ERR_INVALID_ARGUMENT;
     const std::string f = family;
@@ -1494,6 +1500,7 @@
     else if (f == "max_clusters") m.max_clusters = static_cast<int>(value);
     else if (f == "items_per_slot") g_plan_overrides.items_per_slot = static_cast<int>(value);
     else if (f == "tile_width") g_plan_overrides.tile_width = static_cast<int>(value);
+    else if (f == "no_room_kernel") g_plan_overrides.no_room_kernel = value != 0;
     else return fail(PT_ERR_INVALID_ARGUMENT, "unknown mutation family " + f);
     return PT_OK;
 }
diff --git a/path-tracing_amd/csrc/pt_cull_tables.cpp b/path-tracing_amd/csrc/pt_cull_tables.cpp
--- a/path-tracing_amd/csrc/pt_cull_tables.cpp
+++ b/path-tracing_amd/csrc/pt_cull_tables.cpp
@@ -993,6 +993,16 @@
         for (uint32_t k = 0; k < static_cast<uint32_t>(n_small_slots); ++k) out.emis_bvh = out.emis_bvh || emits(k);
 }
 
+bool room_shaped(const CullTables &t) {
+    if (t.big || !t.bvh.empty()) return false;
+    if (t.clusters.empty() || t.clusters.size() > 2) return false;
+    const ClusterDesc &large = t.clusters.back();
+    if (large.kind != 1u || large.n_tri == 0 || large.n_tri > static_cast<uint32_t>(kChunk)) return false;
+    const uint32_t pair_bits = 0x55555555u & (large.n_tri >= 32u ? 0xFFFFFFFFu : ((1u << large.n_tri) - 1u));
+    if (large.level_off[0] != pair_bits) return false;
+    return t.clusters.size() == 1 || t.clusters.front().kind == 0u;
+}
+
 }
 
 double vertex_extent(const HostScene &s) {
@@ -1047,6 +1057,7 @@
     out.cc_all.t_guard = all.t_guard;
 
     fill_emitter_masks(s, n_small_slots, out);
-}
-
-}
+    out.room = room_shaped(out);
+}
+
+}
diff --git a/path-tracing_amd/csrc/pt_integrator_body.inc b/path-tracing_amd/csrc/pt_integrator_body.inc
--- a/path-tracing_amd/csrc/pt_integrator_body.inc
+++ b/path-tracing_amd/csrc/pt_integrator_body.inc
@@ -1,5 +1,8 @@
-    constexpr int POOL = ADAPT & ~1;
+    constexpr int POOL = ADAPT & 6;
     constexpr bool CAM = (ADAPT & 1) != 0;
+    constexpr bool ROOM = (ADAPT & 8) != 0;
+    static_assert(!ROOM || (ADAPT == 8 && !SKY && !BIG && !STATS && !ENV && !LENS && !MOTION && !PROJ && !ENVMAP && !GLASS && !TEX && !SMOOTH && !ROUGH && !DIRECT && !ENVDIRECT),
+                  "the room instantiations are forms of the statistics-free plain small-scene kernel alone");
     static_assert(!LENS || CAM, "a lens kernel is the lens variant of a camera twin");
     static_assert(!DIRECT || (SMOOTH && ROUGH), "the direct term is written in the smooth scatter step: a direct kernel is a rough kernel with DIRECT");
     static_assert(!ENVDIRECT || (DIRECT && ENVMAP), "an environment-sampling kernel is a direct kernel with an environment");
@@ -528,7 +531,7 @@
             }
             for (;;) {
                 if (BIG && !any_of(searched)) break;
-                closest_hit<ENV, kLastSegmentFilter, kDynSlots>(a, lds, q, searched, inside, lane, eps, best, hit, hit_rec, wst, emis_phase, two);
+                closest_hit<ENV, kLastSegmentFilter, kDynSlots, ROOM>(a, lds, q, searched, inside, lane, eps, best, hit, hit_rec, wst, emis_phase, two);
                 if (!emis_phase) break;
                 emis_phase = false;
 #pragma unroll
diff --git a/path-tracing_amd/csrc/pt_kernels.hip b/path-tracing_amd/csrc/pt_kernels.hip
--- a/path-tracing_amd/csrc/pt_kernels.hip
+++ b/path-tracing_amd/csrc/pt_kernels.hip
@@ -451,7 +451,7 @@
 }
 
 #define PT_SLOT_ON(k) ((k) == 0 || k1_on)
-template <bool ENV, bool EMIS, bool DYN = false, class Lds, class Stats>
+template <bool ENV, bool EMIS, bool DYN = false, bool ROOM = false, class Lds, class Stats>
 __device__ __forceinline__ void closest_hit(const RenderArgs &a, Lds &lds, const Ray (&q)[Lds::kRays], const bool (&live)[Lds::kRays],
                                             const bool (&in_envelope)[Lds::kRays], int lane, float eps, float (&best)[Lds::kRays],
                                             int (&hit)[Lds::kRays], const ExactRec *(&hit_rec)[Lds::kRays], Stats &st, bool emis_flag = false,
@@ -629,6 +629,46 @@
     const ConstF spheres = (ConstF)reinterpret_cast<uintptr_t>(a.spheres);
     const ConstF bary = (ConstF)reinterpret_cast<uintptr_t>(a.bary);
     constexpr int kDescWords = sizeof(ClusterDesc) / 4;
+    if constexpr (ROOM) {
+        static_assert(EMIS && !ENV && !DYN && !Lds::kPrefilter, "the room instantiations are forms of the statistics-free plain small-scene kernel");
+        {
+            const ConstF cp = clusters + kDescWords * (a.n_clusters - 1);
+            const uint32_t first_tri = ((ConstU)cp)[4], n_tri = ((ConstU)cp)[5], off = ((ConstU)cp)[7];
+            float k1 = a.k1, k2 = a.k2, a_max = a.a_max, m0q = a.m0_quad, t_guard = a.t_guard;
+            asm volatile("" : "+v"(k1), "+v"(k2), "+v"(a_max), "+v"(m0q), "+v"(t_guard));
+            const ConstF bp = bary + 12 * static_cast<size_t>(off);
+            uint32_t m[R];
+#pragma unroll
+            for (int k = 0; k < R; ++k) m[k] = 0;
+            auto quad = [&](uint32_t k0) {
+                const CullRec rec = load_cull(bp + 12 * k0);
+#pragma unroll
+                for (int k = 0; k < R; ++k) m[k] |= (~cull_reject_quad(rec, q[k], k1, k2, a_max, m0q, t_guard) & 3u) << k0;
+            };
+            if (emis_only) {
+                for (uint32_t rest = (a.emis_large_w0 | (a.emis_large_w0 >> 1)) & 0x55555555u; rest != 0; rest &= rest - 1) quad(__builtin_ctz(rest));
+#pragma unroll
+                for (int k = 0; k < R; ++k) m[k] &= a.emis_large_w0;
+            } else {
+                for (uint32_t k0 = 0; k0 < n_tri; k0 += 2) quad(k0);
+            }
+#pragma unroll
+            for (int k = 0; k < R; ++k) m[k] = valid[k] ? m[k] : 0u;
+            add_pending(m, first_tri, n_tri);
+            flush_pending();
+        }
+        if (a.n_clusters > 1 && !(emis_only && !(a.emis_clusters & 1u))) {
+            constexpr int cl = 0;
+            const ConstF cp = clusters;
+            const uint32_t first_tri = ((ConstU)cp)[4], n_tri = ((ConstU)cp)[5], off = ((ConstU)cp)[7];
+            bool pc[R];
+#pragma unroll
+            for (int k = 0; k < R; ++k) pc[k] = valid[k] & sphere_keep(cp[0], cp[1], cp[2], cp[3], q[k]);
+            if (any_ray(pc)) {
+#include "pt_sphere_tree_walk.inc"
+            }
+        }
+    } else
     for (int cl = 0; cl < a.n_clusters; ++cl) {
         const ConstF cp = clusters + kDescWords * cl;
         if (emis_only && cl < 32 && !((a.emis_clusters >> cl) & 1u)) continue;
@@ -643,204 +683,7 @@
         }
         if (!any_ray(pc)) continue;
         if (kSphereTrees && kind == 0) {
-            const uint32_t n_levels = ((ConstU)cp)[8];
-            const uint32_t top = n_levels - 1;
-            if (lane < static_cast<int>(n_levels)) {
-                lds.level_off[lane] = lane == 0 ? 0u : a.clusters[cl].level_off[lane - 1];
-                lds.level_cnt[lane] = (n_tri + (1u << (3 * lane)) - 1u) >> (3 * lane);
-            }
-            wave_sync();
-            uint32_t n_nodes = 0;
-            uint32_t tmask[R];
-#pragma unroll
-            for (int k = 0; k < R; ++k) tmask[k] = 0;
-            auto any_tmask = [&]() {
-                uint32_t x = tmask[0];
-#pragma unroll
-                for (int k = 1; k < R; ++k) x |= tmask[k];
-                return __any(x != 0);
-            };
-            auto push_top = [&](uint32_t top) {
-#pragma unroll
-                for (int k = 0; k < R; ++k) {
-                    if (!PT_SLOT_ON(k)) continue;
-                    while (__any(tmask[k] != 0)) {
-                        const bool has = tmask[k] != 0;
-                        const unsigned long long ball = __ballot(has);
-                        if (n_nodes + __builtin_popcountll(ball) > kNodeStack) return;
-                        if (has) {
-                            const uint32_t j = __builtin_ctz(tmask[k]);
-                            tmask[k] &= tmask[k] - 1;
-                            lds.nodes[n_nodes + lanes_below(ball)] = (static_cast<uint32_t>(lane + 64 * k) << Lds::kNodeSrcShift) | (top << Lds::kNodeLevShift) | j;
-                        }
-                        n_nodes += __builtin_popcountll(ball);
-                    }
-                }
-            };
-            bool rooted = false;
-            if (top >= 1) {
-                unsigned long long pcb[R];
-                uint32_t rcnt = 0;
-#pragma unroll
-                for (int k = 0; k < R; ++k) {
-                    pcb[k] = 0;
-                    if (!PT_SLOT_ON(k)) continue;
-                    pcb[k] = __ballot(pc[k]);
-                    rcnt += __builtin_popcountll(pcb[k]);
-                }
-                const uint32_t clev = top - 1;
-                const uint32_t nchild = (n_tri + (1u << (3 * clev)) - 1u) >> (3 * clev);
-                const uint32_t sh = rcnt <= 1u ? 6u : rcnt <= 2u ? 5u : rcnt <= 4u ? 4u : rcnt <= 8u ? 3u : rcnt <= 16u ? 2u : 0u;
-                const uint32_t per = (nchild + (1u << sh) - 1u) >> sh;
-                if (rcnt <= 16u && per <= 8u) {
-                    ++st.w_node_rounds;
-                    {
-                        uint32_t at = 0;
-#pragma unroll
-                        for (int k = 0; k < R; ++k) {
-                            if (!PT_SLOT_ON(k)) continue;
-                            if (pc[k]) lds.nodes[at + lanes_below(pcb[k])] = static_cast<uint32_t>(lane + 64 * k);
-                            at += __builtin_popcountll(pcb[k]);
-                        }
-                    }
-                    wave_sync();
-                    const uint32_t item = static_cast<uint32_t>(lane) >> sh, sub = static_cast<uint32_t>(lane) & ((1u << sh) - 1u);
-                    const uint32_t c0 = clev == 0 ? sub * per : sub, cstep = clev == 0 ? 1u : (1u << sh);
-                    uint32_t m = 0, src = 0;
-                    if (item < rcnt) {
-                        src = lds.nodes[item];
-                        Ray r;
-                        r.ox = lds.ray[0][src]; r.oy = lds.ray[1][src]; r.oz = lds.ray[2][src];
-                        r.dx = lds.ray[3][src]; r.dy = lds.ray[4][src]; r.dz = lds.ray[5][src];
-                        const float4 *cs = reinterpret_cast<const float4 *>(a.spheres) + off + lds.level_off[clev] + c0;
-                        auto test = [&](auto per_c) {
-                            constexpr uint32_t kPer = decltype(per_c)::value;
-#pragma unroll
-                            for (uint32_t i = 0; i < kPer; ++i) {
-                                const float4 sp = cs[i * cstep];
-                                m |= sphere_keep(sp.x, sp.y, sp.z, sp.w, r) ? (1u << i) : 0u;
-                            }
-                            const uint32_t left = nchild > c0 ? nchild - c0 : 0u;
-                            const uint32_t n_ok = min((left + cstep - 1u) >> (clev == 0 ? 0u : sh), kPer);
-                            m &= (1u << n_ok) - 1u;
-                        };
-                        if (per == 1u) test(std::integral_constant<uint32_t, 1>());
-                        else if (per == 2u) test(std::integral_constant<uint32_t, 2>());
-                        else if (per <= 4u) test(std::integral_constant<uint32_t, 4>());
-                        else test(std::integral_constant<uint32_t, 8>());
-                    }
-                    wave_sync();
-                    const uint32_t mc = __builtin_popcount(m);
-                    const uint32_t incl = wave_scan_inclusive(mc), tot = wave_last(incl);
-                    if (clev == 0) {
-                        if (n_pairs + tot > kPairQueue) drain_pairs(0);
-                        if (tot <= kPairQueue) {
-                            emit_pairs(m, first_tri + c0, src, incl - mc, tot);
-                            rooted = true;
-                        }
-                    } else if (tot <= kNodeStack) {
-                        emit_bits(lds.nodes, n_nodes + incl - mc, m, (src << Lds::kNodeSrcShift) | (clev << Lds::kNodeLevShift) | c0, sh);
-                        n_nodes += tot;
-                        wave_sync();
-                        rooted = true;
-                    }
-                }
-            }
-            if (!rooted) {
-            const uint32_t top_off = top == 0 ? 0u : ((ConstU)cp)[8 + top];
-            const uint32_t top_cnt = (n_tri + (1u << (3 * top)) - 1u) >> (3 * top);
-            const ConstF tp = spheres + 4 * (static_cast<size_t>(off) + top_off);
-            for (uint32_t j = 0; j < top_cnt; ++j) {
-                const float sx = tp[4 * j], sy = tp[4 * j + 1], sz = tp[4 * j + 2], sr = tp[4 * j + 3];
-#pragma unroll
-                for (int k = 0; k < R; ++k)
-                    if (PT_SLOT_ON(k)) tmask[k] |= sphere_keep(sx, sy, sz, sr, q[k]) ? (1u << j) : 0u;
-            }
-#pragma unroll
-            for (int k = 0; k < R; ++k) tmask[k] = pc[k] ? tmask[k] : 0u;
-            PT_STAMP(st, 1);
-            if (top == 0) {
-                add_pending(tmask, first_tri, n_tri);
-#pragma unroll
-                for (int k = 0; k < R; ++k) tmask[k] = 0;
-            } else {
-                push_top(top);
-                wave_sync();
-            }
-            }
-            while (n_nodes > 0 || any_tmask()) {
-                if (n_nodes == 0) {
-                    push_top(top);
-                    wave_sync();
-                }
-                ++st.w_node_rounds;
-                const uint32_t cnt = min(64u, n_nodes);
-                uint32_t shift = cnt <= 8u ? 3u : cnt <= 16u ? 2u : cnt <= 32u ? 1u : 0u;
-                uint32_t m8, src, level, child0, keep, packed, incl, tot;
-                bool leaf;
-                for (;;) {
-                    m8 = 0; src = 0; level = 1; child0 = 0;
-                    const uint32_t item = static_cast<uint32_t>(lane) >> shift, sub = static_cast<uint32_t>(lane) & ((1u << shift) - 1u);
-                    if (item < cnt) {
-                        const uint32_t e = lds.nodes[n_nodes - 1 - item];
-                        src = e >> Lds::kNodeSrcShift;
-                        level = (e >> Lds::kNodeLevShift) & 7u;
-                        child0 = (e & ((1u << Lds::kNodeLevShift) - 1u)) * kFan;
-                        Ray r;
-                        r.ox = lds.ray[0][src]; r.oy = lds.ray[1][src]; r.oz = lds.ray[2][src];
-                        r.dx = lds.ray[3][src]; r.dy = lds.ray[4][src]; r.dz = lds.ray[5][src];
-                        const float4 *cs = reinterpret_cast<const float4 *>(a.spheres) + off + lds.level_off[level - 1] + child0;
-                        auto test = [&](auto per_c) {
-                            constexpr int per = decltype(per_c)::value;
-#pragma unroll
-                            for (int i = 0; i < per; ++i) {
-                                const uint32_t c = sub + (static_cast<uint32_t>(i) << shift);
-                                const float4 sp = cs[c];
-                                m8 |= sphere_keep(sp.x, sp.y, sp.z, sp.w, r) ? (1u << c) : 0u;
-                            }
-                        };
-                        if (shift == 0u) test(std::integral_constant<int, 8>());
-                        else if (shift == 1u) test(std::integral_constant<int, 4>());
-                        else if (shift == 2u) test(std::integral_constant<int, 2>());
-                        else test(std::integral_constant<int, 1>());
-                        const uint32_t real = lds.level_cnt[level - 1];
-                        const uint32_t left = real > child0 ? real - child0 : 0u;
-                        m8 &= left >= 8u ? 0xFFu : ((1u << left) - 1u);
-                    }
-                    leaf = level == 1;
-                    uint32_t kids = __builtin_popcount(m8);
-                    keep = cnt;
-                    packed = leaf ? kids << 16 : kids;
-                    incl = wave_scan_inclusive(packed);
-                    tot = wave_last(incl);
-                    if (n_pairs + (tot >> 16) > kPairQueue) drain_pairs(0);
-                    if (n_pairs + (tot >> 16) <= kPairQueue && n_nodes - cnt + (tot & 0xFFFFu) <= kNodeStack) break;
-                    if (shift != 0u) { shift = 0u; continue; }
-                    const bool fits = static_cast<uint32_t>(lane) < cnt && n_pairs + (incl >> 16) <= kPairQueue &&
-                                      (n_nodes - (lane + 1)) + (incl & 0xFFFFu) <= kNodeStack;
-                    const unsigned long long fb = __ballot(fits);
-                    keep = (fb == ~0ull) ? 64u : static_cast<uint32_t>(__builtin_ctzll(~fb));
-                    if (keep == 0) keep = 1;
-                    ++st.w_partial;
-                    if (static_cast<uint32_t>(lane) >= keep) m8 = 0;
-                    kids = __builtin_popcount(m8);
-                    packed = leaf ? kids << 16 : kids;
-                    incl = wave_scan_inclusive(packed);
-                    tot = wave_last(incl);
-                    break;
-                }
-                n_nodes -= keep;
-                wave_sync();
-                {
-                    const uint32_t excl = incl - packed;
-                    emit_bits(leaf ? lds.pairs : lds.nodes, leaf ? n_pairs + (excl >> 16) : n_nodes + (excl & 0xFFFFu), m8,
-                              leaf ? ((first_tri + child0) | (src << 24)) : ((src << Lds::kNodeSrcShift) | ((level - 1) << Lds::kNodeLevShift) | child0));
-                    n_nodes += tot & 0xFFFFu;
-                    n_pairs += tot >> 16;
-                }
-                wave_sync();
-            }
-            PT_STAMP(st, 2);
+#include "pt_sphere_tree_walk.inc"
         } else {
             float k1 = a.k1, k2 = a.k2, a_max = a.a_max, m0 = a.m0, m0q = a.m0_quad, t_guard = a.t_guard;
             asm volatile("" : "+v"(k1), "+v"(k2), "+v"(a_max), "+v"(m0), "+v"(m0q), "+v"(t_guard));
@@ -1275,6 +1118,12 @@
     hipLaunchKernelGGL(kernel, dim3(args.n_tiles * args.n_chunks), dim3(kBlock), 0, stream, args);
     return hipGetLastError();
 }
+#elif defined(PT_ROOM_UNIT)
+void (*room_kernel(bool narrow))(const RenderArgs) {
+    if (!narrow) return &integrate_kernel<false, false, false, false, false, 8>;
+    if constexpr (plan::variant_exists({false, false, false, false, true, 0, 0, true}, kBuild)) return &integrate_kernel<false, false, false, false, true, 8>;
+    else return nullptr;
+}
 #elif defined(PT_SURFACE_UNIT)
 #define PT_UNIT_NAME_1 glass
 #define PT_UNIT_NAME_2 texture
@@ -1535,6 +1384,7 @@
 Kernel kernel_of() {
     constexpr plan::Variant v = plan::variant_of(I);
     if constexpr (!plan::variant_exists(v, kBuild)) return nullptr;
+    else if constexpr (v.room) return room_kernel(v.narrow);
     else if constexpr (plan::view_has_motion(v.view) && plan::view_has_lens(v.view)) return &integrate_kernel_motion_lens<v.sky, v.big, v.stats, v.env, v.narrow, v.pool | 1>;
     else if constexpr (plan::view_has_motion(v.view)) return &integrate_kernel_motion<v.sky, v.big, v.stats, v.env, v.narrow, v.pool | 1>;
     else if constexpr (plan::view_has_lens(v.view)) return &integrate_kernel_lens<v.sky, v.big, v.stats, v.env, v.narrow, v.pool | 1>;
@@ -1542,7 +1392,7 @@
 }
 template <int... I>
 std::array<Kernel, sizeof...(I)> kernel_table(std::integer_sequence<int, I...>) { return {kernel_of<I>()...}; }
-const auto kKernels = kernel_table(std::make_integer_sequence<int, plan::kAllVariants>());
+const auto kKernels = kernel_table(std::make_integer_sequence<int, plan::kKernelIds>());
 static_assert(plan::variant_id({true, true, true, true, false, 0, plan::kViews - 1}) < plan::kAllVariants, "every view's ids fit the table");
 template <int R>
 Kernel projection_kernel_of() {
@@ -1562,6 +1412,7 @@
 hipError_t launch_integrator(const RenderArgs &args, const plan::Variant &v, hipStream_t stream) {
     const int rows = args.row_end - args.row_begin;
     if (rows <= 0 || args.width <= 0) return hipSuccess;
+    if (v.room && (surface_unit_of(args) != kNoSurfaceUnit || args.env_map != nullptr || args.projection != 0)) return hipErrorInvalidDeviceFunction;
     if (const int unit = surface_unit_of(args)) return launch_surface_integrator(unit, args, v, stream);
     if (args.env_map != nullptr) return launch_environment_integrator(args, v, stream);
     const Kernel kernel = kernel_for(v, args.projection != 0);
@@ -1572,7 +1423,7 @@
 
 hipError_t integrator_waves_per_cu(const plan::Variant &v, int *waves) {
     constexpr int kDevices = 16;
-    static std::atomic<int> cache[kDevices][plan::kAllVariants];
+    static std::atomic<int> cache[kDevices][plan::kKernelIds];
     const Kernel kernel = kKernels[plan::variant_id(v)];
     if (!kernel) return hipErrorInvalidDeviceFunction;
     int dev = 0;
diff --git a/path-tracing_amd/csrc/pt_kernels.hpp b/path-tracing_amd/csrc/pt_kernels.hpp
--- a/path-tracing_amd/csrc/pt_kernels.hpp
+++ b/path-tracing_amd/csrc/pt_kernels.hpp
@@ -92,6 +92,7 @@
 }
 hipError_t launch_integrator(const RenderArgs &args, const plan::Variant &v, hipStream_t stream);
 hipError_t launch_environment_integrator(const RenderArgs &args, const plan::Variant &v, hipStream_t stream);
+void (*room_kernel(bool narrow))(const RenderArgs);
 hipError_t launch_surface_integrator(int unit, const RenderArgs &args, const plan::Variant &v, hipStream_t stream);
 hipError_t integrator_waves_per_cu(const plan::Variant &v, int *waves);
 hipError_t launch_projection_rays(const RenderArgs &args, int width, int height, int row_begin, int rows, float *d_origins, float *d_directions,
diff --git a/path-tracing_amd/csrc/pt_launch_plan.hpp b/path-tracing_amd/csrc/pt_launch_plan.hpp
--- a/path-tracing_amd/csrc/pt_launch_plan.hpp
+++ b/path-tracing_amd/csrc/pt_launch_plan.hpp
@@ -18,9 +18,11 @@
 struct Variant {
     bool sky, big, stats, env, narrow;
     int pool, view;
+    bool room = false;
 };
 constexpr bool operator==(const Variant &a, const Variant &b) {
-    return a.sky == b.sky && a.big == b.big && a.stats == b.stats && a.env == b.env && a.narrow == b.narrow && a.pool == b.pool && a.view == b.view;
+    return a.sky == b.sky && a.big == b.big && a.stats == b.stats && a.env == b.env && a.narrow == b.narrow && a.pool == b.pool && a.view == b.view &&
+           a.room == b.room;
 }
 
 constexpr int rays_per_lane(const Build &b, bool sky, bool big, bool stats) { return (!sky && !stats) ? (big ? b.rays_big : b.rays_small) : 1; }
@@ -30,16 +32,23 @@
 constexpr int view_of(bool camera, bool lens, bool motion) { return motion ? (lens ? 4 : 3) : lens ? 2 : camera ? 1 : 0; }
 constexpr bool view_has_lens(int view) { return view == 2 || view == 4; }
 constexpr bool view_has_motion(int view) { return view == 3 || view == 4; }
+constexpr int kRoomVariants = 2, kKernelIds = kAllVariants + kRoomVariants;
 constexpr int variant_id(const Variant &v) {
+    if (v.room) return kAllVariants + v.narrow;
     return kVariantsPerView * v.view + (v.narrow ? 16 + 2 * v.big + v.env : v.pool ? 20 + 2 * v.big + (v.pool == 4) : ((v.sky * 2 + v.big) * 2 + v.stats) * 2 + v.env);
 }
 constexpr Variant variant_of(int id) {
+    if (id >= kAllVariants) return {false, false, false, false, id - kAllVariants == 1, 0, 0, true};
     const int view = id / kVariantsPerView, r = id % kVariantsPerView;
     if (r < 16) return {(r & 8) != 0, (r & 4) != 0, (r & 2) != 0, (r & 1) != 0, false, 0, view};
     if (r < 20) return {false, (r & 2) != 0, false, (r & 1) != 0, true, 0, view};
     return {false, (r & 2) != 0, false, false, false, (r & 1) ? 4 : 2, view};
 }
 constexpr bool variant_exists(const Variant &v, const Build &b) {
+    if (v.room) {
+        if (b.wide_only || v.sky || v.big || v.stats || v.env || v.pool || v.view != 0) return false;
+        return !v.narrow || rays_per_lane(b, false, false, false) > 1;
+    }
     if (b.wide_only && (v.narrow || v.pool || v.view != 0)) return false;
     if (!v.narrow && !v.pool) return true;
     if (v.sky || v.stats || (v.pool && v.env)) return false;
@@ -51,6 +60,7 @@
     int items_per_slot = 0;
     int chunk_min = 0;
     int regen_min_dead = 0;
+    int no_room_kernel = 0;
 };
 
 struct Launch {
@@ -60,6 +70,7 @@
     int pass_begin, pass_count;
     int view;
     int cu_count;
+    bool room = false;
 };
 
 struct Tiles {
@@ -95,6 +106,8 @@
     }
     t.variant.narrow = t.narrow != 0;
     t.variant.pool = t.adapt_pool;
+    t.variant.room = l.room && !o.no_room_kernel && !b.wide_only && !l.sky && !l.big && !stats && !l.may_leave_envelope && l.error < 0.0f &&
+                     l.view == 0 && t.adapt_pool == 0;
     const int tile_px = t.adapt_pool ? t.adapt_pool : rays;
     t.blocks_x = (l.width + b.tile_w * tile_px - 1) / (b.tile_w * tile_px);
     t.n_tiles = static_cast<uint32_t>(t.blocks_x) * rows;
diff --git a/path-tracing_amd/csrc/pt_room_kernels.hip b/path-tracing_amd/csrc/pt_room_kernels.hip
--- /dev/null
+++ b/path-tracing_amd/csrc/pt_room_kernels.hip
@@ -0,0 +1,2 @@
+#define PT_ROOM_UNIT
+#include "pt_kernels.hip"
diff --git a/path-tracing_amd/csrc/pt_scene.hpp b/path-tracing_amd/csrc/pt_scene.hpp
--- a/path-tracing_amd/csrc/pt_scene.hpp
+++ b/path-tracing_amd/csrc/pt_scene.hpp
@@ -105,6 +105,7 @@
     uint32_t emis_clusters = 0xFFFFFFFFu;
     uint32_t emis_large_w0 = 0xFFFFFFFFu;
     bool emis_bvh = true;
+    bool room = false;
 };
 
 #ifdef PT_TEST_HOOKS
diff --git a/path-tracing_amd/csrc/pt_sphere_tree_walk.inc b/path-tracing_amd/csrc/pt_sphere_tree_walk.inc
--- /dev/null
+++ b/path-tracing_amd/csrc/pt_sphere_tree_walk.inc
@@ -0,0 +1,198 @@
+            const uint32_t n_levels = ((ConstU)cp)[8];
+            const uint32_t top = n_levels - 1;
+            if (lane < static_cast<int>(n_levels)) {
+                lds.level_off[lane] = lane == 0 ? 0u : a.clusters[cl].level_off[lane - 1];
+                lds.level_cnt[lane] = (n_tri + (1u << (3 * lane)) - 1u) >> (3 * lane);
+            }
+            wave_sync();
+            uint32_t n_nodes = 0;
+            uint32_t tmask[R];
+#pragma unroll
+            for (int k = 0; k < R; ++k) tmask[k] = 0;
+            auto any_tmask = [&]() {
+                uint32_t x = tmask[0];
+#pragma unroll
+                for (int k = 1; k < R; ++k) x |= tmask[k];
+                return __any(x != 0);
+            };
+            auto push_top = [&](uint32_t top) {
+#pragma unroll
+                for (int k = 0; k < R; ++k) {
+                    if (!PT_SLOT_ON(k)) continue;
+                    while (__any(tmask[k] != 0)) {
+                        const bool has = tmask[k] != 0;
+                        const unsigned long long ball = __ballot(has);
+                        if (n_nodes + __builtin_popcountll(ball) > kNodeStack) return;
+                        if (has) {
+                            const uint32_t j = __builtin_ctz(tmask[k]);
+                            tmask[k] &= tmask[k] - 1;
+                            lds.nodes[n_nodes + lanes_below(ball)] = (static_cast<uint32_t>(lane + 64 * k) << Lds::kNodeSrcShift) | (top << Lds::kNodeLevShift) | j;
+                        }
+                        n_nodes += __builtin_popcountll(ball);
+                    }
+                }
+            };
+            bool rooted = false;
+            if (top >= 1) {
+                unsigned long long pcb[R];
+                uint32_t rcnt = 0;
+#pragma unroll
+                for (int k = 0; k < R; ++k) {
+                    pcb[k] = 0;
+                    if (!PT_SLOT_ON(k)) continue;
+                    pcb[k] = __ballot(pc[k]);
+                    rcnt += __builtin_popcountll(pcb[k]);
+                }
+                const uint32_t clev = top - 1;
+                const uint32_t nchild = (n_tri + (1u << (3 * clev)) - 1u) >> (3 * clev);
+                const uint32_t sh = rcnt <= 1u ? 6u : rcnt <= 2u ? 5u : rcnt <= 4u ? 4u : rcnt <= 8u ? 3u : rcnt <= 16u ? 2u : 0u;
+                const uint32_t per = (nchild + (1u << sh) - 1u) >> sh;
+                if (rcnt <= 16u && per <= 8u) {
+                    ++st.w_node_rounds;
+                    {
+                        uint32_t at = 0;
+#pragma unroll
+                        for (int k = 0; k < R; ++k) {
+                            if (!PT_SLOT_ON(k)) continue;
+                            if (pc[k]) lds.nodes[at + lanes_below(pcb[k])] = static_cast<uint32_t>(lane + 64 * k);
+                            at += __builtin_popcountll(pcb[k]);
+                        }
+                    }
+                    wave_sync();
+                    const uint32_t item = static_cast<uint32_t>(lane) >> sh, sub = static_cast<uint32_t>(lane) & ((1u << sh) - 1u);
+                    const uint32_t c0 = clev == 0 ? sub * per : sub, cstep = clev == 0 ? 1u : (1u << sh);
+                    uint32_t m = 0, src = 0;
+                    if (item < rcnt) {
+                        src = lds.nodes[item];
+                        Ray r;
+                        r.ox = lds.ray[0][src]; r.oy = lds.ray[1][src]; r.oz = lds.ray[2][src];
+                        r.dx = lds.ray[3][src]; r.dy = lds.ray[4][src]; r.dz = lds.ray[5][src];
+                        const float4 *cs = reinterpret_cast<const float4 *>(a.spheres) + off + lds.level_off[clev] + c0;
+                        auto test = [&](auto per_c) {
+                            constexpr uint32_t kPer = decltype(per_c)::value;
+#pragma unroll
+                            for (uint32_t i = 0; i < kPer; ++i) {
+                                const float4 sp = cs[i * cstep];
+                                m |= sphere_keep(sp.x, sp.y, sp.z, sp.w, r) ? (1u << i) : 0u;
+                            }
+                            const uint32_t left = nchild > c0 ? nchild - c0 : 0u;
+                            const uint32_t n_ok = min((left + cstep - 1u) >> (clev == 0 ? 0u : sh), kPer);
+                            m &= (1u << n_ok) - 1u;
+                        };
+                        if (per == 1u) test(std::integral_constant<uint32_t, 1>());
+                        else if (per == 2u) test(std::integral_constant<uint32_t, 2>());
+                        else if (per <= 4u) test(std::integral_constant<uint32_t, 4>());
+                        else test(std::integral_constant<uint32_t, 8>());
+                    }
+                    wave_sync();
+                    const uint32_t mc = __builtin_popcount(m);
+                    const uint32_t incl = wave_scan_inclusive(mc), tot = wave_last(incl);
+                    if (clev == 0) {
+                        if (n_pairs + tot > kPairQueue) drain_pairs(0);
+                        if (tot <= kPairQueue) {
+                            emit_pairs(m, first_tri + c0, src, incl - mc, tot);
+                            rooted = true;
+                        }
+                    } else if (tot <= kNodeStack) {
+                        emit_bits(lds.nodes, n_nodes + incl - mc, m, (src << Lds::kNodeSrcShift) | (clev << Lds::kNodeLevShift) | c0, sh);
+                        n_nodes += tot;
+                        wave_sync();
+                        rooted = true;
+                    }
+                }
+            }
+            if (!rooted) {
+            const uint32_t top_off = top == 0 ? 0u : ((ConstU)cp)[8 + top];
+            const uint32_t top_cnt = (n_tri + (1u << (3 * top)) - 1u) >> (3 * top);
+            const ConstF tp = spheres + 4 * (static_cast<size_t>(off) + top_off);
+            for (uint32_t j = 0; j < top_cnt; ++j) {
+                const float sx = tp[4 * j], sy = tp[4 * j + 1], sz = tp[4 * j + 2], sr = tp[4 * j + 3];
+#pragma unroll
+                for (int k = 0; k < R; ++k)
+                    if (PT_SLOT_ON(k)) tmask[k] |= sphere_keep(sx, sy, sz, sr, q[k]) ? (1u << j) : 0u;
+            }
+#pragma unroll
+            for (int k = 0; k < R; ++k) tmask[k] = pc[k] ? tmask[k] : 0u;
+            PT_STAMP(st, 1);
+            if (top == 0) {
+                add_pending(tmask, first_tri, n_tri);
+#pragma unroll
+                for (int k = 0; k < R; ++k) tmask[k] = 0;
+            } else {
+                push_top(top);
+                wave_sync();
+            }
+            }
+            while (n_nodes > 0 || any_tmask()) {
+                if (n_nodes == 0) {
+                    push_top(top);
+                    wave_sync();
+                }
+                ++st.w_node_rounds;
+                const uint32_t cnt = min(64u, n_nodes);
+                uint32_t shift = cnt <= 8u ? 3u : cnt <= 16u ? 2u : cnt <= 32u ? 1u : 0u;
+                uint32_t m8, src, level, child0, keep, packed, incl, tot;
+                bool leaf;
+                for (;;) {
+                    m8 = 0; src = 0; level = 1; child0 = 0;
+                    const uint32_t item = static_cast<uint32_t>(lane) >> shift, sub = static_cast<uint32_t>(lane) & ((1u << shift) - 1u);
+                    if (item < cnt) {
+                        const uint32_t e = lds.nodes[n_nodes - 1 - item];
+                        src = e >> Lds::kNodeSrcShift;
+                        level = (e >> Lds::kNodeLevShift) & 7u;
+                        child0 = (e & ((1u << Lds::kNodeLevShift) - 1u)) * kFan;
+                        Ray r;
+                        r.ox = lds.ray[0][src]; r.oy = lds.ray[1][src]; r.oz = lds.ray[2][src];
+                        r.dx = lds.ray[3][src]; r.dy = lds.ray[4][src]; r.dz = lds.ray[5][src];
+                        const float4 *cs = reinterpret_cast<const float4 *>(a.spheres) + off + lds.level_off[level - 1] + child0;
+                        auto test = [&](auto per_c) {
+                            constexpr int per = decltype(per_c)::value;
+#pragma unroll
+                            for (int i = 0; i < per; ++i) {
+                                const uint32_t c = sub + (static_cast<uint32_t>(i) << shift);
+                                const float4 sp = cs[c];
+                                m8 |= sphere_keep(sp.x, sp.y, sp.z, sp.w, r) ? (1u << c) : 0u;
+                            }
+                        };
+                        if (shift == 0u) test(std::integral_constant<int, 8>());
+                        else if (shift == 1u) test(std::integral_constant<int, 4>());
+                        else if (shift == 2u) test(std::integral_constant<int, 2>());
+                        else test(std::integral_constant<int, 1>());
+                        const uint32_t real = lds.level_cnt[level - 1];
+                        const uint32_t left = real > child0 ? real - child0 : 0u;
+                        m8 &= left >= 8u ? 0xFFu : ((1u << left) - 1u);
+                    }
+                    leaf = level == 1;
+                    uint32_t kids = __builtin_popcount(m8);
+                    keep = cnt;
+                    packed = leaf ? kids << 16 : kids;
+                    incl = wave_scan_inclusive(packed);
+                    tot = wave_last(incl);
+                    if (n_pairs + (tot >> 16) > kPairQueue) drain_pairs(0);
+                    if (n_pairs + (tot >> 16) <= kPairQueue && n_nodes - cnt + (tot & 0xFFFFu) <= kNodeStack) break;
+                    if (shift != 0u) { shift = 0u; continue; }
+                    const bool fits = static_cast<uint32_t>(lane) < cnt && n_pairs + (incl >> 16) <= kPairQueue &&
+                                      (n_nodes - (lane + 1)) + (incl & 0xFFFFu) <= kNodeStack;
+                    const unsigned long long fb = __ballot(fits);
+                    keep = (fb == ~0ull) ? 64u : static_cast<uint32_t>(__builtin_ctzll(~fb));
+                    if (keep == 0) keep = 1;
+                    ++st.w_partial;
+                    if (static_cast<uint32_t>(lane) >= keep) m8 = 0;
+                    kids = __builtin_popcount(m8);
+                    packed = leaf ? kids << 16 : kids;
+                    incl = wave_scan_inclusive(packed);
+                    tot = wave_last(incl);
+                    break;
+                }
+                n_nodes -= keep;
+                wave_sync();
+                {
+                    const uint32_t excl = incl - packed;
+                    emit_bits(leaf ? lds.pairs : lds.nodes, leaf ? n_pairs + (excl >> 16) : n_nodes + (excl & 0xFFFFu), m8,
+                              leaf ? ((first_tri + child0) | (src << 24)) : ((src << Lds::kNodeSrcShift) | ((level - 1) << Lds::kNodeLevShift) | child0));
+                    n_nodes += tot & 0xFFFFu;
+                    n_pairs += tot >> 16;
+                }
+                wave_sync();
+            }
+            PT_STAMP(st, 2);
```

Result: faster. 7650, median of 6 (+4.9%).
